# takah29/3d-reconstruction-from-multi-view-exp

Hardware: AMD Instinct MI355X
Metric: BA iterations/sec + residual-Jacobian GObs/s, 1M pts x 100 cams fp64 (higher is better)
Workload: dtype f64

## Files before the change

3d-reconstruction-from-multi-view-exp_amd/csrc/check_isa.py:

```python
#!/usr/bin/env python3
import re
import sys

KERNELS = {"k_schur_slots": (("vmcnt(7)", 7), ("vmcnt(8)", 8)),
           "k_schur_lanes": (("vmcnt(13)", 14), ("vmcnt(17)", 18))}
SLOTS_ONLY = "k_schur_slots"
VM_LOOP_OPS = ("global_load_lds_dwordx4", "global_load_lds_dword ")


def kernel_lines(text, name="k_schur_slots"):
    m = re.search(r"^_ZN\d+_GLOBAL__N_1" + str(len(name)) + name + r"E\w*:[^\n]*\n(.*?)^\.Lfunc_end", text, re.S | re.M)
    if not m:
        return None
    return [ln.strip() for ln in m.group(1).splitlines()]


def in_loop(lines, i):
    for k in range(i, -1, -1):
        m = re.match(r"\.(LBB\w+):(.*)", lines[k])
        if m:
            return "Loop" in m.group(2)
    return False


def loop_blocks(lines, wait_index):
    hdr = r"\.(LBB\w+):.*This (?:Inner )?Loop Header: Depth=1"
    head = max(i for i in range(wait_index + 1) if re.match(hdr, lines[i]))
    name = re.match(hdr, lines[head]).group(1)[1:]
    children = set()
    for ln in lines[head + 1:]:
        m = re.match(r";\s+Child Loop (BB\w+) Depth", ln)
        if not m:
            break
        children.add(m.group(1))
    own, inner = [], []
    cur = None
    for i, ln in enumerate(lines):
        m = re.match(r"\.(LBB\w+):(.*)", ln)
        if m:
            label, note = m.group(1)[1:], m.group(2)
            if i == head or f"Header={name} Depth=1" in note:
                cur = own
            elif label in children or any(f"Header={c} " in note for c in children):
                cur = inner
            else:
                cur = None
            continue
        if cur is not None:
            cur.append(ln)
    return own, inner


def check_kernel(text, name, counts):
    errs = []
    lines = kernel_lines(text, name)
    if lines is None:
        return [f"{name} not found in the ISA"]
    for count, n_ops in counts:
        idx = [i for i, ln in enumerate(lines) if ln.startswith("s_waitcnt " + count)]
        if name != SLOTS_ONLY:
            idx = [i for i in idx if in_loop(lines, i)]
        if len(idx) != 1:
            errs.append(f"{name}: expected one `s_waitcnt {count}` (the loop's counted wait), found {len(idx)}")
            continue
        body, inner = loop_blocks(lines, idx[0])
        bad = [ln for ln in body + inner if ln.startswith(("scratch_", "buffer_"))]
        if bad:
            errs.append(f"{name} {count} loop: scratch / buffer access inside the loop: {bad[:3]}")
        straight = [ln for ln in body if ln.startswith(VM_LOOP_OPS)]
        if len(straight) != n_ops:
            errs.append(f"{name} {count} loop: {len(straight)} LDS-DMA operations per iteration, the wait counts {n_ops}")
        other = [ln for ln in body if ln.startswith(("global_load", "global_store", "global_atomic", "flat_")) and not ln.startswith(VM_LOOP_OPS)]
        if other:
            errs.append(f"{name} {count} loop: vector-memory operations the wait does not count (or that return data to a register): {other[:3]}")
        stray = [ln for ln in inner if ln.startswith(VM_LOOP_OPS)]
        if stray:
            errs.append(f"{name} {count} loop: LDS-DMA inside the pacing block: {stray[:3]}")
    if name != SLOTS_ONLY:
        return errs
    for ln in lines:
        if re.match(r"\w+\s+m0\b", ln) and not ln.startswith("s_mov_b32 m0,"):
            errs.append(f"{name}: M0 written outside the gathers' asm statements: {ln}")
    vg = re.search(r"^\s*\.set _ZN\d+_GLOBAL__N_1" + str(len(name)) + name + r"E\w*\.num_vgpr, (\d+)", text, re.M)
    if vg and int(vg.group(1)) > 168:
        errs.append(f"{name} needs {vg.group(1)} VGPRs: more than the 168 of three waves per SIMD")
    return errs


# ... 48 lines not shown
```

3d-reconstruction-from-multi-view-exp_amd/csrc/host_check.cpp:

```cpp
#include <cmath>
#include <cstdio>
#include <cstring>
#include <limits>
#include <string>
#include <vector>

#include "mvba_host.h"
#include "mvba_ransac_host.h"
#include "mvba_tracks_host.h"
#include "mvba_match_host.h"

namespace mvba {
thread_local std::string g_err;
}
using namespace mvba;

static int failures = 0;
#define CHECK(x) do { if (!(x)) { std::printf("host_check: line %d: %s\n", __LINE__, #x); ++failures; } } while (0)

int main() {
  {
    const int n = 3;
    const double D[9] = {1.0, 0, 0, 0, 4.0, 0, 0, 0, 2.0};
    const double V[9] = {-0.5, 0.6, 0.0,
// ... 382 lines not shown
    int32_t cam[5], node[5], track[5];
    double xy[10];
    auto run = [&](const int64_t *kp_, const double *kxy_, const int32_t *e, int64_t ne, int32_t ml, int64_t *pt_, int32_t *cam_, int32_t *node_,
                   double *xy_, int32_t *track_, int64_t *cnt_) { return tracks_check_args(3, kp_, kxy_, e, ne, ml, pt_, cam_, node_, xy_, track_, cnt_); };
    CHECK(run(kp, kxy, edges, 3, 2, pt, cam, node, xy, track, counts) == MVBA_OK);
    CHECK(run(kp, nullptr, edges, 3, 2, pt, cam, node, nullptr, track, counts) == MVBA_OK);
    CHECK(run(kp, kxy, nullptr, 0, 2, pt, cam, node, xy, track, counts) == MVBA_OK);
    CHECK(run(nullptr, kxy, edges, 3, 2, pt, cam, node, xy, track, counts) == MVBA_ERR_BADARG && g_err == "null argument: kp_ptr (argument 2)");
    CHECK(run(kp, kxy, edges, 3, 2, nullptr, cam, node, xy, track, counts) == MVBA_ERR_BADARG && g_err == "null argument: pt_ptr (argument 8)");
    CHECK(run(kp, kxy, edges, 3, 2, pt, nullptr, node, xy, track, counts) == MVBA_ERR_BADARG && g_err == "null argument: cam_idx (argument 9)");
    CHECK(run(kp, kxy, edges, 3, 2, pt, cam, nullptr, xy, track, counts) == MVBA_ERR_BADARG && g_err == "null argument: obs_node (argument 10)");
    CHECK(run(kp, kxy, edges, 3, 2, pt, cam, node, xy, nullptr, counts) == MVBA_ERR_BADARG && g_err == "null argument: node_track (argument 12)");
    CHECK(run(kp, kxy, edges, 3, 2, pt, cam, node, xy, track, nullptr) == MVBA_ERR_BADARG && g_err == "null argument: counts (argument 13)");
    CHECK(run(kp, nullptr, edges, 3, 2, pt, cam, node, xy, track, counts) == MVBA_ERR_BADARG && g_err == "null argument: kp_xy (argument 3) with an xy to fill");
    CHECK(run(kp, kxy, edges, -1, 2, pt, cam, node, xy, track, counts) == MVBA_ERR_BADARG && g_err == "n_edges = -1: negative size");
    CHECK(run(kp, kxy, nullptr, 3, 2, pt, cam, node, xy, track, counts) == MVBA_ERR_BADARG && g_err == "null argument: edges (argument 4) with n_edges = 3");
    CHECK(run(kp, kxy, edges, 3, 1, pt, cam, node, xy, track, counts) == MVBA_ERR_BADARG && g_err == "min_length = 1 must be at least 2");
    CHECK(run(down, kxy, edges, 3, 2, pt, cam, node, xy, track, counts) == MVBA_ERR_BADARG && g_err.rfind("kp_ptr is not ascending", 0) == 0);
    CHECK(run(kp, kxy, high, 2, 2, pt, cam, node, xy, track, counts) == MVBA_ERR_BADARG && g_err == "edges[1][0] = 5: node id out of range, n_nodes = 5");
    CHECK(run(kp, kxy, low, 2, 2, pt, cam, node, xy, track, counts) == MVBA_ERR_BADARG && g_err == "edges[1][1] = -1: node id out of range, n_nodes = 5");
    CHECK(run(kp, kxy, high, 1, 2, pt, cam, node, xy, track, counts) == MVBA_OK);
  }
  {
    const double r2 = match_ratio2(0.8);
    CHECK(r2 == 0.8 * 0.8 && match_ratio2(1.0) == 1.0);
    CHECK(match_ambiguous(100, -1, r2) && match_ambiguous(0, -1, 1.0));
    CHECK(!match_ambiguous(63, 100, r2) && match_ambiguous(65, 100, r2));
    CHECK(match_ambiguous(100, 100, 1.0) && !match_ambiguous(99, 100, 1.0));
    CHECK(match_ambiguous(0, 0, 1.0) && !match_ambiguous(0, 1, r2));
    CHECK(!match_ambiguous(33292799, 33292800, 1.0) && match_ambiguous(33292800, 33292800, 1.0));
    const int64_t kp[5] = {0, 10, 10, 40, 45};
    const int32_t pr[10] = {0, 2, 2, 0, 1, 3, 3, 2, 0, 3};
    CHECK(match_chunk_end(kp, pr, 5, 0, false, 1000) == 5 && match_chunk_end(kp, pr, 5, 0, true, 1000) == 5);
    CHECK(match_chunk_end(kp, pr, 5, 0, false, 40) == 3);
    CHECK(match_chunk_end(kp, pr, 5, 0, true, 40) == 1);
    CHECK(match_chunk_end(kp, pr, 5, 1, true, 1) == 2);
    CHECK(match_chunk_end(kp, pr, 5, 2, false, 0) == 3 && match_chunk_end(kp, pr, 5, 3, false, 0) == 4);
    CHECK(match_chunk_end(kp, pr, 5, 5, true, 10) == 5 && match_chunk_end(kp, pr, 0, 0, true, 10) == 0);
    for (int32_t p0 = 0, guard = 0; p0 < 5 && guard < 10; ++guard) {
      const int32_t p1 = match_chunk_end(kp, pr, 5, p0, true, 35);
      CHECK(p1 > p0 && p1 <= 5);
      p0 = p1;
    }
  }
  {
    const int64_t kp[4] = {0, 2, 2, 5}, down[4] = {0, 3, 2, 5}, off[3] = {1, 2, 3}, big[2] = {0, 1LL << 31}, none[3] = {0, 0, 0};
    const int64_t huge[3] = {0, 1LL << 30, (1LL << 30) + 1};
    const uint8_t desc[5 * 32] = {0};
    const int32_t pr[4] = {0, 2, 2, 0}, high[4] = {0, 2, 3, 0}, low[2] = {0, -1}, self[4] = {0, 2, 2, 2}, twice[4] = {0, 1, 0, 1}, empty[4] = {1, 0, 1, 2};
    int64_t mp[3], counts[MATCH_N_COUNTS], Q = -1;
    int32_t kpp[10], d2[5];
    auto run = [&](int32_t m, const int64_t *kp_, const uint8_t *desc_, int32_t dim, const int32_t *pairs, int32_t np, double ratio, int64_t *mp_,
                   int32_t *kpp_, int32_t *d2_, int64_t *cnt_) { return match_check_args(m, kp_, desc_, dim, pairs, np, ratio, mp_, kpp_, d2_, cnt_, &Q); };
    CHECK(run(3, kp, desc, 32, pr, 2, 0.8, mp, kpp, d2, counts) == MVBA_OK && Q == 5);
    CHECK(run(3, kp, desc, 512, pr, 2, 0.0, mp, kpp, d2, counts) == MVBA_OK && run(3, kp, desc, 16, pr, 2, 1.0, mp, kpp, d2, counts) == MVBA_OK);
    CHECK(run(3, kp, desc, 32, nullptr, 0, 0.8, mp, kpp, d2, counts) == MVBA_OK && Q == 0);
    CHECK(run(3, kp, desc, 32, empty, 2, 0.8, mp, kpp, d2, counts) == MVBA_OK && Q == 0);
    CHECK(run(2, none, nullptr, 128, nullptr, 0, 0.8, mp, kpp, d2, counts) == MVBA_OK);
    CHECK(run(3, nullptr, desc, 32, pr, 2, 0.8, mp, kpp, d2, counts) == MVBA_ERR_BADARG && g_err == "null argument: kp_ptr (argument 2)");
    CHECK(run(3, kp, desc, 32, pr, 2, 0.8, nullptr, kpp, d2, counts) == MVBA_ERR_BADARG && g_err == "null argument: match_ptr (argument 10)");
    CHECK(run(3, kp, desc, 32, pr, 2, 0.8, mp, nullptr, d2, counts) == MVBA_ERR_BADARG && g_err == "null argument: kp_pairs (argument 11)");
    CHECK(run(3, kp, desc, 32, pr, 2, 0.8, mp, kpp, nullptr, counts) == MVBA_ERR_BADARG && g_err == "null argument: dist2 (argument 12)");
    CHECK(run(3, kp, desc, 32, pr, 2, 0.8, mp, kpp, d2, nullptr) == MVBA_ERR_BADARG && g_err == "null argument: counts (argument 16)");
    CHECK(run(3, kp, nullptr, 32, pr, 2, 0.8, mp, kpp, d2, counts) == MVBA_ERR_BADARG && g_err == "null argument: desc (argument 3) with 5 keypoints");
    CHECK(run(3, kp, desc, 32, nullptr, 2, 0.8, mp, kpp, d2, counts) == MVBA_ERR_BADARG && g_err == "null argument: pairs (argument 5) with n_pairs = 2");
    CHECK(run(3, kp, desc, 32, pr, -1, 0.8, mp, kpp, d2, counts) == MVBA_ERR_BADARG && g_err == "n_pairs = -1: negative size");
    CHECK(run(0, kp, desc, 32, pr, 2, 0.8, mp, kpp, d2, counts) == MVBA_ERR_BADARG && g_err == "n_images = 0 must be at least 1");
    CHECK(run(2, off, desc, 32, pr, 0, 0.8, mp, kpp, d2, counts) == MVBA_ERR_BADARG && g_err == "kp_ptr[0] = 1 must be 0");
    CHECK(run(3, down, desc, 32, pr, 2, 0.8, mp, kpp, d2, counts) == MVBA_ERR_BADARG && g_err == "kp_ptr is not ascending: kp_ptr[2] = 2 after 3");
    CHECK(run(1, big, desc, 32, pr, 0, 0.8, mp, kpp, d2, counts) == MVBA_ERR_BADARG && g_err == "n_nodes = kp_ptr[n_images] = 2147483648 must be < 2^31");
    for (int32_t dim : {0, 8, 24, 520, 528, -16}) {
      CHECK(run(3, kp, desc, dim, pr, 2, 0.8, mp, kpp, d2, counts) == MVBA_ERR_BADARG);
      CHECK(g_err == "dim = " + std::to_string(dim) + " must be a multiple of 16 in 16 .. 512");
    }
    CHECK(run(3, kp, desc, 32, pr, 2, -0.1, mp, kpp, d2, counts) == MVBA_ERR_BADARG && g_err == "ratio = -0.100000 must be in (0, 1], or 0 for no ratio test");
    CHECK(run(3, kp, desc, 32, pr, 2, 1.5, mp, kpp, d2, counts) == MVBA_ERR_BADARG && g_err == "ratio = 1.500000 must be in (0, 1], or 0 for no ratio test");
    CHECK(run(3, kp, desc, 32, pr, 2, std::numeric_limits<double>::quiet_NaN(), mp, kpp, d2, counts) == MVBA_ERR_BADARG && g_err.find("nan must be in") != std::string::npos);
    CHECK(run(3, kp, desc, 32, high, 2, 0.8, mp, kpp, d2, counts) == MVBA_ERR_BADARG && g_err == "pairs[1][0] = 3: image index out of range, n_images = 3");
    CHECK(run(3, kp, desc, 32, low, 1, 0.8, mp, kpp, d2, counts) == MVBA_ERR_BADARG && g_err == "pairs[0][1] = -1: image index out of range, n_images = 3");
    CHECK(run(3, kp, desc, 32, self, 2, 0.8, mp, kpp, d2, counts) == MVBA_ERR_BADARG && g_err == "pairs[1] = (2, 2): an image is not matched with itself");
    CHECK(run(2, huge, desc, 32, twice, 2, 0.8, mp, kpp, d2, counts) == MVBA_ERR_BADARG && g_err == "Q = 2147483648 queries up to pair 1: the sum over the pairs must be < 2^31");
    CHECK(run(2, huge, desc, 32, twice, 1, 0.8, mp, kpp, d2, counts) == MVBA_OK && Q == (1LL << 30));
  }
  if (failures) return 1;
  std::printf("host_check ok\n");
  return 0;
}
```

3d-reconstruction-from-multi-view-exp_amd/csrc/mvba.hip:

```cpp
#include <dlfcn.h>
#include <hip/hip_runtime.h>
#include <rccl/rccl.h>

#include <algorithm>
#include <atomic>
#include <chrono>
#include <cmath>
#include <cstdlib>
#include <cstring>
#include <thread>
#include <type_traits>
#include <utility>
#include <vector>

#include "mvba_common.h"
#include "mvba_host.h"
#include "mvba_ransac_host.h"
#include "mvba_tracks_host.h"
#include "mvba_match_host.h"

namespace mvba {
thread_local std::string g_err;
}
using namespace mvba;
// ... 28 lines not shown
  Rccl r;
  r.lib = lib;
  r.origin = origin;
#define BIND(field, sym)                                                                       \
  if (!(r.field = reinterpret_cast<decltype(r.field)>(dlsym(lib, sym))))                       \
    return fail(MVBA_ERR_RCCL, std::string("librccl (") + origin + ") lacks " + sym)
  BIND(GetVersion, "ncclGetVersion");
  BIND(GetUniqueId, "ncclGetUniqueId");
  BIND(CommInitRank, "ncclCommInitRank");
  BIND(CommDestroy, "ncclCommDestroy");
  BIND(AllReduce, "ncclAllReduce");
  BIND(AllGather, "ncclAllGather");
  BIND(GetErrorString, "ncclGetErrorString");
#undef BIND
  if (r.GetVersion(&r.version) != ncclSuccess) return fail(MVBA_ERR_RCCL, "ncclGetVersion failed");
  const int major = r.version >= 10000 ? r.version / 10000 : r.version / 1000;
  if (major != NCCL_MAJOR)
    return fail(MVBA_ERR_RCCL, "librccl (" + origin + ") is NCCL " + std::to_string(r.version) + ", this library was built against " +
                                   std::to_string(NCCL_VERSION_CODE));
  g_rccl = r;
  return MVBA_OK;
}
}

namespace {

#include "mvba_device.h"
#include "mvba_linearize.h"
#include "mvba_schur.h"
#include "mvba_dense.h"
#include "mvba_solve.h"
#include "mvba_tail.h"
#include "mvba_index.h"
#include "mvba_cov.h"
#include "mvba_map.h"

}

enum { SCHUR_PAIRS = 1, SCHUR_SLOTS = 2, SCHUR_DENSE = 3 };
struct mvba_handle {
  int device = 0;
  hipStream_t stream = nullptr;
  DevBufs mem;
  long long N = 0, nobs = 0;
  int m = 0, gauge_axis = 0, D = 0, ld = 0;
  double f0 = 1.0;
  long long *d_pt_ptr = nullptr;
  int *d_cam = nullptr, *d_obs_pt = nullptr;
  double2 *d_xy = nullptr;
  int *d_tiles = nullptr;
  int *d_tile_slot = nullptr;
  int4 *d_splits = nullptr;
  double *d_PLsplit = nullptr;
  int n_splits = 0;
  int n_tiles = 0;
  bool any_split = false;
  int k1_threads = 512;
  bool use_pairs = true;
  int schur_mode = 2;
  long long n_items = 0, n_items_offdiag = 0, n_slot_items = 0;
  int n_units = 0, rccl_version = 0, q_max = 0, n_waves = 0, slot_nR = 8, slot_nseg = 0;
  int slot_w = PSTEP;
  long long *d_range_o0 = nullptr;
  int *d_seg_end = nullptr, *d_prog = nullptr;
  bool check_solve = false;
  double check_solve_tol = 1e-8;
  bool gcam = false;
  double *d_cam18 = nullptr, *d_dxi10 = nullptr;
  bool index_on_device = false;
  int4 *d_wdesc = nullptr;
  int *d_it_x = nullptr;
  int *d_wunits = nullptr;
  bool force_big = false;
  int *d_it_k = nullptr, *d_it_l = nullptr, *d_it_a = nullptr, *d_unit_ptr = nullptr, *d_q_ptr = nullptr, *d_q_units = nullptr;
  int4 *d_units = nullptr;
  double *d_partial = nullptr;
  double *d_dense_part = nullptr;
  int *d_dense_obs = nullptr;
  int dense_blocks = 0, dense_tiles = 0;
  double *d_X[2] = {nullptr, nullptr}, *d_cam15[2] = {nullptr, nullptr};
  int cur = 0;
  bool have_params = false, linearized = false, have_trial = false;
  double2 *d_rec = nullptr;
  double *d_PL = nullptr, *d_PB = nullptr;
  double *d_Ab = nullptr, *d_Ared = nullptr, *d_Ztiles = nullptr, *d_Lblk = nullptr, *d_dxi = nullptr, *d_dX = nullptr, *d_lu = nullptr;
  int *d_ipiv = nullptr;
  double *d_partials = nullptr, *d_cost = nullptr, *h_cost = nullptr;
  double *d_mail = nullptr;
  unsigned long long cost_seq = 0;
  bool mail_pending = false;
  int n_partials = 0, cost_grid = 0;
  int *d_flag = nullptr, *h_flag = nullptr;
  unsigned *d_bar = nullptr;
  int n_cu = 1;
  bool chol_onepass = true;
  int trail64_min = 200;
  unsigned barrier_polls = 1u << 22;
  ncclComm_t comm = nullptr;
  mvba_host_allreduce_fn host_ar = nullptr;
  void *host_ar_user = nullptr;
  std::vector<double> host_buf;
  int rank = 0, nranks = 1;
  double *d_allcost = nullptr, *h_allcost = nullptr, *d_sim = nullptr;
  std::vector<double *> snap_slabs;
  long long n_snap = 0;
  int profiling = 0;
  mvba_stats stats{};
  struct Ev { int kid; hipEvent_t a, b; };
  std::vector<Ev> pending;
  std::vector<hipEvent_t> pool;
  double *d_cov_sig = nullptr, *d_cov_panel = nullptr, *d_cov_pts = nullptr, *d_cov_cam = nullptr;
  int loss = LOSS_SQUARED;
  double loss_b = 0.0;
  double *d_sqw = nullptr;
  double2 *d_resid = nullptr;
  double *d_init_cams = nullptr;
  bool mapped = false;
  int n_free = 0, map_ld = 0, map_U = 0;
  std::vector<int> map_col, map_ptr, map_mem;
  int *d_map_col = nullptr, *d_map_ptr = nullptr, *d_map_mem = nullptr;
  double *d_map_x = nullptr, *d_cov_sigv = nullptr;
  int2 *d_map_pairs = nullptr;
  double *d_map_part = nullptr;
  int n_map_pairs = 0, map_nblk = 1;
  uint8_t *d_held = nullptr;
  long long n_held = 0;
  int solve_D() const { return mapped ? n_free : D; }
  int solve_ld() const { return mapped ? map_ld : ld; }
};

namespace {

const char *kKernelNames[MVBA_K_COUNT] = {"resid_jac", "point_blocks", "point_inv", "schur",
                                          "allreduce", "solve",        "backsub_cost", "cost"};

struct Timed {
  mvba_handle *h;
  int kid;
  hipEvent_t a = nullptr, b = nullptr;
  bool on = false;
  Timed(mvba_handle *h_, int kid_) : h(h_), kid(kid_) {
    on = kid >= 0 && (h->profiling == 1 || (h->profiling == 2 && (kid == MVBA_K_SCHUR || kid == MVBA_K_RESID_JAC)));
    if (!on) return;
    auto get = [&]() {
      hipEvent_t e;
      if (!h->pool.empty()) { e = h->pool.back(); h->pool.pop_back(); }
      else hipEventCreate(&e);
      return e;
    };
    a = get(); b = get();
    hipEventRecord(a, h->stream);
  }
  ~Timed() {
    if (!on) return;
    hipEventRecord(b, h->stream);
    h->pending.push_back({kid, a, b});
  }
};

void drain_events(mvba_handle *h) {
  for (auto &p : h->pending) {
    float ms = 0.f;
    if (hipEventElapsedTime(&ms, p.a, p.b) == hipSuccess) {
      h->stats.ms[p.kid] += ms;
      h->stats.launches[p.kid] += 1;
    }
// ... 88 lines not shown
  const void *fn(bool rb) const { return rb ? (const void *)robust : (const void *)squared; }
};
template <typename... A>
LossKernel<A...> loss_kernel(void (*squared)(A...), void (*robust)(A..., LossArgs)) { return {squared, robust}; }

template <typename... A, typename... Args>
void launch_loss(mvba_handle *h, LossKernel<A...> k, dim3 grid, dim3 block, size_t lds, Args... args) {
  if (h->loss != LOSS_SQUARED) hipLaunchKernelGGL(k.robust, grid, block, lds, h->stream, args..., LossArgs{h->loss_b, h->d_sqw});
  else hipLaunchKernelGGL(k.squared, grid, block, lds, h->stream, args...);
}

auto resid_jac_kernel(bool gcam, int loss) {
  if (loss == LOSS_CAUCHY)
    return gcam ? loss_kernel(k_resid_jac<true>, k_resid_jac<true, LOSS_CAUCHY, LossArgs>) : loss_kernel(k_resid_jac<false>, k_resid_jac<false, LOSS_CAUCHY, LossArgs>);
  return gcam ? loss_kernel(k_resid_jac<true>, k_resid_jac<true, LOSS_HUBER, LossArgs>) : loss_kernel(k_resid_jac<false>, k_resid_jac<false, LOSS_HUBER, LossArgs>);
}
auto cost_kernel(bool gcam, int loss) {
  if (loss == LOSS_CAUCHY)
    return gcam ? loss_kernel(k_cost<true>, k_cost<true, LOSS_CAUCHY, LossArgs>) : loss_kernel(k_cost<false>, k_cost<false, LOSS_CAUCHY, LossArgs>);
  return gcam ? loss_kernel(k_cost<true>, k_cost<true, LOSS_HUBER, LossArgs>) : loss_kernel(k_cost<false>, k_cost<false, LOSS_HUBER, LossArgs>);
}
template <int G>
auto backsub_kernel_g(int bt, bool gcam) {
  if (gcam) return loss_kernel(k_backsub<G, 256, true>, k_backsub<G, 256, true, true, LossArgs>);
  if (bt == 1024) return loss_kernel(k_backsub<G, 1024>, k_backsub<G, 1024, false, true, LossArgs>);
  if (bt == 512) return loss_kernel(k_backsub<G, 512>, k_backsub<G, 512, false, true, LossArgs>);
  return loss_kernel(k_backsub<G>, k_backsub<G, 256, false, true, LossArgs>);
}
auto backsub_kernel(int G, int bt, bool gcam) {
  return G == 2 ? backsub_kernel_g<2>(bt, gcam) : (G == 4 ? backsub_kernel_g<4>(bt, gcam) : backsub_kernel_g<8>(bt, gcam));
}
template <int T>
auto dense_kernel_t(bool table) {
  return table ? loss_kernel(k_schur_dense<T, true>, k_schur_dense<T, true, true, LossArgs>)
               : loss_kernel(k_schur_dense<T, false>, k_schur_dense<T, false, true, LossArgs>);
}
auto dense_kernel(int T, bool table) {
  switch (T) {
    case 1: return dense_kernel_t<1>(table);
    case 2: return dense_kernel_t<2>(table);
    case 3: return dense_kernel_t<3>(table);
    case 4: return dense_kernel_t<4>(table);
    case 5: return dense_kernel_t<5>(table);
    case 6: return dense_kernel_t<6>(table);
    case 7: return dense_kernel_t<7>(table);
    case 8: return dense_kernel_t<8>(table);
    case 9: return dense_kernel_t<9>(table);
    case 10: return dense_kernel_t<10>(table);
    case 11: return dense_kernel_t<11>(table);
    default: return dense_kernel_t<12>(table);
  }
}
size_t dense_lds_bytes(int T, int mm) {
  const int CH = dense_ch(T);
  return sizeof(double) * ((size_t)2 * 3 * CH * 16 * T + (size_t)2 * CH * mm * 32) + sizeof(double2) * CH * ((size_t)mm * REC + 8) +
         sizeof(double) * (CH * (size_t)mm + 2 * 3 * CH);
}

size_t k1_lds_bytes(int m, bool gcam, int threads) {
  return (size_t)((gcam ? 0 : ((m * CAM_LDS + 1) & ~1)) + (threads / 64) * 64 * 2 * REC) * sizeof(double);
}
size_t cam_lds_bytes(int m, bool gcam, bool with_dxi) { return gcam ? 0 : (size_t)m * (CAM_LDS + (with_dxi ? DXI_LDS : 0)) * sizeof(double); }

void cam_tables(mvba_handle *h, const double *cam15, const double *dxi) {
  if (h->gcam) hipLaunchKernelGGL(k_cam_tables, dim3((h->m + 255) / 256), dim3(256), 0, h->stream, h->m, cam15, dxi, h->f0, h->d_cam18, h->d_dxi10);
}
int launch_cost(mvba_handle *h, const double *cam15, const double *X) {
  const size_t lds = cam_lds_bytes(h->m, h->gcam, false);
  cam_tables(h, cam15, nullptr);
  launch_loss(h, cost_kernel(h->gcam, h->loss), dim3(h->cost_grid), dim3(lds > 40 * 1024 ? 512 : 256), lds, h->nobs, h->m, cam15, X,
              h->d_obs_pt, h->d_cam, h->d_xy, h->f0, h->d_partials, h->d_cam18);
  double *mail = cost_mail(h);
  const unsigned long long seq = h->cost_seq;
  hipLaunchKernelGGL(k_sum_partials, dim3(1), dim3(1024), 0, h->stream, h->d_partials, h->cost_grid, h->d_cost, h->d_flag, mail, seq);
  MVBA_HIP(hipGetLastError());
  return MVBA_OK;
}

struct CreateKnobs {
  bool schur_set = false;
  bool schur_slots = false, schur_lanes = false, schur_pairs = false, schur_dense = false;
  bool index_host = false, index_global = false;
  bool force_big = false;
  bool chol_launches = false;
  int trail64_min = 200;
  unsigned barrier_polls = 1u << 22;
  bool check_solve = false;
  double check_solve_tol = 1e-8;
  bool timing = false;
};

CreateKnobs read_create_knobs() {
  CreateKnobs k;
  auto is = [](const char *ev, const char *v) { return ev && !strcmp(ev, v); };
  const char *schur = getenv("MVBA_SCHUR");
  k.schur_set = schur != nullptr;
  k.schur_slots = is(schur, "slots");
  k.schur_lanes = is(schur, "lanes");
  k.schur_pairs = is(schur, "pairs");
  k.schur_dense = is(schur, "dense");
  const char *index = getenv("MVBA_INDEX");
  k.index_host = is(index, "host");
  k.index_global = is(index, "global");
  k.force_big = getenv("MVBA_FORCE_BIG") != nullptr;
  k.chol_launches = is(getenv("MVBA_CHOL"), "launches");
  if (const char *ev = getenv("MVBA_TRAIL64_MIN")) k.trail64_min = std::max(0, atoi(ev));
  if (const char *ev = getenv("MVBA_CHOL_BARRIER_POLLS")) k.barrier_polls = (unsigned)std::max(0LL, atoll(ev));
  if (const char *ev = getenv("MVBA_CHECK_SOLVE")) {
    const double v = atof(ev);
    k.check_solve = v != 0.0;
    if (v > 0.0 && v < 1.0) k.check_solve_tol = v;
  }
  k.timing = getenv("MVBA_CREATE_TIMING") != nullptr;
  return k;
}

#include "mvba_create.h"

}

extern "C" {

const char *mvba_version(void) { return "mvba 0.2 (gfx950)"; }
const char *mvba_last_error(void) { return g_err.c_str(); }
const char *mvba_kernel_name(int32_t k) { return (k >= 0 && k < MVBA_K_COUNT) ? kKernelNames[k] : ""; }

int mvba_device_count(int32_t *count) {
  int n = 0;
  hipError_t e = hipGetDeviceCount(&n);
  if (e != hipSuccess) {
    *count = 0;
    return fail(MVBA_ERR_HIP, std::string("hipGetDeviceCount: ") + hipGetErrorString(e));
  }
  *count = n;
  return MVBA_OK;
}

int mvba_create(const mvba_problem *p, mvba_handle **out) { return create_engine(p, LOSS_SQUARED, 0.0, out); }

int mvba_create_robust(const mvba_problem *p, int32_t loss, double scale, mvba_handle **out) {
  if (!p || !out) return fail(MVBA_ERR_BADARG, "null argument");
  if (loss == LOSS_SQUARED) return create_engine(p, LOSS_SQUARED, 0.0, out);
  if (loss != LOSS_HUBER && loss != LOSS_CAUCHY)
    return fail(MVBA_ERR_BADARG, "loss = " + std::to_string(loss) + " is not a loss (0 squared, 1 Huber, 2 Cauchy)");
  if (!(scale > 0.0) || !std::isfinite(scale))
    return fail(MVBA_ERR_BADARG, "loss scale = " + std::to_string(scale) + " must be finite and > 0 for a robust loss");
  if (!(p->f0 > 0.0) || !std::isfinite(p->f0)) return fail(MVBA_ERR_BADARG, "a robust loss needs f0 > 0");
  const double r = scale / p->f0;
  return create_engine(p, loss, r * r, out);
}

void mvba_destroy(mvba_handle *h) {
  if (!h) return;
  hipSetDevice(h->device);
  if (h->stream) hipStreamSynchronize(h->stream);
  if (h->comm) g_rccl.CommDestroy(h->comm);
  h->mem.release_all();
  if (h->h_cost) hipHostFree(h->h_cost);
  if (h->h_allcost) hipHostFree(h->h_allcost);
  for (auto &p : h->pending) { hipEventDestroy(p.a); hipEventDestroy(p.b); }
  for (auto e : h->pool) hipEventDestroy(e);
  if (h->stream) hipStreamDestroy(h->stream);
  delete h;
}

namespace {
void pack_cam15(int m, const double *f, const double *u, const double *t, const double *R, double *cam ) {
  for (int k = 0; k < m; ++k) {
    double *c = cam + (size_t)k * CAM_IN;
    c[0] = f[k]; c[1] = u[2 * k]; c[2] = u[2 * k + 1];
    for (int i = 0; i < 3; ++i) c[3 + i] = t[3 * k + i];
    for (int i = 0; i < 9; ++i) c[6 + i] = R[9 * k + i];
  }
}
void unpack_cam15(const double *cam , int m, double *f, double *u, double *t, double *R) {
  for (int k = 0; k < m; ++k) {
    const double *c = cam + (size_t)k * CAM_IN;
    f[k] = c[0]; u[2 * k] = c[1]; u[2 * k + 1] = c[2];
    for (int i = 0; i < 3; ++i) t[3 * k + i] = c[3 + i];
    for (int i = 0; i < 9; ++i) R[9 * k + i] = c[6 + i];
  }
}
}

int mvba_set_params(mvba_handle *h, const double *X, const double *f, const double *u, const double *t, const double *R) {
  if (!h || !X || !f || !u || !t || !R) return fail(MVBA_ERR_BADARG, "null argument");
  MVBA_HIP(hipSetDevice(h->device));
  std::vector<double> cam((size_t)h->m * CAM_IN);
  pack_cam15(h->m, f, u, t, R, cam.data());
  MVBA_HIP(hipMemcpyAsync(h->d_X[h->cur], X, sizeof(double) * 3 * h->N, hipMemcpyHostToDevice, h->stream));
  MVBA_HIP(hipMemcpyAsync(h->d_cam15[h->cur], cam.data(), sizeof(double) * cam.size(), hipMemcpyHostToDevice, h->stream));
  MVBA_HIP(hipStreamSynchronize(h->stream));
  h->have_params = true; h->linearized = false; h->have_trial = false;
  return MVBA_OK;
}

int mvba_get_params(mvba_handle *h, double *X, double *f, double *u, double *t, double *R) {
  if (!h || !X || !f || !u || !t || !R) return fail(MVBA_ERR_BADARG, "null argument");
  if (!h->have_params) return fail(MVBA_ERR_STATE, "no parameters set");
  MVBA_HIP(hipSetDevice(h->device));
  std::vector<double> cam((size_t)h->m * CAM_IN);
  MVBA_HIP(hipMemcpyAsync(X, h->d_X[h->cur], sizeof(double) * 3 * h->N, hipMemcpyDeviceToHost, h->stream));
  MVBA_HIP(hipMemcpyAsync(cam.data(), h->d_cam15[h->cur], sizeof(double) * cam.size(), hipMemcpyDeviceToHost, h->stream));
  MVBA_HIP(hipStreamSynchronize(h->stream));
  unpack_cam15(cam.data(), h->m, f, u, t, R);
  return MVBA_OK;
}

int mvba_apply_similarity(mvba_handle *h, const double *R0, const double *t0, double scale) {
  if (!h || !R0 || !t0) return fail(MVBA_ERR_BADARG, "null argument");
  if (!h->have_params) return fail(MVBA_ERR_STATE, "no parameters set");
  MVBA_HIP(hipSetDevice(h->device));
  double T[13];
  memcpy(T, R0, 9 * sizeof(double));
  memcpy(T + 9, t0, 3 * sizeof(double));
  T[12] = scale;
  if (!h->d_sim) {
    int rc = h->mem.alloc(&h->d_sim, 13);
    if (rc) return rc;
  }
  MVBA_HIP(hipMemcpyAsync(h->d_sim, T, sizeof(T), hipMemcpyHostToDevice, h->stream));
  const long long n = std::max<long long>(h->N, h->m);
  hipLaunchKernelGGL(k_similarity, dim3((unsigned)((n + 255) / 256)), dim3(256), 0, h->stream, h->N, h->m, h->d_X[h->cur],
                     h->d_cam15[h->cur], h->d_sim);
  MVBA_HIP(hipGetLastError());
  MVBA_HIP(hipStreamSynchronize(h->stream));
  h->linearized = false; h->have_trial = false;
  return MVBA_OK;
}

int mvba_cost(mvba_handle *h, double *E) {
  if (!h || !E) return fail(MVBA_ERR_BADARG, "null argument");
  if (!h->have_params) return fail(MVBA_ERR_STATE, "no parameters set");
  MVBA_HIP(hipSetDevice(h->device));
  {
    Timed t(h, MVBA_K_COST);
    int rc = launch_cost(h, h->d_cam15[h->cur], h->d_X[h->cur]);
    if (rc) return rc;
  }
  return global_cost(h, E);
}

namespace {
void launch_resid_jac(mvba_handle *h) {
  const int kt = h->k1_threads;
  cam_tables(h, h->d_cam15[h->cur], nullptr);
  const int wpb = kt / 64;
  const int grid = std::max(1, std::min(2048 * 256 / kt, (h->n_tiles + wpb - 1) / wpb));
  launch_loss(h, resid_jac_kernel(h->gcam, h->loss), dim3(grid), dim3(kt), k1_lds_bytes(h->m, h->gcam, kt), h->nobs, h->m, h->d_cam15[h->cur],
              h->d_X[h->cur], h->d_obs_pt, h->d_cam, h->d_xy, h->f0, h->d_tiles, h->n_tiles, h->d_rec, h->d_PL,
              h->d_tile_slot, h->d_PLsplit, h->d_cam18);
  if (h->n_splits)
    hipLaunchKernelGGL(k_sum_split, dim3((9 * h->n_splits + 255) / 256), dim3(256), 0, h->stream, h->n_splits, h->d_splits,
                       h->d_PLsplit, h->d_PL);
}

void launch_point_inv(mvba_handle *h, double c) {
  const int m = h->m;
  const size_t n9 = 9 * (size_t)m, nA = strip_offset(m, m);
  const long long nAb = (long long)(nA + n9);
  const unsigned grid = (unsigned)std::max<long long>((h->N + 255) / 256, std::min<long long>((nAb + 1023) / 1024, 4096));
  const long long nprog = h->slot_w == LANES_W ? 0 : (long long)h->slot_nR * h->slot_nseg * PACE_STRIDE;
  const int want_r = h->schur_mode == SCHUR_DENSE ? 1 : 0;
  if (h->n_held)
    hipLaunchKernelGGL(k_point_inv<const uint8_t *>, dim3(std::max(grid, 1u)), dim3(256), 0, h->stream, h->N, c, h->d_PL, h->d_PB, h->d_flag,
                       h->d_Ab, nAb, h->d_prog, nprog, want_r, (const uint8_t *)h->d_held);
  else
    hipLaunchKernelGGL(k_point_inv<>, dim3(std::max(grid, 1u)), dim3(256), 0, h->stream, h->N, c, h->d_PL, h->d_PB, h->d_flag,
                       h->d_Ab, nAb, h->d_prog, nprog, want_r);
}

void launch_schur(mvba_handle *h, double c) {
  const int m = h->m;
  const size_t nA = strip_offset(m, m);
  double *d_A = h->d_Ab, *d_b = h->d_Ab + nA;
  if (h->use_pairs) {
    const bool big = (std::max<long long>(h->nobs, h->N) + 1) * 128LL >= (1LL << 32) || h->force_big;
    if (h->schur_mode == SCHUR_SLOTS && h->slot_w == LANES_W) {
      if (h->n_waves)
        hipLaunchKernelGGL(k_schur_lanes, dim3(h->n_waves), dim3(64), LANES_LDS, h->stream, h->d_wdesc, h->d_wunits, h->d_it_x, h->d_rec, h->d_PB, c,
                           h->f0, h->d_partial, h->slot_nR, h->d_range_o0);
    } else if (h->schur_mode == SCHUR_SLOTS) {
      if (h->n_waves)
        hipLaunchKernelGGL(k_schur_slots, dim3(h->n_waves), dim3(64), SLOT_LDS, h->stream, h->d_wdesc,
                           h->d_wunits, h->d_it_x, (const int *)nullptr, (const int *)nullptr, h->d_rec, h->d_PB, c, h->f0, h->d_partial,
                           h->slot_nR, h->d_seg_end, h->d_prog, h->slot_nseg, SLOT_LAG, h->d_range_o0);
    } else if (h->n_units) {
      auto launch = [&](auto kern, auto... robust) {
        hipLaunchKernelGGL(kern, dim3(8 * h->q_max), dim3(64), PAIRS_LDS, h->stream, h->d_units, h->d_q_ptr, h->d_q_units, h->d_it_k, h->d_it_l,
                           h->d_it_a, h->d_rec, h->d_PB, c, h->f0, h->d_partial, robust...);
      };
      if (h->loss != LOSS_SQUARED) launch(big ? k_schur_pairs_big_robust : k_schur_pairs_robust, (const double *)h->d_sqw);
      else launch(big ? k_schur_pairs_big : k_schur_pairs);
    }
    hipLaunchKernelGGL(k_schur_reduce, dim3((unsigned)((long long)m * (m + 1) / 2)), dim3(128), 0, h->stream, m, h->d_unit_ptr,
                       h->d_partial, d_A, d_b);
  } else if (h->schur_mode == SCHUR_DENSE) {
    const int T = (9 * m + 15) / 16;
    launch_loss(h, dense_kernel(T, h->d_dense_obs != nullptr), dim3(h->dense_blocks), dim3(64 * (dense_consumers(T) + dense_ch(T))), dense_lds_bytes(T, m),
                (const double2 *)h->d_rec, (const double *)h->d_PB, (const int *)h->d_dense_obs, (long long)h->N, m, 1.0 / h->f0, h->d_dense_part);
    const long long n_el = (long long)nA + 9 * m;
    hipLaunchKernelGGL(k_schur_dense_finish, dim3((unsigned)((n_el + 3) / 4)), dim3(256), 0, h->stream, m, T, h->dense_blocks,
                       (const double *)h->d_dense_part, c, d_A, d_b);
  }
}

int allreduce_Ab(mvba_handle *h, bool timed) {
  const int m = h->m;
  const size_t n9 = 9 * (size_t)m, nA = strip_offset(m, m);
  if (h->comm) {
    Timed t(h, timed ? MVBA_K_ALLREDUCE : -1);
    ncclResult_t r = g_rccl.AllReduce(h->d_Ab, h->d_Ab, nA + n9, ncclDouble, ncclSum, h->comm, h->stream);
    if (r != ncclSuccess) return fail(MVBA_ERR_RCCL, std::string("ncclAllReduce: ") + g_rccl.GetErrorString(r));
  } else if (h->host_ar) {
    h->host_buf.resize(nA + n9);
    MVBA_HIP(hipMemcpyAsync(h->host_buf.data(), h->d_Ab, sizeof(double) * (nA + n9), hipMemcpyDeviceToHost, h->stream));
    MVBA_HIP(hipStreamSynchronize(h->stream));
    const auto t0 = std::chrono::steady_clock::now();
    if (h->host_ar(h->host_ar_user, h->host_buf.data(), (int64_t)(nA + n9))) return fail(MVBA_ERR_RCCL, "host all-reduce callback failed");
    MVBA_HIP(hipMemcpyAsync(h->d_Ab, h->host_buf.data(), sizeof(double) * (nA + n9), hipMemcpyHostToDevice, h->stream));
    if (timed && h->profiling) {
      h->stats.ms[MVBA_K_ALLREDUCE] += std::chrono::duration<double, std::milli>(std::chrono::steady_clock::now() - t0).count();
      h->stats.launches[MVBA_K_ALLREDUCE] += 1;
    }
  }
  return MVBA_OK;
}

void launch_map_tied(mvba_handle *h, double *M, int ld, int mirror) {
  if (!h->n_map_pairs) return;
  hipLaunchKernelGGL(k_map_tied, dim3(h->n_map_pairs, h->map_nblk), dim3(256), 0, h->stream, h->m, (const double *)h->d_Ab,
                     (const int *)h->d_map_ptr, (const int *)h->d_map_mem, (const int2 *)h->d_map_pairs, h->d_map_part);
  hipLaunchKernelGGL(k_map_tied_finish, dim3((h->n_map_pairs + 255) / 256), dim3(256), 0, h->stream, h->n_map_pairs, h->map_nblk, ld,
                     mirror, (const int2 *)h->d_map_pairs, (const double *)h->d_map_part, M);
}

void launch_factor(mvba_handle *h) {
  const int m = h->m, D = h->solve_D();
  double *d_A = h->d_Ab, *d_b = h->d_Ab + strip_offset(m, m);
  const int ld = h->solve_ld();
  const int ntc = (D + NB - 1) / NB;
  if (h->mapped) {
    const int U = h->map_U, ntu = (U + NB - 1) / NB;
    hipLaunchKernelGGL(k_map_compact, dim3(ntu * (ntu + 1) / 2 + (D + 255) / 256), dim3(256), 0, h->stream, D, ld, m, U, ntu, d_A, d_b,
                       h->d_map_ptr, h->d_map_mem, h->d_Ared, h->d_bar, 1 + 4 * ((D + SBW - 1) / SBW));
    if (U < D)
      hipLaunchKernelGGL(k_map_rows, dim3((D + 63) / 64, D - U), dim3(256), 0, h->stream, D, ld, m, U, d_A, h->d_map_ptr, h->d_map_mem,
                         h->d_Ared);
    launch_map_tied(h, h->d_Ared, ld, 0);
  } else
  hipLaunchKernelGGL(k_compact, dim3(ntc * (ntc + 1) / 2 + (D + 255) / 256), dim3(256), 0, h->stream, D, ld, m, h->gauge_axis, ntc, d_A, d_b,
                     h->d_Ared, h->d_bar, 1 + 4 * ((D + SBW - 1) / SBW));
  for (int jS = 0; jS < D; jS += SBW) {
    const int jE = std::min(jS + SBW, D);
    hipLaunchKernelGGL(k_chol_super, dim3((D + 1 - jE + 63) / 64), dim3(SUPER_THREADS), SUPER_LDS, h->stream, h->d_Ared, ld, D, jS,
                       h->d_Ztiles + (size_t)(jS / NB) * NB * NB, h->d_Lblk + (size_t)(jS / SBW) * SBW * SBW, h->d_flag);
    if (jE < D) {
      const int nt32 = (D + 1 - jE + NB - 1) / NB, nt64 = (D + 1 - jE + TB - 1) / TB;
      if (jE - jS == SBW && nt64 * (nt64 + 1) / 2 >= h->trail64_min)
        hipLaunchKernelGGL(k_chol_trail64, dim3(nt64 * (nt64 + 1) / 2), dim3(256), TRAIL64_LDS, h->stream, h->d_Ared, ld, D, jS, jE);
      else
        hipLaunchKernelGGL(k_chol_trail32, dim3(nt32 * (nt32 + 1) / 2), dim3(256), 0, h->stream, h->d_Ared, ld, D, jS, jE);
// ... 291 lines not shown
  if (!pairs.empty()) MVBA_HIP(hipMemcpy(h->d_map_pairs, pairs.data(), sizeof(int2) * pairs.size(), hipMemcpyHostToDevice));
  MVBA_HIP(hipMemcpy(h->d_map_col, col, sizeof(int) * n9, hipMemcpyHostToDevice));
  MVBA_HIP(hipMemcpy(h->d_map_ptr, ptr.data(), sizeof(int) * (n_free + 1), hipMemcpyHostToDevice));
  MVBA_HIP(hipMemcpy(h->d_map_mem, mem.data(), sizeof(int) * mem.size(), hipMemcpyHostToDevice));
  h->map_col.assign(col, col + n9);
  h->map_ptr = ptr;
  h->map_mem = mem;
  h->n_free = n_free;
  h->map_ld = (n_free + 3) & ~3;
  h->map_U = U;
  h->mapped = true;
  return MVBA_OK;
}

int mvba_set_point_hold(mvba_handle *h, const uint8_t *held) {
  if (!h) return fail(MVBA_ERR_BADARG, "null handle");
  MVBA_HIP(hipSetDevice(h->device));
  long long n_held = 0;
  std::vector<uint8_t> mask;
  if (held) {
    mask.resize((size_t)h->N);
    for (long long a = 0; a < h->N; ++a) n_held += (mask[(size_t)a] = held[a] ? 1 : 0);
  }
  if (n_held && !h->d_held) {
    int rc = h->mem.alloc(&h->d_held, (size_t)h->N);
    if (rc) return rc;
  }
  if (n_held) {
    MVBA_HIP(hipStreamSynchronize(h->stream));
    MVBA_HIP(hipMemcpy(h->d_held, mask.data(), mask.size(), hipMemcpyHostToDevice));
  }
  h->n_held = n_held;
  h->have_trial = false;
  return MVBA_OK;
}

int mvba_residuals(mvba_handle *h, double *e) {
  if (!h || !e) return fail(MVBA_ERR_BADARG, "null argument");
  if (!h->have_params) return fail(MVBA_ERR_STATE, "no parameters set");
  MVBA_HIP(hipSetDevice(h->device));
  if (!h->nobs) return MVBA_OK;
  if (!h->d_resid) {
    int rc = h->mem.alloc(&h->d_resid, h->nobs);
    if (rc) return rc;
  }
  const size_t lds = cam_lds_bytes(h->m, h->gcam, false);
  cam_tables(h, h->d_cam15[h->cur], nullptr);
  const unsigned grid = (unsigned)std::min<long long>(4096, (h->nobs + 255) / 256);
  hipLaunchKernelGGL(h->gcam ? k_residuals<true> : k_residuals<false>, dim3(grid), dim3(256), lds, h->stream, h->nobs, h->m,
                     (const double *)h->d_cam15[h->cur], (const double *)h->d_X[h->cur], (const int *)h->d_obs_pt, (const int *)h->d_cam,
                     (const double2 *)h->d_xy, h->f0, h->d_resid, (const double *)h->d_cam18);
  MVBA_HIP(hipGetLastError());
  MVBA_HIP(hipMemcpyAsync(e, h->d_resid, sizeof(double2) * h->nobs, hipMemcpyDeviceToHost, h->stream));
  MVBA_HIP(hipStreamSynchronize(h->stream));
  return MVBA_OK;
}

int mvba_covariance(mvba_handle *h, double *point_cov, double *cam_cov, double *cam_cov_full, double *timings_ms) {
  if (!h) return fail(MVBA_ERR_BADARG, "null handle");
  if (h->loss != LOSS_SQUARED)
    return fail(MVBA_ERR_BADARG, "mvba_covariance: the covariance is defined for the squared loss only (this engine has a robust loss)");
  if (!h->have_params) return fail(MVBA_ERR_STATE, "no parameters set");
  MVBA_HIP(hipSetDevice(h->device));
  const int m = h->m, D = h->solve_D(), ld = h->solve_ld(), nt = (D + NB - 1) / NB;
  const size_t n_sig = sig_block(m, m, m);
  auto free_cov = [&]() {
    for (double **q : {&h->d_cov_sig, &h->d_cov_panel, &h->d_cov_pts, &h->d_cov_cam}) h->mem.release(*q);
  };
  int local_rc = MVBA_OK;
  if (!h->d_cov_sig || !h->d_cov_panel || !h->d_cov_pts || !h->d_cov_cam) {
    free_cov();
    local_rc = h->mem.alloc(&h->d_cov_sig, n_sig);
    if (!local_rc) local_rc = h->mem.alloc(&h->d_cov_panel, 2 * (size_t)h->D * NB);
    if (!local_rc) local_rc = h->mem.alloc(&h->d_cov_pts, 6 * (size_t)h->N);
    if (!local_rc) local_rc = h->mem.alloc(&h->d_cov_cam, 81 * (size_t)m);
    if (local_rc) free_cov();
  }
  hipEvent_t ev[5] = {};
  struct EvFree { hipEvent_t *e; ~EvFree() { for (int i = 0; i < 5; ++i) if (e[i]) hipEventDestroy(e[i]); } } ev_free{ev};
  for (auto &e : ev)
    if (!local_rc && hipEventCreate(&e) != hipSuccess) local_rc = fail(MVBA_ERR_HIP, "hipEventCreate failed");
  const int mv = (D + 6) / 9 + 1;
  if (!local_rc && h->mapped && D > 0 && !h->d_cov_sigv) local_rc = h->mem.alloc(&h->d_cov_sigv, n_sig);
  const bool sharded = h->comm || h->host_ar;
  if (local_rc && !sharded) return local_rc;
  const std::string local_err = local_rc ? g_err : std::string();
  double *d_b = h->d_Ab + strip_offset(m, m);
  if (!local_rc) {
    MVBA_HIP(hipEventRecord(ev[0], h->stream));
    if (h->nobs) launch_resid_jac(h);
    h->linearized = true; h->have_trial = false;
    launch_point_inv(h, 0.0);
    launch_schur(h, 0.0);
    MVBA_HIP(hipGetLastError());
  } else {
    MVBA_HIP(hipMemsetAsync(d_b + 3, 0xFF, sizeof(double), h->stream));
  }
  {
    int rc = allreduce_Ab(h, false);
    if (rc) return rc;
  }
  if (sharded) {
    double mark = 0.0;
    MVBA_HIP(hipMemcpyAsync(&mark, d_b + 3, sizeof(double), hipMemcpyDeviceToHost, h->stream));
    MVBA_HIP(hipStreamSynchronize(h->stream));
    if (local_rc) return fail(local_rc, local_err);
    if (std::isnan(mark))
      return fail(MVBA_ERR_HIP, "mvba_covariance: another rank could not allocate its covariance buffers (or the reduced system is not finite)");
  }
  MVBA_HIP(hipEventRecord(ev[1], h->stream));
  if (D > 0) launch_factor(h);
  MVBA_HIP(hipEventRecord(ev[2], h->stream));
  if (D > 0)
  hipLaunchKernelGGL(k_cov_assemble, dim3(nt), dim3(256), 0, h->stream, h->d_Ared, ld, D, (const double *)h->d_Ztiles,
                     (const double *)h->d_Lblk);
  double *panel[2] = {h->d_cov_panel, h->d_cov_panel + (size_t)D * NB};
  for (int J = nt - 1; J >= 0; --J) {
    const int grid = (nt - 1 - J) + (J >= 1 ? nt - J : 0);
    if (grid)
      hipLaunchKernelGGL(k_cov_trtri, dim3(grid), dim3(256), 0, h->stream, h->d_Ared, ld, D, nt, J, (const double *)panel[J & 1],
                         panel[(J + 1) & 1]);
  }
  MVBA_HIP(hipMemsetAsync(h->d_cov_sig, 0, sizeof(double) * n_sig, h->stream));
  if (h->mapped) {
    if (D > 0) {
      hipLaunchKernelGGL(k_cov_lauum, dim3(nt * (nt + 1) / 2), dim3(256), 0, h->stream, (const double *)h->d_Ared, ld, D, nt, mv,
                         h->gauge_axis, h->d_cov_sigv);
      hipLaunchKernelGGL(k_map_cov_expand, dim3((unsigned)((81 * m + 255) / 256), m), dim3(256), 0, h->stream, m, mv, h->gauge_axis,
                         (const int *)h->d_map_col, (const double *)h->d_cov_sigv, h->d_cov_sig);
    }
  } else
  hipLaunchKernelGGL(k_cov_lauum, dim3(nt * (nt + 1) / 2), dim3(256), 0, h->stream, (const double *)h->d_Ared, ld, D, nt, m,
                     h->gauge_axis, h->d_cov_sig);
  MVBA_HIP(hipEventRecord(ev[3], h->stream));
  if (h->N && point_cov) {
    const double pairs = h->N ? 0.5 * ((double)h->nobs / (double)h->N) * ((double)h->nobs / (double)h->N + 1.0) : 0.0;
    const int G = pairs > 48.0 ? 64 : (pairs > 24.0 ? 32 : (pairs > 12.0 ? 16 : 8));
    const unsigned grid = (unsigned)std::min<long long>(8192, (h->N * G + 255) / 256);
    auto launch = [&](auto kern, auto... held) {
      hipLaunchKernelGGL(kern, dim3(grid), dim3(256), 0, h->stream, h->N, m, (const long long *)h->d_pt_ptr, (const int *)h->d_cam,
                         (const double2 *)h->d_rec, (const double *)h->d_PL, (const double *)h->d_cov_sig, 1.0 / h->f0, h->d_cov_pts,
                         h->d_flag, held...);
    };
    if (h->n_held) {
      using M = const uint8_t *;
      launch(G == 64 ? k_point_cov<64, M> : (G == 32 ? k_point_cov<32, M> : (G == 16 ? k_point_cov<16, M> : k_point_cov<8, M>)), (M)h->d_held);
    } else
      launch(G == 64 ? k_point_cov<64> : (G == 32 ? k_point_cov<32> : (G == 16 ? k_point_cov<16> : k_point_cov<8>)));
  }
  if (cam_cov)
    hipLaunchKernelGGL(k_cov_cam_diag, dim3((unsigned)((81LL * m + 255) / 256)), dim3(256), 0, h->stream, m,
                       (const double *)h->d_cov_sig, h->d_cov_cam);
  MVBA_HIP(hipGetLastError());
  MVBA_HIP(hipEventRecord(ev[4], h->stream));
  int fl = 0;
  MVBA_HIP(hipMemcpyAsync(&fl, h->d_flag, sizeof(int), hipMemcpyDeviceToHost, h->stream));
  MVBA_HIP(hipStreamSynchronize(h->stream));
  if (fl) {
    MVBA_HIP(hipMemsetAsync(h->d_flag, 0, sizeof(int), h->stream));
    MVBA_HIP(hipStreamSynchronize(h->stream));
    if (fl & (FLAG_POINT_SINGULAR | FLAG_COV_POINT)) return fail(MVBA_ERR_SINGULAR, "Singular matrix (a point block E_a is singular: a point seen once, or without parallax)");
    return fail(MVBA_ERR_SINGULAR, "Singular matrix (the undamped reduced camera system is not positive definite)");
  }
  if (timings_ms)
    for (int i = 0; i < 4; ++i) {
      float ms = 0.f;
      MVBA_HIP(hipEventElapsedTime(&ms, ev[i], ev[i + 1]));
      timings_ms[i] = ms;
    }
  if (point_cov && h->N) MVBA_HIP(hipMemcpy(point_cov, h->d_cov_pts, sizeof(double) * 6 * h->N, hipMemcpyDeviceToHost));
  if (cam_cov) MVBA_HIP(hipMemcpy(cam_cov, h->d_cov_cam, sizeof(double) * 81 * m, hipMemcpyDeviceToHost));
  if (cam_cov_full) {
    std::vector<double> strip((size_t)SIG_BS * m);
    const size_t n9 = 9 * (size_t)m;
    for (int k = 0; k < m; ++k) {
      MVBA_HIP(hipMemcpy(strip.data(), h->d_cov_sig + sig_block(k, k, m), sizeof(double) * SIG_BS * (m - k), hipMemcpyDeviceToHost));
      for (int l = k; l < m; ++l) {
        const double *b = strip.data() + (size_t)SIG_BS * (l - k);
        for (int i = 0; i < 9; ++i)
          for (int j = 0; j < 9; ++j) {
            const double v = 2.0 * b[9 * i + j];
            cam_cov_full[(9 * (size_t)k + i) * n9 + 9 * (size_t)l + j] = v;
            cam_cov_full[(9 * (size_t)l + j) * n9 + 9 * (size_t)k + i] = v;
          }
      }
    }
  }
  return MVBA_OK;
}

namespace {
constexpr int SNAP_SLAB = 8;
size_t snap_stride(const mvba_handle *h) { return (3 * (size_t)h->N + (size_t)CAM_IN * h->m + 1) & ~(size_t)1; }
double *snap_entry(const mvba_handle *h, long long i) { return h->snap_slabs[(size_t)(i / SNAP_SLAB)] + snap_stride(h) * (size_t)(i % SNAP_SLAB); }
}

int mvba_snapshot(mvba_handle *h) {
  if (!h) return fail(MVBA_ERR_BADARG, "null handle");
  if (!h->have_params) return fail(MVBA_ERR_STATE, "no parameters set");
  MVBA_HIP(hipSetDevice(h->device));
  if ((size_t)(h->n_snap / SNAP_SLAB) >= h->snap_slabs.size()) {
    double *p = nullptr;
    int rc = h->mem.alloc(&p, snap_stride(h) * SNAP_SLAB);
    if (rc) return rc;
    h->snap_slabs.push_back(p);
  }
  double *dst = snap_entry(h, h->n_snap);
  MVBA_HIP(hipMemcpyAsync(dst, h->d_X[h->cur], sizeof(double) * 3 * h->N, hipMemcpyDeviceToDevice, h->stream));
  MVBA_HIP(hipMemcpyAsync(dst + 3 * h->N, h->d_cam15[h->cur], sizeof(double) * CAM_IN * h->m, hipMemcpyDeviceToDevice, h->stream));
  h->n_snap++;
  return MVBA_OK;
}

int mvba_snapshot_count(mvba_handle *h, int64_t *n) {
  if (!h || !n) return fail(MVBA_ERR_BADARG, "null argument");
  *n = h->n_snap;
  return MVBA_OK;
}

int mvba_snapshot_read(mvba_handle *h, int64_t i, double *X, double *f, double *u, double *t, double *R) {
  if (!h || !X || !f || !u || !t || !R) return fail(MVBA_ERR_BADARG, "null argument");
  if (i < 0 || i >= h->n_snap) return fail(MVBA_ERR_BADARG, "no such log entry");
  MVBA_HIP(hipSetDevice(h->device));
  const double *src = snap_entry(h, i);
  std::vector<double> cam((size_t)h->m * CAM_IN);
  MVBA_HIP(hipMemcpyAsync(X, src, sizeof(double) * 3 * h->N, hipMemcpyDeviceToHost, h->stream));
  MVBA_HIP(hipMemcpyAsync(cam.data(), src + 3 * h->N, sizeof(double) * cam.size(), hipMemcpyDeviceToHost, h->stream));
  MVBA_HIP(hipStreamSynchronize(h->stream));
  unpack_cam15(cam.data(), h->m, f, u, t, R);
  return MVBA_OK;
}

int mvba_snapshot_restore(mvba_handle *h, int64_t i) {
  if (!h) return fail(MVBA_ERR_BADARG, "null handle");
  if (i < 0 || i >= h->n_snap) return fail(MVBA_ERR_BADARG, "no such log entry");
  MVBA_HIP(hipSetDevice(h->device));
  const double *src = snap_entry(h, i);
  MVBA_HIP(hipMemcpyAsync(h->d_X[h->cur], src, sizeof(double) * 3 * h->N, hipMemcpyDeviceToDevice, h->stream));
  MVBA_HIP(hipMemcpyAsync(h->d_cam15[h->cur], src + 3 * h->N, sizeof(double) * CAM_IN * h->m, hipMemcpyDeviceToDevice, h->stream));
  h->have_params = true; h->linearized = false; h->have_trial = false;
  return MVBA_OK;
}

int mvba_snapshot_clear(mvba_handle *h) {
  if (!h) return fail(MVBA_ERR_BADARG, "null handle");
  h->n_snap = 0;
  return MVBA_OK;
}

int mvba_set_profiling(mvba_handle *h, int32_t enabled) {
  if (!h) return fail(MVBA_ERR_BADARG, "null handle");
  h->profiling = enabled == 2 ? 2 : (enabled != 0);
  return MVBA_OK;
}

int mvba_get_stats(mvba_handle *h, mvba_stats *out) {
  if (!h || !out) return fail(MVBA_ERR_BADARG, "null argument");
  MVBA_HIP(hipSetDevice(h->device));
  int rc = sync_and_drain(h);
  if (rc) return rc;
  *out = h->stats;
  return MVBA_OK;
}

int mvba_get_info(mvba_handle *h, int64_t *out8) {
  if (!h || !out8) return fail(MVBA_ERR_BADARG, "null argument");
  out8[0] = h->n_items;
  out8[1] = h->n_items_offdiag;
  out8[2] = h->n_units;
  out8[3] = h->schur_mode | (h->schur_mode == SCHUR_SLOTS ? h->slot_w << 8 : 0);
  out8[4] = h->rccl_version;
  out8[5] = NCCL_VERSION_CODE;
  out8[6] = h->nranks;
  out8[7] = h->schur_mode == SCHUR_SLOTS ? h->n_slot_items : 0;
  return MVBA_OK;
}

int mvba_reset_stats(mvba_handle *h) {
  if (!h) return fail(MVBA_ERR_BADARG, "null handle");
  MVBA_HIP(hipSetDevice(h->device));
  int rc = sync_and_drain(h);
  if (rc) return rc;
  h->stats = mvba_stats{};
  return MVBA_OK;
}

int mvba_comm_unique_id(void *id128) {
  if (!id128) return fail(MVBA_ERR_BADARG, "null argument");
  static_assert(sizeof(ncclUniqueId) == 128, "ncclUniqueId size");
  if (int rc = rccl_load()) return rc;
  ncclUniqueId id;
  ncclResult_t r = g_rccl.GetUniqueId(&id);
  if (r != ncclSuccess) return fail(MVBA_ERR_RCCL, std::string("ncclGetUniqueId: ") + g_rccl.GetErrorString(r));
  memcpy(id128, &id, 128);
  return MVBA_OK;
}

int mvba_comm_init(mvba_handle *h, const void *id128, int32_t rank, int32_t n_ranks) {
  if (!h || !id128 || n_ranks < 1 || rank < 0 || rank >= n_ranks) return fail(MVBA_ERR_BADARG, "bad comm arguments");
  MVBA_HIP(hipSetDevice(h->device));
  if (int rc = rccl_load()) return rc;
  ncclUniqueId id;
  memcpy(&id, id128, 128);
  ncclResult_t r = g_rccl.CommInitRank(&h->comm, n_ranks, id, rank);
  if (r != ncclSuccess) return fail(MVBA_ERR_RCCL, std::string("ncclCommInitRank: ") + g_rccl.GetErrorString(r));
  h->rank = rank; h->nranks = n_ranks;
  h->rccl_version = g_rccl.version;
  int rc = h->mem.alloc(&h->d_allcost, 2 * (size_t)n_ranks);
  if (rc) return rc;
  MVBA_HIP(hipHostMalloc((void **)&h->h_allcost, 2 * sizeof(double) * n_ranks));
  return MVBA_OK;
}

int mvba_comm_init_host(mvba_handle *h, int32_t rank, int32_t n_ranks, mvba_host_allreduce_fn fn, void *user) {
  if (!h || !fn || n_ranks < 1 || rank < 0 || rank >= n_ranks) return fail(MVBA_ERR_BADARG, "bad comm arguments");
  if (h->comm) return fail(MVBA_ERR_STATE, "handle already has an RCCL communicator");
  h->host_ar = fn; h->host_ar_user = user;
  h->rank = rank; h->nranks = n_ranks;
  return MVBA_OK;
}

int mvba_debug_read(mvba_handle *h, int32_t which, double *out, int64_t capacity, int64_t *n) {
  if (!h || !n) return fail(MVBA_ERR_BADARG, "null argument");
  MVBA_HIP(hipSetDevice(h->device));
  const size_t n9 = 9 * (size_t)h->m;
  long long cnt = 0;
  switch (which) {
    case MVBA_BUF_RESIDUAL: cnt = 2 * h->nobs; break;
    case MVBA_BUF_JX: cnt = 6 * h->nobs; break;
    case MVBA_BUF_JC: cnt = 18 * h->nobs; break;
    case MVBA_BUF_E: cnt = 6 * h->N; break;
    case MVBA_BUF_DP: cnt = 3 * h->N; break;
    case MVBA_BUF_A_FULL: cnt = n9 * n9; break;
    case MVBA_BUF_B_FULL: cnt = n9; break;
    case MVBA_BUF_DXI: cnt = n9; break;
    case MVBA_BUF_DX: case MVBA_BUF_TRIAL_X: cnt = 3 * h->N; break;
    case MVBA_BUF_TRIAL_CAM: cnt = (long long)CAM_IN * h->m; break;
    case MVBA_BUF_INDEX_K: case MVBA_BUF_INDEX_L: case MVBA_BUF_INDEX_A:
      cnt = h->schur_mode == SCHUR_SLOTS ? h->n_slot_items : (h->schur_mode == SCHUR_PAIRS ? h->n_items : 0);
      break;
    case MVBA_BUF_INDEX_SEG: cnt = h->schur_mode == SCHUR_SLOTS ? (long long)h->n_waves * h->slot_nseg : 0; break;
    case MVBA_BUF_WEIGHT: cnt = h->nobs; break;
    default: return fail(MVBA_ERR_BADARG, "unknown buffer id");
  }
  *n = cnt;
  if (!out) return MVBA_OK;
  if (capacity < cnt) return fail(MVBA_ERR_BADARG, "output buffer too small");
  MVBA_HIP(hipStreamSynchronize(h->stream));
  auto d2h = [&](const void *src, size_t bytes) { return hipMemcpy(out, src, bytes, hipMemcpyDeviceToHost); };
  if (which == MVBA_BUF_RESIDUAL || which == MVBA_BUF_JX || which == MVBA_BUF_JC) {
    std::vector<double> r((size_t)2 * REC * h->nobs);
    MVBA_HIP(hipMemcpy(r.data(), h->d_rec, sizeof(double) * r.size(), hipMemcpyDeviceToHost));
    std::vector<double> sw;
    if (h->loss != LOSS_SQUARED && which == MVBA_BUF_JC) {
      sw.resize(h->nobs);
      MVBA_HIP(hipMemcpy(sw.data(), h->d_sqw, sizeof(double) * sw.size(), hipMemcpyDeviceToHost));
    }
    for (long long o = 0; o < h->nobs; ++o) {
      const double cu = sw.empty() ? 1.0 / h->f0 : sw[o] / h->f0;
      const double *q = r.data() + (size_t)o * 2 * REC;
      if (which == MVBA_BUF_RESIDUAL) {
        out[2 * o] = q[14]; out[2 * o + 1] = q[15];
      } else if (which == MVBA_BUF_JX) {
        for (int rr = 0; rr < 2; ++rr) for (int i = 0; i < 3; ++i) out[6 * o + 3 * rr + i] = q[2 * i + rr];
      } else {
        double *jc = out + 18 * o;
        for (int rr = 0; rr < 2; ++rr) {
          jc[9 * rr + 0] = q[6 + rr];
          jc[9 * rr + 1] = rr == 0 ? cu : 0.0;
          jc[9 * rr + 2] = rr == 1 ? cu : 0.0;
          for (int i = 0; i < 3; ++i) jc[9 * rr + 3 + i] = -q[2 * i + rr];
          for (int i = 0; i < 3; ++i) jc[9 * rr + 6 + i] = q[8 + 2 * i + rr];
        }
      }
    }
  } else if (which == MVBA_BUF_WEIGHT) {
    if (h->loss != LOSS_SQUARED) MVBA_HIP(d2h(h->d_sqw, sizeof(double) * h->nobs));
    else for (long long o = 0; o < h->nobs; ++o) out[o] = 1.0;
  } else if (which == MVBA_BUF_E || which == MVBA_BUF_DP) {
    std::vector<double> pl(9 * (size_t)h->N);
    MVBA_HIP(hipMemcpy(pl.data(), h->d_PL, sizeof(double) * pl.size(), hipMemcpyDeviceToHost));
    for (long long a = 0; a < h->N; ++a) {
      if (which == MVBA_BUF_E) for (int i = 0; i < 6; ++i) out[6 * a + i] = pl[9 * a + i];
      else for (int i = 0; i < 3; ++i) out[3 * a + i] = pl[9 * a + 6 + i];
    }
  } else if (which == MVBA_BUF_A_FULL) {
    const int m = h->m;
    std::vector<double> pk(strip_offset(m, m));
    MVBA_HIP(hipMemcpy(pk.data(), h->d_Ab, sizeof(double) * pk.size(), hipMemcpyDeviceToHost));
    for (size_t r = 0; r < n9; ++r)
      for (size_t cc = 0; cc < n9; ++cc) {
        const size_t lo = std::min(r, cc), hi = std::max(r, cc);
        const int k = (int)(lo / 9), l = (int)(hi / 9);
        const size_t rr = (k == l) ? r : lo, c2 = (k == l) ? cc : hi;
        out[r * n9 + cc] = pk[strip_offset(k, m) + (rr - 9 * k) * (size_t)(9 * (m - k)) + (c2 - 9 * k)];
      }
  } else if (which == MVBA_BUF_B_FULL) {
    MVBA_HIP(d2h(h->d_Ab + strip_offset(h->m, h->m), sizeof(double) * cnt));
  } else if (which == MVBA_BUF_DXI) {
    MVBA_HIP(d2h(h->d_dxi, sizeof(double) * cnt));
  } else if (which == MVBA_BUF_DX) {
    MVBA_HIP(d2h(h->d_dX, sizeof(double) * cnt));
  } else if (which == MVBA_BUF_TRIAL_X) {
    MVBA_HIP(d2h(h->d_X[1 - h->cur], sizeof(double) * cnt));
  } else if (which == MVBA_BUF_TRIAL_CAM) {
    MVBA_HIP(d2h(h->d_cam15[1 - h->cur], sizeof(double) * cnt));
  } else if (which >= MVBA_BUF_INDEX_K && which <= MVBA_BUF_INDEX_SEG) {
    if (h->schur_mode == SCHUR_SLOTS && which != MVBA_BUF_INDEX_SEG) {
      const int W = h->slot_w, row = slot_idx_ints(W);
      const long long n_steps = cnt / W;
      std::vector<int> tmp((size_t)n_steps * row);
      if (cnt) MVBA_HIP(hipMemcpy(tmp.data(), h->d_it_x, sizeof(int) * tmp.size(), hipMemcpyDeviceToHost));
      const int off = which == MVBA_BUF_INDEX_K ? 0 : (which == MVBA_BUF_INDEX_L ? W : 2 * W);
      for (long long st = 0; st < n_steps; ++st)
        for (int sl = 0; sl < W; ++sl) out[st * W + sl] = (double)tmp[(size_t)st * row + off + sl];
      return MVBA_OK;
    }
    const int *src = which == MVBA_BUF_INDEX_K ? h->d_it_k : (which == MVBA_BUF_INDEX_L ? h->d_it_l : (which == MVBA_BUF_INDEX_A ? h->d_it_a : h->d_seg_end));
    std::vector<int> tmp((size_t)cnt);
    if (cnt) MVBA_HIP(hipMemcpy(tmp.data(), src, sizeof(int) * tmp.size(), hipMemcpyDeviceToHost));
    for (long long i = 0; i < cnt; ++i) out[i] = (double)tmp[i];
  }
  return MVBA_OK;
}

int mvba_project(const double *X, int64_t n_points, const double *K, const double *R, const double *t, int32_t n_images,
                 const int64_t *pt_ptr, const int32_t *cam_idx, int64_t n_obs, double *xy, int32_t device) {
  if (!X || !K || !R || !t || !xy) return fail(MVBA_ERR_BADARG, "null argument");
  if (n_points < 0 || n_images < 1 || n_obs < 0 || (pt_ptr && !cam_idx)) return fail(MVBA_ERR_BADARG, "bad sizes");
  if (!pt_ptr && n_obs != n_points * (int64_t)n_images) return fail(MVBA_ERR_BADARG, "dense grid needs n_obs = n_points * n_images");
  if (n_points >= (1LL << 31)) return fail(MVBA_ERR_BADARG, "n_points must be < 2^31");
  if ((size_t)n_images * 12 * sizeof(double) > 160 * 1024 - 256) return fail(MVBA_ERR_BADARG, "too many cameras for the LDS camera table (max 1704)");
  if (n_obs == 0) return MVBA_OK;
  if (device >= 0) MVBA_HIP(hipSetDevice(device));
// ... 66 lines not shown
```

3d-reconstruction-from-multi-view-exp_amd/csrc/mvba_create.h:

```cpp

__global__ __launch_bounds__(256) void k_xy_from_planes(const double2 *__restrict__ planes, long long N, int m, double2 *__restrict__ xy) {
  const long long a = (long long)blockIdx.x * 256 + threadIdx.x;
  const int k = blockIdx.y;
  if (a < N) xy[a * m + k] = planes[(long long)k * N + a];
}

#define CR(x) do { int rc_ = (x); if (rc_) return rc_; } while (0)
#define CRH(x) do { hipError_t e_ = (x); if (e_ != hipSuccess) return fail(MVBA_ERR_HIP, std::string(#x) + ": " + hipGetErrorString(e_)); } while (0)

struct CreateTimer {
  bool on;
  std::chrono::steady_clock::time_point t_last = std::chrono::steady_clock::now();
  void lap(const char *what) {
    if (!on) return;
    const auto now = std::chrono::steady_clock::now();
    fprintf(stderr, "mvba_create: %-28s %8.1f ms\n", what, std::chrono::duration<double, std::milli>(now - t_last).count());
    t_last = now;
  }
};

int validate_problem(const mvba_problem *p, std::vector<int> &obs_pt) {
  if (p->n_points < 0 || p->n_images < 2 || p->n_obs < 0 || !p->pt_ptr || (p->n_obs && (!p->cam_idx || !p->xy)))
    return fail(MVBA_ERR_BADARG, "bad problem sizes or null arrays (need n_images >= 2)");
  if (p->gauge_axis != 0 && p->gauge_axis != 1) return fail(MVBA_ERR_BADARG, "gauge_axis must be 0 or 1");
// ... 544 lines not shown
  hipLaunchKernelGGL(dv.hist_lds ? k_idx_fill<false> : k_idx_fill<true>, dim3((unsigned)(dv.idx_waves / IDX_WAVES)), dim3(64 * IDX_WAVES), dv.idx_lds,
                     stream, N, m, (int)P, in.d_pt_ptr, in.d_cam, dv.idx_chunk, dv.d_hist, d_S, d_vp_ptr, d_vp_off, d_pk, d_pl, d_pa,
                     (const int *)nullptr);
  CRH(hipGetLastError());
  timer.lap("items sorted by pair");
  std::vector<long long> lo_tab((size_t)VP * (nR + 1));
  {
    long long *d_rl = nullptr, *d_lo = nullptr;
    CR(tmp.alloc(&d_rl, (size_t)nR + 1)); CR(tmp.alloc(&d_lo, lo_tab.size()));
    CRH(hipMemcpyAsync(d_rl, R.lo.data(), sizeof(long long) * (nR + 1), hipMemcpyHostToDevice, stream));
    const long long nt = (long long)lo_tab.size();
    hipLaunchKernelGGL(k_idx_bounds, dim3((unsigned)((nt + 255) / 256)), dim3(256), 0, stream, VP, nR, d_vp_off, d_rl, d_pa, d_lo, (const int *)nullptr);
    CRH(hipMemcpyAsync(lo_tab.data(), d_lo, sizeof(long long) * nt, hipMemcpyDeviceToHost, stream));
    CRH(hipStreamSynchronize(stream));
    tmp.release(d_rl); tmp.release(d_lo);
  }
  std::vector<int> uid;
  number_units(in, plan, [&](int v, int r) { return lo_tab[(size_t)v * (nR + 1) + r]; }, ix, uid);
  timer.lap("units");
  if (plan.mode == SCHUR_SLOTS) {
    SlotWaves sw = make_slot_waves(in, plan, uid, ix);
    const long long n_waves = sw.n_waves;
    const int nSeg = sw.nSeg;
    CR(upload_range_o0(in, R, engine, ix));
    long long *d_slbeg = nullptr, *d_wbeg = nullptr;
    int *d_sllen = nullptr, *d_wsteps = nullptr;
    CR(tmp.alloc(&d_slbeg, sw.sl_beg.size())); CR(tmp.alloc(&d_sllen, sw.sl_len.size()));
    CR(tmp.alloc(&d_wsteps, (size_t)n_waves)); CR(tmp.alloc(&d_wbeg, (size_t)n_waves + 1));
    CRH(hipMemcpyAsync(d_slbeg, sw.sl_beg.data(), sizeof(long long) * sw.sl_beg.size(), hipMemcpyHostToDevice, stream));
    CRH(hipMemcpyAsync(d_sllen, sw.sl_len.data(), sizeof(int) * sw.sl_len.size(), hipMemcpyHostToDevice, stream));
    const int W = plan.W;
    const auto merge_count = W == LANES_W ? k_idx_merge<false, LANES_W> : k_idx_merge<false, PSTEP>;
    const auto merge_fill = W == LANES_W ? k_idx_merge<true, LANES_W> : k_idx_merge<true, PSTEP>;
    hipLaunchKernelGGL(merge_count, dim3((unsigned)n_waves), dim3(64), 0, stream, n_waves, nR, nSeg, slot_skew(W), SLOT_SEG, d_slbeg, d_sllen,
                       ix.d_range_o0, d_pk, d_pl, d_pa, d_wbeg, 0, (int)N, d_wsteps, (int *)nullptr, (int *)nullptr, (int *)nullptr,
                       (int *)nullptr, (const long long *)in.d_pt_ptr);
    std::vector<int> ws32(n_waves);
    CRH(hipMemcpyAsync(ws32.data(), d_wsteps, sizeof(int) * n_waves, hipMemcpyDeviceToHost, stream));
    CRH(hipStreamSynchronize(stream));
    for (long long b = 0; b < n_waves; ++b) sw.w_steps[b] = ws32[b];
    timer.lap("slot merge (count)");
    long long total_steps = 0;
    CR(place_slot_steps(plan, sw, ix, total_steps));
    const size_t rows = (size_t)total_steps * W;
    CR(engine.alloc(&ix.d_it_k, rows)); CR(engine.alloc(&ix.d_it_l, rows)); CR(engine.alloc(&ix.d_it_a, rows));
    CR(engine.alloc(&ix.d_seg_end, ix.seg_end.size()));
    CRH(hipMemcpyAsync(d_wbeg, sw.w_beg.data(), sizeof(long long) * (n_waves + 1), hipMemcpyHostToDevice, stream));
    hipLaunchKernelGGL(merge_fill, dim3((unsigned)n_waves), dim3(64), 0, stream, n_waves, nR, nSeg, slot_skew(W), SLOT_SEG, d_slbeg, d_sllen,
                       ix.d_range_o0, d_pk, d_pl, d_pa, d_wbeg, 0, (int)N, d_wsteps, ix.d_it_k, ix.d_it_l, ix.d_it_a, ix.d_seg_end, (const long long *)in.d_pt_ptr);
    CRH(hipGetLastError());
    CRH(hipStreamSynchronize(stream));
    timer.lap("slot merge (fill)");
    finish_slot_waves(plan, sw, total_steps, ix);
  } else {
    build_work_queues(in, plan, uid, ix);
    engine.adopt(tmp, d_pk); engine.adopt(tmp, d_pl); engine.adopt(tmp, d_pa);
    ix.d_it_k = d_pk; ix.d_it_l = d_pl; ix.d_it_a = d_pa;
  }
  tmp.release_all();
  ix.on_device = true;
  return MVBA_OK;
}

int alloc_engine_buffers(mvba_handle *h, K1Tiles &t) {
  const long long N = h->N, nobs = h->nobs;
  const int m = h->m;
  h->cost_grid = (int)std::max<long long>(1, std::min<long long>(2048, (nobs + 255) / 256));
  h->n_partials = std::max(h->cost_grid, 4096);
  CR(h->mem.alloc(&h->d_obs_pt, nobs));
  CR(h->mem.alloc(&h->d_xy, nobs));
  h->n_tiles = (int)t.tiles.size() - 1;
  h->any_split = t.any_split;
  if (t.any_split) {
    t.tile_slot.resize(t.tiles.size(), -1);
    h->n_splits = (int)t.splits.size();
    CR(h->mem.alloc(&h->d_tile_slot, t.tile_slot.size()));
    CR(h->mem.alloc(&h->d_splits, t.splits.size()));
    CR(h->mem.alloc(&h->d_PLsplit, 9 * (size_t)t.n_split_slots));
    CRH(hipMemcpy(h->d_tile_slot, t.tile_slot.data(), sizeof(int) * t.tile_slot.size(), hipMemcpyHostToDevice));
    CRH(hipMemcpy(h->d_splits, t.splits.data(), sizeof(int4) * t.splits.size(), hipMemcpyHostToDevice));
  }
  CR(h->mem.alloc(&h->d_tiles, t.tiles.size()));
  for (int i = 0; i < 2; ++i) { CR(h->mem.alloc(&h->d_X[i], 3 * N)); CR(h->mem.alloc(&h->d_cam15[i], (size_t)CAM_IN * m)); }
  CR(h->mem.alloc(&h->d_rec, (size_t)REC * (nobs + 1)));
  if (h->loss != LOSS_SQUARED) {
    CR(h->mem.alloc(&h->d_sqw, nobs + 1));
    CRH(hipMemset(h->d_sqw, 0, sizeof(double) * (nobs + 1)));
  }
  CR(h->mem.alloc(&h->d_PL, 9 * N));
  CR(h->mem.alloc(&h->d_PB, (size_t)PBS * (N + 1)));
  CRH(hipMemset(h->d_rec + (size_t)REC * nobs, 0, sizeof(double2) * REC));
  CRH(hipMemset(h->d_PB + (size_t)PBS * N, 0, sizeof(double) * PBS));
  const size_t n9 = 9 * (size_t)m;
  CR(h->mem.alloc(&h->d_Ab, strip_offset(m, m) + n9));
  CR(h->mem.alloc(&h->d_Ared, (size_t)(h->D + 1) * h->ld));
  CR(h->mem.alloc(&h->d_Lblk, (size_t)((h->D + SBW - 1) / SBW) * SBW * SBW));
  CR(h->mem.alloc(&h->d_Ztiles, (size_t)((h->D + NB - 1) / NB) * NB * NB));
  CR(h->mem.alloc(&h->d_dxi, n9));
  CR(h->mem.alloc(&h->d_dX, 3 * N));
  CR(h->mem.alloc(&h->d_partials, h->n_partials));
  CR(h->mem.alloc(&h->d_cost, 2));
  CR(h->mem.alloc(&h->d_flag, 1));
  CR(h->mem.alloc(&h->d_bar, 1 + 4 * (size_t)((9 * m + SBW - 1) / SBW)));
  CRH(hipHostMalloc((void **)&h->h_cost, 4 * sizeof(double), hipHostMallocMapped));
  memset(h->h_cost, 0, 4 * sizeof(double));
  if (hipHostGetDevicePointer((void **)&h->d_mail, h->h_cost, 0) != hipSuccess) h->d_mail = nullptr;
  h->h_flag = reinterpret_cast<int *>(h->h_cost + 1);
  return MVBA_OK;
}

int upload_schur_index(mvba_handle *h, const SchurPlan &plan, SchurIndex &ix) {
  const int m = h->m;
  h->n_items = plan.L.T;
  h->n_items_offdiag = plan.L.T - plan.L.Tdiag;
  h->n_units = (int)ix.units.size();
  h->n_waves = ix.n_waves; h->slot_nR = ix.slot_nR; h->slot_nseg = ix.slot_nseg; h->n_slot_items = ix.n_slot_items;
  h->slot_w = ix.slot_w;
  h->index_on_device = ix.on_device;
  h->d_range_o0 = ix.d_range_o0;
  if (ix.on_device) { h->d_it_k = ix.d_it_k; h->d_it_l = ix.d_it_l; h->d_it_a = ix.d_it_a; h->d_seg_end = ix.d_seg_end; }
  const size_t P1 = (size_t)m * (m + 1) / 2 + 1;
  if (!ix.on_device) { CR(h->mem.alloc(&h->d_it_k, ix.it_k.size())); CR(h->mem.alloc(&h->d_it_l, ix.it_l.size())); CR(h->mem.alloc(&h->d_it_a, ix.it_a.size())); }
  CR(h->mem.alloc(&h->d_units, ix.units.size())); CR(h->mem.alloc(&h->d_unit_ptr, P1));
  CR(h->mem.alloc(&h->d_q_ptr, 9)); CR(h->mem.alloc(&h->d_q_units, ix.q_units.size()));
  CR(h->mem.alloc(&h->d_wdesc, ix.wdesc.size())); CR(h->mem.alloc(&h->d_wunits, ix.wunits.size()));
  if (!ix.on_device) CR(h->mem.alloc(&h->d_seg_end, ix.seg_end.size()));
  CR(h->mem.alloc(&h->d_prog, (size_t)h->slot_nR * std::max(1, h->slot_nseg) * PACE_STRIDE));
  if (!ix.seg_end.empty() && !ix.on_device) CRH(hipMemcpy(h->d_seg_end, ix.seg_end.data(), sizeof(int) * ix.seg_end.size(), hipMemcpyHostToDevice));
  if (!ix.wdesc.empty()) {
    CRH(hipMemcpy(h->d_wdesc, ix.wdesc.data(), sizeof(int4) * ix.wdesc.size(), hipMemcpyHostToDevice));
    CRH(hipMemcpy(h->d_wunits, ix.wunits.data(), sizeof(int) * ix.wunits.size(), hipMemcpyHostToDevice));
  }
  CR(h->mem.alloc(&h->d_partial, (size_t)UNIT_STRIDE * ix.units.size()));
  if (!ix.it_k.empty()) {
    CRH(hipMemcpy(h->d_it_k, ix.it_k.data(), sizeof(int) * ix.it_k.size(), hipMemcpyHostToDevice));
    CRH(hipMemcpy(h->d_it_l, ix.it_l.data(), sizeof(int) * ix.it_l.size(), hipMemcpyHostToDevice));
    CRH(hipMemcpy(h->d_it_a, ix.it_a.data(), sizeof(int) * ix.it_a.size(), hipMemcpyHostToDevice));
  }
  if (!ix.it_k.empty() || ix.on_device) {
    if (h->schur_mode == SCHUR_PAIRS) {
      std::vector<int4> qdesc(ix.units.size());
      for (size_t i = 0; i < ix.q_units.size(); ++i) qdesc[i] = ix.units[ix.q_units[i]];
      CRH(hipMemcpy(h->d_units, qdesc.data(), sizeof(int4) * qdesc.size(), hipMemcpyHostToDevice));
      int mx = 0;
      for (int x = 0; x < 8; ++x) mx = std::max(mx, ix.q_ptr[x + 1] - ix.q_ptr[x]);
      h->q_max = mx;
    }
    if (!ix.q_units.empty()) CRH(hipMemcpy(h->d_q_units, ix.q_units.data(), sizeof(int) * ix.q_units.size(), hipMemcpyHostToDevice));
  }
  if (h->schur_mode == SCHUR_SLOTS && h->n_slot_items) {
    const int W = h->slot_w, row = slot_idx_ints(W);
    const long long n_steps = h->n_slot_items / W;
    CR(h->mem.alloc(&h->d_it_x, (size_t)n_steps * row));
    hipLaunchKernelGGL(k_idx_interleave, dim3((unsigned)((n_steps * row + 255) / 256)), dim3(256), 0, h->stream, n_steps, W, row, h->d_it_k, h->d_it_l,
                       h->d_it_a, h->d_it_x);
    CRH(hipGetLastError());
    CRH(hipStreamSynchronize(h->stream));
    h->mem.release(h->d_it_k); h->mem.release(h->d_it_l); h->mem.release(h->d_it_a);
  }
  CRH(hipMemcpy(h->d_unit_ptr, ix.unit_ptr.data(), sizeof(int) * P1, hipMemcpyHostToDevice));
  CRH(hipMemcpy(h->d_q_ptr, ix.q_ptr.data(), sizeof(int) * 9, hipMemcpyHostToDevice));
  CRH(hipMemset(h->d_partial, 0, sizeof(double) * UNIT_STRIDE * std::max<size_t>(ix.units.size(), 1)));
  return MVBA_OK;
}

int upload_engine(mvba_handle *h, const mvba_problem *p, const std::vector<int> &obs_pt, const K1Tiles &t, const SchurPlan &plan, SchurIndex &ix) {
  const long long N = h->N, nobs = h->nobs;
  const int m = h->m;
  if (nobs) {
    CRH(hipMemcpy(h->d_obs_pt, obs_pt.data(), sizeof(int) * nobs, hipMemcpyHostToDevice));
    if (p->xy_layout == 1) {
      DevBufs tmp;
      double2 *planes = nullptr;
      CRH(hipMalloc((void **)&planes, sizeof(double2) * nobs));
      tmp.own(planes);
      hipError_t e = hipMemcpy(planes, p->xy, sizeof(double2) * nobs, hipMemcpyHostToDevice);
      if (e == hipSuccess) {
        hipLaunchKernelGGL(k_xy_from_planes, dim3((unsigned)((N + 255) / 256), m), dim3(256), 0, 0, planes, N, m, h->d_xy);
        e = hipGetLastError();
        if (e == hipSuccess) e = hipDeviceSynchronize();
      }
      CRH(e);
    } else {
      CRH(hipMemcpy(h->d_xy, p->xy, sizeof(double2) * nobs, hipMemcpyHostToDevice));
    }
  }
  CRH(hipMemcpy(h->d_tiles, t.tiles.data(), sizeof(int) * t.tiles.size(), hipMemcpyHostToDevice));
  CRH(hipMemset(h->d_PL, 0, sizeof(double) * 9 * std::max<long long>(N, 1)));
  CRH(hipMemset(h->d_flag, 0, sizeof(int)));
  if (h->schur_mode == SCHUR_DENSE) {
    const int T = (9 * m + 15) / 16;
    int n_cu_dense = 256;
    hipDeviceGetAttribute(&n_cu_dense, hipDeviceAttributeMultiprocessorCount, h->device);
    h->dense_tiles = T * (T + 1) / 2 + m;
    h->dense_blocks = (int)std::max<long long>(1, std::min<long long>((N + dense_ch(T) - 1) / dense_ch(T), (long long)n_cu_dense * dense_wgs(T)));
    CR(h->mem.alloc(&h->d_dense_part, (size_t)h->dense_blocks * h->dense_tiles * 256));
    if (!plan.dense_obs.empty()) {
      CR(h->mem.alloc(&h->d_dense_obs, plan.dense_obs.size()));
      CRH(hipMemcpy(h->d_dense_obs, plan.dense_obs.data(), sizeof(int) * plan.dense_obs.size(), hipMemcpyHostToDevice));
    }
  }
  if (h->use_pairs) CR(upload_schur_index(h, plan, ix));
  return MVBA_OK;
}

int set_kernel_attributes(mvba_handle *h, const CreateKnobs &knobs) {
  const int m = h->m;
  const bool robust = h->loss != LOSS_SQUARED;
  auto set_lds = [](const void *f, size_t bytes) { return hipFuncSetAttribute(f, hipFuncAttributeMaxDynamicSharedMemorySize, (int)bytes); };
  const size_t cam_lds = cam_lds_bytes(m, h->gcam, true);
  if (h->gcam) { CR(h->mem.alloc(&h->d_cam18, (size_t)m * CAM_LDS)); CR(h->mem.alloc(&h->d_dxi10, (size_t)m * DXI_LDS)); }
  for (int G : {2, 4, 8})
    for (int bt : {256, 512, 1024}) {
      CRH(set_lds(backsub_kernel(G, bt, false).fn(false), cam_lds));
      if (robust) CRH(set_lds(backsub_kernel(G, bt, false).fn(true), cam_lds));
    }
  CRH(set_lds((const void *)k_chol_super, SUPER_LDS));
  CRH(set_lds((const void *)k_chol_backsolve_all<true>, BACKSOLVE_LDS));
  {
    int per_cu = 0;
    CRH(hipDeviceGetAttribute(&h->n_cu, hipDeviceAttributeMultiprocessorCount, h->device));
    CRH(hipOccupancyMaxActiveBlocksPerMultiprocessor(&per_cu, (const void *)k_chol_backsolve_all<true>, SUPER_THREADS, BACKSOLVE_LDS));
    h->chol_onepass = per_cu >= 1 && !knobs.chol_launches;
    h->trail64_min = knobs.trail64_min;
    h->barrier_polls = knobs.barrier_polls;
  }
  const size_t k1_lds = k1_lds_bytes(m, h->gcam, h->k1_threads);
  CRH(set_lds(resid_jac_kernel(h->gcam, h->loss).fn(false), k1_lds));
  CRH(set_lds(cost_kernel(false, h->loss).fn(false), cam_lds));
  CRH(set_lds((const void *)k_residuals<false>, cam_lds));
  if (robust) {
    CRH(set_lds(resid_jac_kernel(h->gcam, h->loss).fn(true), k1_lds));
    CRH(set_lds(cost_kernel(false, h->loss).fn(true), cam_lds));
  }
  if (h->schur_mode == SCHUR_DENSE) {
    const int T = (9 * m + 15) / 16;
    CRH(set_lds(dense_kernel(T, h->d_dense_obs != nullptr).fn(robust), dense_lds_bytes(T, 16 * T / 9)));
  }
  return MVBA_OK;
}

int build_engine(mvba_handle *h, const mvba_problem *p, const CreateKnobs &knobs, const std::vector<int> &obs_pt, K1Tiles &tiles, CreateTimer &timer) {
  const long long N = h->N, nobs = h->nobs;
  const int m = h->m;
  if (p->device >= 0) CRH(hipSetDevice(p->device));
  CRH(hipGetDevice(&h->device));
  CRH(hipStreamCreateWithFlags(&h->stream, hipStreamNonBlocking));
  CR(h->mem.alloc(&h->d_pt_ptr, N + 1));
  CR(h->mem.alloc(&h->d_cam, nobs));
  CRH(hipMemcpy(h->d_pt_ptr, p->pt_ptr, sizeof(long long) * (N + 1), hipMemcpyHostToDevice));
  if (nobs) CRH(hipMemcpy(h->d_cam, p->cam_idx, sizeof(int) * nobs, hipMemcpyHostToDevice));
  timer.lap("device, topology upload");
  h->k1_threads = k1_block_threads(m, h->gcam);

  const bool dev_build = N > 0 && nobs > 0 && !knobs.index_host;
  const IndexInput in{p, N, nobs, (long long)m * (m + 1) / 2, m,
                      (int)std::max(1u, std::min({std::thread::hardware_concurrency(), 16u, (unsigned)m})), h->stream, h->d_pt_ptr, h->d_cam};
  DeviceIndexBuild dv;
  SchurPlan plan;
  SchurIndex ix;
  CR(decide_schur_form(in, knobs, h->loss, h->device, [&](std::vector<long long> &cnt) {
    return dev_build ? count_pairs_device(in, knobs, dv, cnt) : count_pairs_host(in, cnt);
  }, plan, timer));
  h->schur_mode = plan.mode;
  h->use_pairs = plan.mode != SCHUR_DENSE;
  if (h->use_pairs) CR(dev_build ? build_index_device(in, plan, dv, h->mem, ix, timer) : build_index_host(in, plan, h->mem, ix, timer));
  timer.lap("queues / wave descriptors");

  CR(alloc_engine_buffers(h, tiles));
  timer.lap("allocations");
  CR(upload_engine(h, p, obs_pt, tiles, plan, ix));
  timer.lap("uploads");
  CR(set_kernel_attributes(h, knobs));
  timer.lap("attributes");
  return MVBA_OK;
}

int create_engine(const mvba_problem *p, int loss, double loss_b, mvba_handle **out) {
  if (!p || !out) return fail(MVBA_ERR_BADARG, "null argument");
  const CreateKnobs knobs = read_create_knobs();
  CreateTimer timer{knobs.timing};
  std::vector<int> obs_pt;
  CR(validate_problem(p, obs_pt));
  timer.lap("validate, obs_pt");
  K1Tiles tiles = build_k1_tiles(p);
  timer.lap("K1 tiles");

  mvba_handle *h = new mvba_handle();
  const int m = p->n_images;
  h->N = p->n_points; h->nobs = p->n_obs; h->m = m; h->gauge_axis = p->gauge_axis; h->f0 = p->f0; h->D = 9 * m - 7; h->ld = (h->D + 3) & ~3;
  h->loss = loss; h->loss_b = loss_b;
  h->gcam = m > LDS_CAMERAS;
  h->force_big = knobs.force_big;
  h->check_solve = knobs.check_solve;
  h->check_solve_tol = knobs.check_solve_tol;
  if (int rc = build_engine(h, p, knobs, obs_pt, tiles, timer)) {
    const std::string err = g_err;
    mvba_destroy(h);
    g_err = err;
    return rc;
  }
  *out = h;
  return MVBA_OK;
}

#undef CR
#undef CRH
```

3d-reconstruction-from-multi-view-exp_amd/csrc/mvba_device.h:

```cpp

__device__ __forceinline__ double wave_sum(double v) {
#pragma unroll
  for (int off = 32; off > 0; off >>= 1) v += __shfl_down(v, off, 64);
  return v;
}

__device__ __forceinline__ double block_sum(double v, double *s_red ) {
  v = wave_sum(v);
  const int lane = threadIdx.x & 63, w = threadIdx.x >> 6;
  if (lane == 0) s_red[w] = v;
  __syncthreads();
  double t = 0.0;
  if (threadIdx.x == 0) {
    const int nw = (blockDim.x + 63) >> 6;
    for (int i = 0; i < nw; ++i) t += s_red[i];
  }
  return t;
}

__device__ __forceinline__ void load_cams_to_lds(const double *__restrict__ cam15, int m, double f0,
                                                 double *s_cam) {
  for (int k = threadIdx.x; k < m; k += blockDim.x) expand_cam(cam15 + (size_t)k * CAM_IN, f0, s_cam + k * CAM_LDS);
}

__host__ __device__ __forceinline__ size_t strip_offset(int k, int m) {
  return 81 * ((size_t)k * m - (size_t)k * (k - 1) / 2);
}

__device__ __forceinline__ int keep_index(int i, int gauge_axis) {
  if (i < 3) return i;
  return (i + 6 < 12 + gauge_axis) ? i + 6 : i + 7;
}

#define MVBA_CONST_AS __attribute__((address_space(4)))
template <typename T>
__device__ __forceinline__ const T MVBA_CONST_AS *as_const(const T *p) {
#pragma clang diagnostic push
#pragma clang diagnostic ignored "-Wold-style-cast"
  return (const T MVBA_CONST_AS *)p;
#pragma clang diagnostic pop
}

constexpr int REC = 8;
constexpr int LDS_CAMERAS = 646;

template <bool GCAM>
__device__ __forceinline__ const double *cam_row(const double *gcam, const double *s_cam, int k) {
  if constexpr (GCAM) return gcam + (size_t)k * CAM_LDS;
  else return s_cam + k * CAM_LDS;
}
template <bool GCAM>
__device__ __forceinline__ const double *dxi_row(const double *gdxi, const double *s_dxi, int k) {
  if constexpr (GCAM) return gdxi + (size_t)DXI_LDS * k;
  else return s_dxi + DXI_LDS * k;
}
template <bool GCAM>
__device__ __forceinline__ void stage_cams(const double *cam15, int m, double f0, double *s_cam) {
  if constexpr (!GCAM) {
    load_cams_to_lds(cam15, m, f0, s_cam);
    __syncthreads();
  }
}

struct LossArgs {
  double b;
  double *sqw;
};

constexpr int PBS = 16;
constexpr int PACE_STRIDE = 32;
```

3d-reconstruction-from-multi-view-exp_amd/csrc/mvba_host.h:

```cpp
#pragma once
#include <algorithm>
#include <cmath>
#include <cstddef>
#include <numeric>
#include <vector>

#include "mvba_common.h"

namespace mvba {

struct DevBufs {
  std::vector<void *> bufs;
  DevBufs() = default;
  DevBufs(const DevBufs &) = delete;
  DevBufs &operator=(const DevBufs &) = delete;
  ~DevBufs() { release_all(); }
  template <typename T>
  int alloc(T **p, size_t n) {
    const size_t bytes = std::max<size_t>(n, 1) * sizeof(T);
    const hipError_t e = hipMalloc((void **)p, bytes);
    if (e != hipSuccess) {
      size_t fr = 0, tot = 0;
      hipMemGetInfo(&fr, &tot);
      *p = nullptr;
      return fail(MVBA_ERR_HIP, std::string("hipMalloc of ") + std::to_string(bytes) + " bytes: " + hipGetErrorString(e) + " (" + std::to_string(fr >> 20) +
                                    " MiB free of " + std::to_string(tot >> 20) + ")");
    }
    bufs.push_back(*p);
    return MVBA_OK;
  }
  void own(void *q) { bufs.push_back(q); }
  bool forget(void *q) {
    auto it = std::find(bufs.begin(), bufs.end(), q);
    if (it == bufs.end()) return false;
    bufs.erase(it);
    return true;
  }
  template <typename T>
  void release(T *&p) {
    if (p && forget(p)) hipFree(p);
    p = nullptr;
  }
  template <typename T>
  void adopt(DevBufs &from, T *p) {
    if (p && from.forget(p)) bufs.push_back(p);
  }
  void release_all() {
    for (void *q : bufs) hipFree(q);
    bufs.clear();
  }
};

inline void descending_order(const double *v, size_t stride, int k, int *order) {
  std::iota(order, order + k, 0);
  std::sort(order, order + k, [&](int a, int b) { return v[(size_t)a * stride] > v[(size_t)b * stride]; });
}

struct Basis {
  std::vector<int> order;
  std::vector<double> sign;
};
inline int select_basis(const double *D, const double *V, int k, int n, int n_rank, Basis &b) {
  for (int i = 0; i < k; ++i)
    if (!std::isfinite(D[(size_t)i * k + i])) return fail(MVBA_ERR_SINGULAR, "SVD did not converge (non-finite values in the measurement matrix)");
  b.order.resize(k);
  descending_order(D, (size_t)k + 1, k, b.order.data());
  b.sign.resize(n_rank);
  for (int i = 0; i < n_rank; ++i) {
    const int col = b.order[i];
    int big = 0;
    for (int c = 1; c < n; ++c)
      if (std::fabs(V[(size_t)c * k + col]) > std::fabs(V[(size_t)big * k + col])) big = c;
    b.sign[i] = V[(size_t)big * k + col] < 0.0 ? -1.0 : 1.0;
  }
  return MVBA_OK;
}
inline double basis_at(const Basis &b, const double *V, int k, int c, int i) { return b.sign[i] * V[(size_t)c * k + b.order[i]]; }
inline void basis_block(const Basis &b, const double *V, int k, int n, int g0, int n_rank, double *Mg) {
  for (int c = 0; c < n; ++c)
    for (int i = 0; i < 4; ++i) Mg[(size_t)c * 4 + i] = g0 + i < n_rank ? basis_at(b, V, k, c, g0 + i) : 0.0;
}

constexpr int GT = 16;
constexpr int ROWS_PER_STEP = 32;
constexpr int GRAM_ROWS = 4 * ROWS_PER_STEP;
constexpr int WIDE_MIN = 64;
constexpr int JACOBI_MAX = 256;
constexpr int WB = 32;
constexpr int JW = 32;
constexpr int JACOBI_LDS_ORDER = 64;
constexpr int PC = 64;
constexpr int DG_ROWS_MAX = 128;
constexpr int FZ_MAXM = 10;
constexpr int DEPTH_MAX_IMAGES = 768;
constexpr size_t LDS_DEFAULT = 64 * 1024;
constexpr size_t JACOBI_LDS_MAX = 96 * 1024;
constexpr size_t ROTATE_LDS_MAX = 64 * 1024;
constexpr size_t PROJECT_LDS_MAX = 160 * 1024 - 64;
constexpr size_t DEPTH_LDS_MAX = 148 * 1024;
constexpr size_t TILE_MAX_BYTES = 120 * 1024;

inline int gram_mode(int n) { return n <= 16 ? 1 : (n <= 24 ? 2 : (n <= 32 ? 3 : 0)); }
inline int gram_tiles(int n) { return (n + GT - 1) / GT; }
inline int gram_pairs(int n) { return gram_mode(n) == 2 ? 2 : gram_tiles(n) * (gram_tiles(n) + 1) / 2; }
inline size_t gram_fused_lds(size_t el, int n) { return std::max<size_t>(el * GRAM_ROWS * n, (size_t)gram_pairs(n) * 8192); }
inline size_t gram_xz_lds(int m, bool rot) {
  return std::max<size_t>(sizeof(double) * (size_t)GRAM_ROWS * ((rot ? 2 : 1) * 3 * m + 2 * m), (size_t)gram_pairs(3 * m) * 8192);
}
inline size_t jacobi_lds(int n) {
  const int np = (n + 1) & ~1;
  if (n <= JW) return 0;
  return sizeof(double) * (3 * (np / 2) + 2) + 16 + (n <= JACOBI_LDS_ORDER ? sizeof(double) * 2 * (size_t)n * n : 0);
}
inline size_t rotate_rows_lds(size_t el, int n) { return (size_t)GRAM_ROWS * n * el; }
inline size_t project_lds(size_t el, int n) { return sizeof(double) * (5 * (size_t)n) + el * 4 * 64 * (size_t)(std::min(n, PC) | 1) + 16; }
inline size_t row_tile_lds(size_t el, int cols) { return el * 4 * 64 * (size_t)(cols | 1); }
inline bool tile_fits(size_t el, int cols) { return row_tile_lds(el, cols) <= TILE_MAX_BYTES; }
inline bool depth_tiled(size_t el, int m) { return tile_fits(el, 4 * m) && 24 * m * sizeof(double) <= 24 * 1024; }
inline size_t depth_primary_lds(size_t el, int m) { return sizeof(double) * 12 * m + row_tile_lds(el, 4 * m) + 16; }
inline size_t depth_primary_wide_lds(int m) { return sizeof(double) * (12 * (size_t)m + 4 * 64 * 14); }
inline size_t dual_apply_lds(size_t el, int m) { return sizeof(double) * 24 * m + row_tile_lds(el, 4 * m) + 16; }
inline size_t dual_apply_wide_lds(int m) { return sizeof(double) * 24 * m; }
inline int dual_gram_rows(int m) { return (int)std::max<size_t>(1, std::min<size_t>(DG_ROWS_MAX, DEPTH_LDS_MAX / (sizeof(double) * (size_t)(((3 * m) | 1) + 4)))); }
inline size_t dual_gram_lds(int m, int rows) { return sizeof(double) * ((size_t)rows * (((3 * m) | 1) + 4)); }
inline size_t dual_gram_mfma_lds(int m) {
  return sizeof(double) * (12 * (size_t)m + 4 * ((size_t)ROWS_PER_STEP * (4 * m + 4) + 4 * ((size_t)ROWS_PER_STEP * (m | 1) + 8)));
}

struct DepthScratch {
  double *Epart = nullptr, *Eout = nullptr, *G12 = nullptr, *V12 = nullptr, *colsum = nullptr, *w12 = nullptr, *own = nullptr;
  DepthScratch() = default;
  static size_t prefix(int blocks, int m) { return (size_t)blocks + 8 + (size_t)m * (144 + 144 + 12 + 12); }
  DepthScratch(double *ddep, int blocks, int m)
      : Epart(ddep), Eout(Epart + blocks), G12(Eout + 8), V12(G12 + (size_t)m * 144), colsum(V12 + (size_t)m * 144),
// ... 5 lines not shown
```

3d-reconstruction-from-multi-view-exp_amd/csrc/mvba_lanes.h:

```cpp
#pragma once

constexpr int LANES_W = 64;
constexpr int LANES_IDX = 3 * LANES_W;
constexpr int LANES_BUF = SchurStage<LANES_W, false, true>::SIZE;
constexpr int LANES_LDS = 3 * LANES_BUF + 2 * LANES_IDX * 4;
static_assert(LANES_BUF == 17408 && LANES_LDS == 53760, "the launch's LDS bytes");
static_assert(SchurStage<LANES_W, true, true>::SIZE <= LANES_BUF, "a diagonal step fits the buffer");
static_assert(3 * ((LANES_LDS + 511) / 512 * 512) <= 160 * 1024, "three waves per CU");

template <bool DIAG>
__device__ __forceinline__ void schur_lanes_run(char *wbuf, const int lane, const long long beg, const int nst,
                                                const int *__restrict__ it_x, const double2 *__restrict__ rec,
                                                const double *__restrict__ PB, const double c, const double cu,
                                                double *__restrict__ out, const int *__restrict__ slot_unit) {
  using S = SchurStage<LANES_W, DIAG, true>;
  constexpr int NPS = S::NPS, BUFSZ = S::SIZE, NBUF = 3;
  constexpr int G = DIAG ? 7 + 1 + 5 : 7 + 7 + 3;
  double acc[9][9];
#pragma unroll
  for (int i = 0; i < 9; ++i)
#pragma unroll
    for (int j = 0; j < 9; ++j) acc[i][j] = 0.0;
  double dg[9], rb[9];
#pragma unroll
  for (int j = 0; j < 9; ++j) dg[j] = rb[j] = 0.0;

  const unsigned lds0 = (unsigned)(unsigned long long)(__attribute__((address_space(3))) char *)wbuf;
  const unsigned ldsx0 = lds0 + NBUF * BUFSZ;
  const int *xring = reinterpret_cast<const int *>(wbuf + NBUF * BUFSZ);
  const int *xbase = it_x + beg * LANES_IDX;
  const int last_st = nst - 1;
  auto rec_row = [&](int j) { return (64 * j + lane) / 7; };
  auto rec_s16 = [&](int j) { return (unsigned)((64 * j + lane) % 7) << 4; };
  auto pb_row = [&](int j) { return (64 * j + lane) / NPS; };
  auto pb_s16 = [&](int j) { return (unsigned)((64 * j + lane) % NPS) << 4; };
  const unsigned lane16 = (unsigned)min(lane, 47) << 4;
  auto index_row = [&](int st, unsigned ring_off) {
    const int *src = xbase + (size_t)min(st, last_st) * LANES_IDX;
    const unsigned dst = ldsx0 + ring_off;
    if (lane < 48) lds_index_row(lane16, src, dst);
  };
  constexpr unsigned RING_B = LANES_IDX * 4;
  auto issue_step = [&](unsigned ring_off, unsigned ring_next, unsigned buf_off, int st_idx) {
    index_row(st_idx, ring_next);
    const int *x = reinterpret_cast<const int *>(reinterpret_cast<const char *>(xring) + ring_off);
    const unsigned buf = lds0 + buf_off;
    int kx[7], ax[NPS], lx[7];
#pragma unroll
    for (int j = 0; j < 7; ++j) kx[j] = x[rec_row(j)];
#pragma unroll
    for (int j = 0; j < NPS; ++j) ax[j] = x[2 * LANES_W + pb_row(j)];
#pragma unroll
    for (int j = 0; j < 7; ++j) lx[j] = DIAG ? (j == 0 ? x[lane] : 0) : x[LANES_W + rec_row(j)];
#pragma unroll
    for (int j = 0; j < 7; ++j) asm volatile("" : "+v"(kx[j]), "+v"(lx[j]));
#pragma unroll
    for (int j = 0; j < NPS; ++j) asm volatile("" : "+v"(ax[j]));
    if (!DIAG) {
#pragma unroll
      for (int j = 0; j < 7; ++j) {
        lds_gather16(kx[j], rec_s16(j), rec, buf + 1024 * j);
        lds_gather16(lx[j], rec_s16(j), rec, buf + S::L + 1024 * j);
      }
    } else {
#pragma unroll
      for (int j = 0; j < 7; ++j) lds_gather16(kx[j], rec_s16(j), rec, buf + 1024 * j);
      lds_gather16(lx[0], 7u << 4, rec, buf + S::L);
    }
#pragma unroll
    for (int j = 0; j < NPS; ++j) lds_gather16(ax[j], pb_s16(j), PB, buf + S::P + 1024 * j);
  };

  auto compute = [&](const char *buf) {
    const double2 *kr = reinterpret_cast<const double2 *>(buf + lane * PROW);
    const double2 *lr = DIAG ? kr : reinterpret_cast<const double2 *>(buf + S::L + lane * PROW);
    const double *pb = reinterpret_cast<const double *>(buf + S::P + lane * (16 * NPS));
    const double2 kx0 = kr[0], kx1 = kr[1], kx2 = kr[2];
    const double2 lx0 = lr[0], lx1 = lr[1], lx2 = lr[2];
    double t00, t01, t10, t11, w0, w1, wgt;
    schur_item<DIAG, true>(kx0, kx1, kx2, lx0, lx1, lx2, pb, buf, S::L, lane, t00, t01, t10, t11, w0, w1, wgt);
    const double2 lf = lr[3], lw0 = lr[4], lw1 = lr[5], lw2 = lr[6];
    const double sx[9] = {lf.x, 1.0, 0.0, lx0.x, lx1.x, lx2.x, lw0.x, lw1.x, lw2.x};
    const double sy[9] = {lf.y, 0.0, 1.0, lx0.y, lx1.y, lx2.y, lw0.y, lw1.y, lw2.y};
    double v0[9], v1[9];
#pragma unroll
    for (int j = 0; j < 9; ++j) {
      if (j == 1) { v0[j] = t00; v1[j] = t10; }
      else if (j == 2) { v0[j] = t01; v1[j] = t11; }
      else { v0[j] = t00 * sx[j] + t01 * sy[j]; v1[j] = t10 * sx[j] + t11 * sy[j]; }
      if (DIAG) {
        dg[j] = fma(wgt, sx[j] * sx[j] + sy[j] * sy[j], dg[j]);
        rb[j] += sx[j] * w0 + sy[j] * w1;
      }
    }
    const double2 kf = kr[3];
#pragma unroll
    for (int j = 0; j < 9; ++j) {
      acc[0][j] = fma(kf.y, v1[j], fma(kf.x, v0[j], acc[0][j]));
      acc[1][j] += v0[j];
      acc[2][j] += v1[j];
      acc[3][j] = fma(kx0.y, v1[j], fma(kx0.x, v0[j], acc[3][j]));
      acc[4][j] = fma(kx1.y, v1[j], fma(kx1.x, v0[j], acc[4][j]));
      acc[5][j] = fma(kx2.y, v1[j], fma(kx2.x, v0[j], acc[5][j]));
    }
    const double2 kw0 = kr[4], kw1 = kr[5], kw2 = kr[6];
#pragma unroll
    for (int j = 0; j < 9; ++j) {
      acc[6][j] = fma(kw0.y, v1[j], fma(kw0.x, v0[j], acc[6][j]));
      acc[7][j] = fma(kw1.y, v1[j], fma(kw1.x, v0[j], acc[7][j]));
      acc[8][j] = fma(kw2.y, v1[j], fma(kw2.x, v0[j], acc[8][j]));
    }
    lds_reads_done();
  };

  constexpr int SLOT_OPS = G;
  index_row(0, 0);
  asm volatile("s_waitcnt vmcnt(0)" ::: "memory");
  issue_step(0, RING_B, 0, 1);
  if (DIAG) asm volatile("s_waitcnt vmcnt(13)" ::: "memory");
  else asm volatile("s_waitcnt vmcnt(17)" ::: "memory");
  issue_step(RING_B, 0, BUFSZ, 2);
  unsigned b0 = 0, b1 = BUFSZ, b2 = 2 * BUFSZ, r0 = 0, r1 = RING_B;
  for (int st = 0; st < nst; ++st) {
    if (DIAG) asm volatile("s_waitcnt vmcnt(13)" ::: "memory");
    else asm volatile("s_waitcnt vmcnt(17)" ::: "memory");
    issue_step(r0, r1, b2, st + 3);
    compute(wbuf + b0);
    { const unsigned tb = b0, tr = r0; b0 = b1; b1 = b2; b2 = tb; r0 = r1; r1 = tr; }
  }
  static_assert(SLOT_OPS == (DIAG ? 13 : 17), "counted wait");
  asm volatile("s_waitcnt vmcnt(0)" ::: "memory");
  const int u = slot_unit[lane];
  if (u >= 0) {
    double *o = out + (size_t)u * UNIT_STRIDE;
#pragma unroll
    for (int i = 0; i < 9; ++i) {
      const double rs = jc_sign(i, cu);
#pragma unroll
      for (int j = 0; j < 9; ++j) {
        const double cs = jc_sign(j, cu);
        o[9 * i + j] = -4.0 * rs * cs * acc[i][j];
      }
    }
    if (DIAG) {
#pragma unroll
      for (int j = 0; j < 9; ++j) {
        const double cs = jc_sign(j, cu);
        o[81 + j] = 2.0 * c * cs * cs * dg[j];
        o[90 + j] = 2.0 * cs * rb[j];
      }
    }
  }
}
```

3d-reconstruction-from-multi-view-exp_amd/csrc/mvba_linearize.h:

```cpp

#define MVBA_RESID_JAC_ARGS                                                                                                 \
  long long nobs, int m, const double *__restrict__ cam15, const double *__restrict__ X, const int *__restrict__ obs_pt,   \
      const int *__restrict__ cam_idx, const double2 *__restrict__ xy, double f0, const int *__restrict__ tile_start,     \
      int n_tiles, double2 *__restrict__ rec, double *__restrict__ PL, const int *__restrict__ tile_slot,                 \
      double *__restrict__ PLsplit, const double *__restrict__ gcam
template <bool GCAM, int LOSS = LOSS_SQUARED, typename... Robust>
__global__ __launch_bounds__(1024, 4) void k_resid_jac(MVBA_RESID_JAC_ARGS, Robust... robust) {
  extern __shared__ __attribute__((aligned(16))) double smem[];
  double *s_cam = smem;
  const int lane = threadIdx.x & 63, wave = threadIdx.x >> 6, nwave = blockDim.x >> 6;
  double2 *stage = reinterpret_cast<double2 *>(smem + (GCAM ? 0 : ((m * CAM_LDS + 1) & ~1))) + wave * (64 * REC);
  constexpr int CS = 65;
  double *contrib = reinterpret_cast<double *>(stage);
  int *seg_start = reinterpret_cast<int *>(contrib + 9 * CS), *seg_pt = seg_start + 66;
  stage_cams<GCAM>(cam15, m, f0, s_cam);
  for (int tile = blockIdx.x * nwave + wave; tile < n_tiles; tile += gridDim.x * nwave) {
    const int ts0 = tile_start[tile], ts1 = tile_start[tile + 1];
    const bool split = ts0 < 0;
    const int slot = split ? as_const(tile_slot)[tile] : 0;
    const long long wbase = split ? ~ts0 : ts0;
    const int n = (int)((ts1 < 0 ? ~ts1 : ts1) - wbase);
    const long long o = wbase + lane;
    const bool live = lane < n;
    int a = -1;
    double c9[9] = {0, 0, 0, 0, 0, 0, 0, 0, 0};
    if (live) {
      a = obs_pt[o];
      const int k = cam_idx[o];
      const double2 z = xy[o];
      const double *Xa = X + 3 * (size_t)a;
      ObsJ J;
      obs_math(Xa[0], Xa[1], Xa[2], cam_row<GCAM>(gcam, s_cam, k), z.x, z.y, f0, J);
      if constexpr (LOSS != LOSS_SQUARED) {
        const LossArgs la = (robust, ...);
        const double sw = loss_sqrt_w<LOSS>(J.e0 * J.e0 + J.e1 * J.e1, la.b);
        J.e0 *= sw;
        J.e1 *= sw;
#pragma unroll
        for (int rr = 0; rr < 2; ++rr) {
#pragma unroll
          for (int i = 0; i < 3; ++i) J.jx[rr][i] *= sw;
          J.jc[rr][0] *= sw;
#pragma unroll
          for (int i = 6; i < 9; ++i) J.jc[rr][i] *= sw;
        }
        la.sqw[o] = sw;
      }
      double2 *row = stage + lane * REC;
      const int sw = lane & 7;
      row[0 ^ sw] = make_double2(J.jx[0][0], J.jx[1][0]);
      row[1 ^ sw] = make_double2(J.jx[0][1], J.jx[1][1]);
      row[2 ^ sw] = make_double2(J.jx[0][2], J.jx[1][2]);
      row[3 ^ sw] = make_double2(J.jc[0][0], J.jc[1][0]);
      row[4 ^ sw] = make_double2(J.jc[0][6], J.jc[1][6]);
      row[5 ^ sw] = make_double2(J.jc[0][7], J.jc[1][7]);
      row[6 ^ sw] = make_double2(J.jc[0][8], J.jc[1][8]);
      row[7 ^ sw] = make_double2(J.e0, J.e1);
      c9[0] = 2.0 * (J.jx[0][0] * J.jx[0][0] + J.jx[1][0] * J.jx[1][0]);
      c9[1] = 2.0 * (J.jx[0][0] * J.jx[0][1] + J.jx[1][0] * J.jx[1][1]);
      c9[2] = 2.0 * (J.jx[0][0] * J.jx[0][2] + J.jx[1][0] * J.jx[1][2]);
      c9[3] = 2.0 * (J.jx[0][1] * J.jx[0][1] + J.jx[1][1] * J.jx[1][1]);
      c9[4] = 2.0 * (J.jx[0][1] * J.jx[0][2] + J.jx[1][1] * J.jx[1][2]);
      c9[5] = 2.0 * (J.jx[0][2] * J.jx[0][2] + J.jx[1][2] * J.jx[1][2]);
      c9[6] = 2.0 * (J.jx[0][0] * J.e0 + J.jx[1][0] * J.e1);
      c9[7] = 2.0 * (J.jx[0][1] * J.e0 + J.jx[1][1] * J.e1);
      c9[8] = 2.0 * (J.jx[0][2] * J.e0 + J.jx[1][2] * J.e1);
    }
    wave_sync();
#pragma unroll
    for (int q = 0; q < REC; ++q) {
      const int ol = q * 8 + (lane >> 3), pos = lane & 7;
      const double2 v = stage[ol * REC + pos];
      if (ol < n) rec[(wbase + ol) * REC + (pos ^ (ol & 7))] = v;
    }
    wave_sync();
    const int a_prev = __shfl_up(a, 1, 64);
    const bool head = live && (lane == 0 || a != a_prev);
    const unsigned long long heads = __ballot(head);
    const int nseg = __popcll(heads);
#pragma unroll
    for (int q = 0; q < 9; ++q) contrib[q * CS + lane] = c9[q];
    if (head) {
      const int rank = __popcll(heads & ((1ull << lane) - 1ull));
      seg_start[rank] = lane;
      seg_pt[rank] = a;
    }
    if (lane == 0) seg_start[nseg] = n;
    wave_sync();
    const int sl = lane / 9, comp = lane - 9 * sl;
    for (int s0 = 0; s0 < nseg; s0 += 7) {
      const int sg = s0 + sl;
      if (sl < 7 && sg < nseg) {
        const int i0 = seg_start[sg], i1 = seg_start[sg + 1];
        double acc = 0.0;
        for (int i = i0; i < i1; ++i) acc += contrib[comp * CS + i];
        if (split) PLsplit[9 * (size_t)slot + comp] = acc;
        else PL[9 * (size_t)seg_pt[sg] + comp] = acc;
      }
    }
    wave_sync();
  }
}

__global__ void k_sum_split(int n_split, const int4 *__restrict__ splits ,
                            const double *__restrict__ PLsplit, double *__restrict__ PL) {
  const int t = blockIdx.x * blockDim.x + threadIdx.x, sp = t / 9, comp = t - 9 * sp;
  if (sp >= n_split) return;
  const int4 d = splits[sp];
  double v = 0.0;
  for (int q = 0; q < d.z; ++q) v += PLsplit[9 * (size_t)(d.y + q) + comp];
  PL[9 * (size_t)d.x + comp] = v;
}

template <typename... Held>
__global__ __launch_bounds__(256) void k_point_inv(long long npts, double c, const double *__restrict__ PL,
                                                   double *__restrict__ PB, int *__restrict__ flag,
                                                   double *__restrict__ Ab, long long nAb, int *__restrict__ prog, long long nprog, int want_r,
                                                   Held... held) {
  static_assert(sizeof...(Held) <= 1, "at most the held mask");
  __shared__ double2 s_out[256 * 8];
  double *s_in = reinterpret_cast<double *>(s_out);
  const long long a0 = (long long)blockIdx.x * 256, a = a0 + threadIdx.x;
  for (long long i = a; i < nAb; i += (long long)gridDim.x * blockDim.x) Ab[i] = 0.0;
  for (long long i = a; i < nprog; i += (long long)gridDim.x * blockDim.x) prog[i] = 0;
  if (a0 >= npts) return;
  const int np = (int)min<long long>(256, npts - a0);
  {
    double t[9];
#pragma unroll
    for (int i = 0; i < 9; ++i) t[i] = PL[9 * a0 + min((int)threadIdx.x + 256 * i, 9 * np - 1)];
#pragma unroll
    for (int i = 0; i < 9; ++i)
      if ((int)threadIdx.x + 256 * i < 9 * np) s_in[threadIdx.x + 256 * i] = t[i];
  }
  __syncthreads();
  double in[9];
#pragma unroll
  for (int i = 0; i < 9; ++i) in[i] = s_in[9 * min((int)threadIdx.x, np - 1) + i];
  __syncthreads();
  bool free_pt = threadIdx.x < np;
  if constexpr (sizeof...(Held) == 1) {
    if (free_pt && (held, ...)[a] != 0) {
      free_pt = false;
      double2 *out = s_out + 8 * threadIdx.x;
      const int sw = threadIdx.x & 7;
#pragma unroll
      for (int q = 0; q < 8; ++q) out[q ^ sw] = make_double2(0.0, q == 4 ? 1.0 : 0.0);
    }
  }
  if (free_pt) {
    const double s = 1.0 + c;
    const double xx = in[0] * s, xy = in[1], xz = in[2], yy = in[3] * s, yz = in[4], zz = in[5] * s;
    const double c00 = yy * zz - yz * yz, c01 = xz * yz - xy * zz, c02 = xy * yz - xz * yy;
    const double det = xx * c00 + xy * c01 + xz * c02;
    if (!(det != 0.0) || !isfinite(det)) atomicOr(flag, FLAG_POINT_SINGULAR);
    const double id = 1.0 / det;
    const double i00 = c00 * id, i01 = c01 * id, i02 = c02 * id;
    const double i11 = (xx * zz - xz * xz) * id, i12 = (xy * xz - xx * yz) * id, i22 = (xx * yy - xy * xy) * id;
    const double g0 = in[6], g1 = in[7], g2 = in[8];
    double2 *out = s_out + 8 * threadIdx.x;
    const int sw = threadIdx.x & 7;
    out[0 ^ sw] = make_double2(i00, i01);
    out[1 ^ sw] = make_double2(i02, i11);
    out[2 ^ sw] = make_double2(i12, i22);
    out[3 ^ sw] = make_double2(i00 * g0 + i01 * g1 + i02 * g2, i01 * g0 + i11 * g1 + i12 * g2);
    out[4 ^ sw] = make_double2(i02 * g0 + i12 * g1 + i22 * g2, 1.0);
    if (want_r) {
      const double d0 = i00, q0 = d0 != 0.0 ? 1.0 / d0 : 0.0, l10 = i01 * q0, l20 = i02 * q0;
      const double d1 = i11 - l10 * i01, q1 = d1 != 0.0 ? 1.0 / d1 : 0.0, l21 = (i12 - l20 * i01) * q1;
      const double d2 = i22 - l20 * i02 - l21 * l21 * d1;
      const double a0 = sqrt(fabs(d0)), a1 = sqrt(fabs(d1)), a2 = sqrt(fabs(d2));
      out[4 ^ sw].y = 1.0 + (d0 < 0.0 ? 1.0 : 0.0) + (d1 < 0.0 ? 2.0 : 0.0) + (d2 < 0.0 ? 4.0 : 0.0);
      out[5 ^ sw] = make_double2(a0, l10 * a0);
      out[6 ^ sw] = make_double2(l20 * a0, a1);
      out[7 ^ sw] = make_double2(l21 * a1, a2);
    } else {
      out[5 ^ sw] = out[6 ^ sw] = out[7 ^ sw] = make_double2(0.0, 0.0);
    }
  }
  __syncthreads();
  double2 *dst = reinterpret_cast<double2 *>(PB + PBS * a0);
  for (int e = threadIdx.x; e < 8 * np; e += 256) {
    const int p = e >> 3, sl = e & 7;
    dst[e] = s_out[8 * p + (sl ^ (p & 7))];
  }
}
```

3d-reconstruction-from-multi-view-exp_amd/csrc/mvba_schur.h:

```cpp


constexpr int PSTEP = 21;
constexpr int PROW = 7 * 16;
constexpr int UNIT_STRIDE = 104;
constexpr int SLOT_IDX = 64;
constexpr int SLOT_IDX_RING = 3;

template <int W, bool DIAG, bool PACKED>
struct SchurStage {
  static constexpr int NPS = DIAG ? 5 : 3;
  static constexpr int L = W * PROW;
  static constexpr int P = L + ((PACKED && DIAG) ? W * 16 : W * PROW);
  static constexpr int SIZE = P + W * 16 * (PACKED ? NPS : 5);
  static constexpr int SQW = DIAG ? L + W * 16 : P + W * 16 * NPS;
  static constexpr int SQW_END = SQW + (DIAG ? 1 : 2) * W * 8;
};
constexpr int PWAVE_LDS = SchurStage<PSTEP, false, false>::SIZE;
constexpr int SLOT_BUF = SchurStage<PSTEP, false, true>::SIZE;
constexpr int PAIRS_LDS = 2 * PWAVE_LDS;
constexpr int SLOT_LDS = 3 * SLOT_BUF + SLOT_IDX_RING * SLOT_IDX * 4;
static_assert(PWAVE_LDS == 6384 && SLOT_BUF == 5712 && SLOT_LDS == 17904, "the launches' LDS bytes");
static_assert(SchurStage<PSTEP, true, false>::SIZE == PWAVE_LDS && SchurStage<PSTEP, true, true>::SIZE <= SLOT_BUF, "a diagonal step fits the buffer");
static_assert(SchurStage<PSTEP, true, false>::SQW_END <= SchurStage<PSTEP, true, false>::P && SchurStage<PSTEP, false, false>::SQW_END <= PWAVE_LDS,
              "robust weights fit the staging buffer");
static_assert(9 * ((SLOT_LDS + 511) / 512 * 512) <= 160 * 1024, "nine waves per CU");

__device__ __forceinline__ void lds_dma16(const void *gsrc, void *lds_wave_uniform) {
  __builtin_amdgcn_global_load_lds(gsrc, (__attribute__((address_space(3))) void *)lds_wave_uniform, 16, 0, 0);
}
__device__ __forceinline__ void lds_gather16(int row, unsigned slot16, const void *base, unsigned lds) {
  unsigned o;
  asm volatile("s_mov_b32 m0, %4\n\tv_lshl_add_u32 %0, %1, 7, %2\n\tglobal_load_lds_dwordx4 %0, %3" : "=&v"(o) : "v"(row), "v"(slot16), "s"(base), "s"(lds) : "memory");
}
__device__ __forceinline__ void lds_index_row(unsigned lane16, const int *src, unsigned dst) {
  asm volatile("s_mov_b32 m0, %2\n\ts_nop 0\n\tglobal_load_lds_dwordx4 %0, %1" ::"v"(lane16), "s"(src), "s"(dst) : "memory");
}
__device__ __forceinline__ void lds_reads_done() { asm volatile("s_waitcnt lgkmcnt(0)" ::: "memory"); }

__device__ __forceinline__ constexpr double jc_sign(int i, double cu) { return (i == 1 || i == 2) ? cu : ((i >= 3 && i < 6) ? -1.0 : 1.0); }

template <bool DIAG, bool PADDED>
__device__ __forceinline__ void schur_item(const double2 kx0, const double2 kx1, const double2 kx2, const double2 lx0, const double2 lx1,
                                           const double2 lx2, const double *pb, const char *buf, const int l_off, const int row, double &t00, double &t01,
                                           double &t10, double &t11, double &w0, double &w1, double &wgt) {
  const double i00 = pb[0], i01 = pb[1], i02 = pb[2], i11 = pb[3], i12 = pb[4], i22 = pb[5];
  const double h0x = i00 * lx0.x + i01 * lx1.x + i02 * lx2.x, h0y = i00 * lx0.y + i01 * lx1.y + i02 * lx2.y;
  const double h1x = i01 * lx0.x + i11 * lx1.x + i12 * lx2.x, h1y = i01 * lx0.y + i11 * lx1.y + i12 * lx2.y;
  const double h2x = i02 * lx0.x + i12 * lx1.x + i22 * lx2.x, h2y = i02 * lx0.y + i12 * lx1.y + i22 * lx2.y;
  t00 = kx0.x * h0x + kx1.x * h1x + kx2.x * h2x, t01 = kx0.x * h0y + kx1.x * h1y + kx2.x * h2y;
  t10 = kx0.y * h0x + kx1.y * h1x + kx2.y * h2x, t11 = kx0.y * h0y + kx1.y * h1y + kx2.y * h2y;
  w0 = 0.0, w1 = 0.0;
  wgt = (DIAG && PADDED) ? pb[9] : 1.0;
  if (DIAG) {
    t00 -= PADDED ? 0.5 * wgt : 0.5;
    t11 -= PADDED ? 0.5 * wgt : 0.5;
    const double2 e = reinterpret_cast<const double2 *>(buf + l_off)[row];
    w0 = kx0.x * pb[6] + kx1.x * pb[7] + kx2.x * pb[8] - e.x;
    w1 = kx0.y * pb[6] + kx1.y * pb[7] + kx2.y * pb[8] - e.y;
    if (PADDED) {
      w0 *= wgt;
      w1 *= wgt;
    }
  }
}

template <class S, bool DIAG, bool PADDED, bool ROBUST>
__device__ __forceinline__ void schur_colgroup_step(const int it, const int sel0, const int sel1, const int sel2, const double al12,
                                                    const double bx1, const char *buf, const int ns,
                                                    double (&acc)[9][3], double (&dg)[3], double (&rb)[3]) {
  const char *kbuf = buf, *lbuf = buf + S::L, *pbuf = buf + S::P;
  if (it < ns) {
    double swk = 1.0, swl = 1.0;
    if (ROBUST) {
      const double *wl = reinterpret_cast<const double *>(buf + S::SQW);
      swk = wl[it];
      swl = DIAG ? swk : wl[PSTEP + it];
    }
    const double2 *kr = reinterpret_cast<const double2 *>(kbuf + it * PROW);
    const double2 *lr = DIAG ? kr : reinterpret_cast<const double2 *>(lbuf + it * PROW);
    const double *pb = reinterpret_cast<const double *>(pbuf + it * (16 * S::NPS));
    const double2 kx0 = kr[0], kx1 = kr[1], kx2 = kr[2], kf = kr[3], kw0 = kr[4], kw1 = kr[5], kw2 = kr[6];
    const double2 lx0 = lr[0], lx1 = lr[1], lx2 = lr[2];
    double t00, t01, t10, t11, w0, w1, wgt;
    schur_item<DIAG, PADDED>(kx0, kx1, kx2, lx0, lx1, lx2, pb, buf, S::L, it, t00, t01, t10, t11, w0, w1, wgt);
    const double2 s0v = lr[sel0], s1v = lr[sel1], s2v = lr[sel2];
    const double bxw = ROBUST ? bx1 * swl : bx1;
    const double sx[3] = {s0v.x, al12 * s1v.x + bxw, al12 * s2v.x};
    const double sy[3] = {s0v.y, al12 * s1v.y, al12 * s2v.y + bxw};
#pragma unroll
    for (int q = 0; q < 3; ++q) {
      const double v0 = t00 * sx[q] + t01 * sy[q], v1 = t10 * sx[q] + t11 * sy[q];
      acc[0][q] = fma(kf.y, v1, fma(kf.x, v0, acc[0][q]));
      if (ROBUST) {
        acc[1][q] = fma(swk, v0, acc[1][q]);
        acc[2][q] = fma(swk, v1, acc[2][q]);
// ... 297 lines not shown
  for (int st = 0; st < nst; ++st) {
    if (DIAG) asm volatile("s_waitcnt vmcnt(7)" ::: "memory");
    else asm volatile("s_waitcnt vmcnt(8)" ::: "memory");
    pace_at(st * PSTEP);
    issue_step(r2, b2);
    index_row(st + 4, r1);
    compute(wbuf + b0, PSTEP);
    { const unsigned tb = b0, tr = r0; b0 = b1; b1 = b2; b2 = tb; r0 = r1; r1 = r2; r2 = tr; }
  }
  static_assert(SLOT_OPS == (DIAG ? 7 : 8), "counted wait");
  asm volatile("s_waitcnt vmcnt(0)" ::: "memory");
  const double cs0 = cg == 1 ? -1.0 : 1.0, cs12 = cg == 0 ? cu : cs0;
  if (lane == 0)
    for (; seg < pace.nseg; ++seg) __hip_atomic_fetch_add(pace.prog + PACE_STRIDE * seg, 1, __ATOMIC_RELAXED, __HIP_MEMORY_SCOPE_AGENT);
  const int u = it < PSTEP ? slot_unit[it] : -1;
  if (u >= 0) {
    double *o = out + (size_t)u * UNIT_STRIDE;
#pragma unroll
    for (int i = 0; i < 9; ++i) {
      const double rs = jc_sign(i, cu);
#pragma unroll
      for (int q = 0; q < 3; ++q) o[9 * i + 3 * cg + q] = -4.0 * rs * (q == 0 ? cs0 : cs12) * acc[i][q];
    }
    if (DIAG) {
#pragma unroll
      for (int q = 0; q < 3; ++q) {
        const double cs = q == 0 ? cs0 : cs12;
        o[81 + 3 * cg + q] = 2.0 * c * cs * cs * dg[q];
        o[90 + 3 * cg + q] = 2.0 * cs * rb[q];
      }
    }
  }
}
__device__ __forceinline__ void schur_slots_wave(const int4 *__restrict__ wdesc, const int *__restrict__ wunits,
                                                 const int *__restrict__ it_k, const int *__restrict__ it_l,
                                                 const int *__restrict__ it_a, const double2 *__restrict__ rec,
                                                 const double *__restrict__ PB, double c, double f0,
                                                 double *__restrict__ partial, int nR, const int *__restrict__ seg_end,
                                                 int *__restrict__ prog, int nseg, int lag,
                                                 const long long *__restrict__ range_o0) {
  extern __shared__ char smem_pairs[];
  const int bid = blockIdx.x;
  const int MVBA_CONST_AS *dp = as_const(reinterpret_cast<const int *>(wdesc)) + 4 * (size_t)bid;
  const int d_x = dp[0], d_y = dp[1], nsteps = dp[2], flags = dp[3];
  if (nsteps <= 0) return;
  const long long beg = ((long long)d_y << 32) | (unsigned)d_x;
  const int *su = wunits + (size_t)bid * PSTEP;
  const int r = bid % nR, live = (flags >> 8) & 0xfff;
  const double2 *rec_r = rec + (size_t)as_const(range_o0)[r] * REC;
  const SlotPace pace{seg_end + (size_t)bid * nseg, prog + (size_t)r * nseg * PACE_STRIDE, live, nseg, lag};
  if (flags & 1)
    schur_slots_run<true>(smem_pairs, (int)threadIdx.x, beg, nsteps, it_k, rec_r, PB, c, 1.0 / f0, partial, su, pace);
  else
    schur_slots_run<false>(smem_pairs, (int)threadIdx.x, beg, nsteps, it_k, rec_r, PB, c, 1.0 / f0, partial, su, pace);
}
#define MVBA_SLOTS_ARGS                                                                                                  \
  const int4 *__restrict__ wdesc, const int *__restrict__ wunits, const int *__restrict__ it_k, const int *__restrict__ it_l, \
      const int *__restrict__ it_a, const double2 *__restrict__ rec, const double *__restrict__ PB, double c, double f0,  \
      double *__restrict__ partial, int nR, const int *__restrict__ seg_end, int *__restrict__ prog,                      \
      int nseg, int lag, const long long *__restrict__ range_o0
__global__ __launch_bounds__(64, 3) void k_schur_slots(MVBA_SLOTS_ARGS) {
  schur_slots_wave(wdesc, wunits, it_k, it_l, it_a, rec, PB, c, f0, partial, nR, seg_end, prog, nseg, lag, range_o0);
}

#include "mvba_lanes.h"
constexpr int slot_idx_ints(int W) { return W == LANES_W ? LANES_IDX : SLOT_IDX; }

__global__ __launch_bounds__(64, 1) void k_schur_lanes(const int4 *__restrict__ wdesc, const int *__restrict__ wunits,
                                                       const int *__restrict__ it_x, const double2 *__restrict__ rec,
                                                       const double *__restrict__ PB, double c, double f0,
                                                       double *__restrict__ partial, int nR,
                                                       const long long *__restrict__ range_o0) {
  extern __shared__ char smem_pairs[];
  const int bid = blockIdx.x;
  const int MVBA_CONST_AS *dp = as_const(reinterpret_cast<const int *>(wdesc)) + 4 * (size_t)bid;
  const int d_x = dp[0], d_y = dp[1], nsteps = dp[2], flags = dp[3];
  if (nsteps <= 0) return;
  const long long beg = ((long long)d_y << 32) | (unsigned)d_x;
  const int *su = wunits + (size_t)bid * LANES_W;
  const double2 *rec_r = rec + (size_t)as_const(range_o0)[bid % nR] * REC;
  if (flags & 1) schur_lanes_run<true>(smem_pairs, (int)threadIdx.x, beg, nsteps, it_x, rec_r, PB, c, 1.0 / f0, partial, su);
  else schur_lanes_run<false>(smem_pairs, (int)threadIdx.x, beg, nsteps, it_x, rec_r, PB, c, 1.0 / f0, partial, su);
}

__global__ __launch_bounds__(128) void k_schur_reduce(int m, const int *__restrict__ unit_ptr,
                                                      const double *__restrict__ partial, double *__restrict__ Afull,
                                                      double *__restrict__ bfull) {
  const long long p = blockIdx.x;
  int k = (int)((2.0 * m + 1.0 - sqrt((2.0 * m + 1.0) * (2.0 * m + 1.0) - 8.0 * (double)p)) * 0.5);
  while ((long long)k * m - (long long)k * (k - 1) / 2 > p) --k;
  while ((long long)(k + 1) * m - (long long)(k + 1) * k / 2 <= p) ++k;
  const int l = k + (int)(p - ((long long)k * m - (long long)k * (k - 1) / 2));
  const int u0 = unit_ptr[p], u1 = unit_ptr[p + 1];
  const int e = threadIdx.x;
  if (e >= (k == l ? 99 : 81)) return;
  auto ordered_sum = [&](int off) {
    double v = 0.0;
    int uu = u0;
    for (; uu + 8 <= u1; uu += 8) {
      double t[8];
#pragma unroll
      for (int q = 0; q < 8; ++q) t[q] = partial[(size_t)(uu + q) * UNIT_STRIDE + off];
#pragma unroll
      for (int q = 0; q < 8; ++q) v += t[q];
    }
    for (; uu < u1; ++uu) v += partial[(size_t)uu * UNIT_STRIDE + off];
    return v;
  };
  const double v = ordered_sum(e);
  double *Ak = Afull + strip_offset(k, m);
  const int Wk = 9 * (m - k);
  if (e < 81) {
    const int i = e / 9, j = e - 9 * i;
    const double d = (k == l && i == j) ? ordered_sum(81 + i) : 0.0;
    Ak[(size_t)i * Wk + 9 * (l - k) + j] = v + d;
  } else if (e >= 90) {
    bfull[9 * k + (e - 90)] = v;
  }
}
```

3d-reconstruction-from-multi-view-exp_amd/lib/_mvba.py:

```python
from __future__ import annotations

import ctypes as C
import os
import threading

import numpy as np

_HERE = os.path.dirname(os.path.abspath(__file__))
LIB_PATH = os.environ.get("MVBA_LIBRARY", os.path.join(os.path.dirname(_HERE), "libmvba.so"))

MVBA_OK, MVBA_ERR_BADARG, MVBA_ERR_SINGULAR, MVBA_ERR_HIP, MVBA_ERR_RCCL, MVBA_ERR_STATE = range(6)

KERNEL_IDS = ("resid_jac", "point_blocks", "point_inv", "schur", "allreduce", "solve", "backsub_cost", "cost")
BUF = {"residual": 0, "JX": 1, "JC": 2, "E": 3, "dP": 4, "A_full": 5, "b_full": 6, "dxi": 7, "dX": 8,
       "trial_X": 9, "trial_cam": 10, "index_k": 11, "index_l": 12, "index_a": 13, "index_seg": 14, "weight": 15}
LOSSES = {"squared": 0, "huber": 1, "cauchy": 2}


def check_loss(loss, loss_scale):
    if not isinstance(loss, str) or loss not in LOSSES:
        raise ValueError(f"loss must be one of {sorted(LOSSES)}, got {loss!r}")
    if loss == "squared":
        return 0, 0.0
    if loss_scale is None:
# ... 298 lines not shown
        self.n_solves += 1
        return E.value

    def commit(self):
        raise_for(self.lib.mvba_commit(self._h), self.lib)

    def set_parameter_map(self, col, n_free=None):
        if col is None:
            raise_for(self.lib.mvba_set_parameter_map(self._h, None, 0), self.lib)
            self.n_free = 9 * self.m - 7
            return
        col = _as(col, np.int32).reshape(-1)
        if col.shape != (9 * self.m,):
            raise ValueError(f"col must have 9 n_images = {9 * self.m} entries, got {col.shape[0]}")
        if n_free is None:
            n_free = int(col.max()) + 1 if col.size else 0
        raise_for(self.lib.mvba_set_parameter_map(self._h, col.ctypes.data_as(C.POINTER(C.c_int32)), int(n_free)), self.lib)
        self.n_free = int(n_free)

    def set_point_hold(self, mask):
        if mask is None:
            raise_for(self.lib.mvba_set_point_hold(self._h, None), self.lib)
            self.n_held_points = 0
            return
        mask = np.asarray(mask)
        if mask.dtype != np.bool_ or mask.shape != (self.n,):
            raise ValueError(f"mask must be a bool array of shape ({self.n},), got {mask.dtype} {mask.shape}")
        m8 = _as(mask, np.uint8)
        raise_for(self.lib.mvba_set_point_hold(self._h, m8.ctypes.data_as(C.POINTER(C.c_uint8))), self.lib)
        self.n_held_points = int(mask.sum())

    def covariance(self, points=True, cameras=True, full=False):
        P = np.empty((self.n, 6)) if points else None
        Cc = np.empty((self.m, 9, 9)) if cameras else None
        Cf = np.empty((9 * self.m, 9 * self.m)) if full else None
        tm = np.zeros(4)
        raise_for(self.lib.mvba_covariance(self._h, _ptr(P) if P is not None else None, _ptr(Cc) if Cc is not None else None,
                                           _ptr(Cf) if Cf is not None else None, _ptr(tm)), self.lib)
        out = {"timings_ms": dict(zip(("schur", "factor", "inverse", "points"), tm.tolist()))}
        if P is not None:
            i = np.array([[0, 1, 2], [1, 3, 4], [2, 4, 5]])
            out["points"] = P[:, i]
        if Cc is not None:
            out["cameras"] = Cc
        if Cf is not None:
            out["cameras_full"] = Cf
        return out

    def triangulate(self, n_refine=2):
        q = np.empty((self.n, 3))
        st = np.empty(self.n, np.int32)
        tm = np.zeros(3)
        raise_for(self.lib.mvba_triangulate_state(self._h, int(n_refine), _ptr(q), st.ctypes.data_as(C.POINTER(C.c_int32)), _ptr(tm)),
                  self.lib)
        return q, st, _timings3(tm)

    def residuals(self):
        e = np.empty((self.n_obs, 2))
        raise_for(self.lib.mvba_residuals(self._h, _ptr(e)), self.lib)
        return e

    def set_profiling(self, on):
        raise_for(self.lib.mvba_set_profiling(self._h, 2 if on == 2 and on is not True else int(bool(on))), self.lib)

    def reset_stats(self):
        raise_for(self.lib.mvba_reset_stats(self._h), self.lib)

    def stats(self):
        s = Stats()
        raise_for(self.lib.mvba_get_stats(self._h, C.byref(s)), self.lib)
        out = {k: {"ms": s.ms[i], "launches": s.launches[i]} for i, k in enumerate(KERNEL_IDS)}
        out["counts"] = {"linearize": s.n_linearize, "try_step": s.n_try_step, "commit": s.n_commit,
                         "lu_fallback": s.n_lu_fallback, "barrier_fallback": s.n_barrier_fallback}
        return out

    def _info(self):
        out = (C.c_int64 * 8)()
        raise_for(self.lib.mvba_get_info(self._h, out), self.lib)
        return list(out)

    def schur_info(self):
        i = self._info()
        return {"items": i[0], "offdiag_items": i[1], "units": i[2], "kernel": ("strip", "pairs", "slots", "dense")[i[3] & 0xff],
                "slot_rows": i[7], "step_width": (i[3] >> 8) & 0xff}

    def rccl_version(self):
        i = self._info()
        return {"loaded": i[4], "compiled_against": i[5], "ranks": i[6]}

    def comm_init(self, id128: bytes, rank: int, n_ranks: int):
        buf = C.create_string_buffer(bytes(id128), 128)
        raise_for(self.lib.mvba_comm_init(self._h, buf, int(rank), int(n_ranks)), self.lib)

    def comm_init_host(self, rank: int, n_ranks: int, allreduce):
        HOSTFN = C.CFUNCTYPE(C.c_int, C.c_void_p, _dp, C.c_int64)

        def _cb(_user, buf, n):
            try:
                allreduce(np.ctypeslib.as_array(buf, shape=(n,)))
                return 0
            except Exception:
                return 1

        self._host_cb = HOSTFN(_cb)
        raise_for(self.lib.mvba_comm_init_host(self._h, int(rank), int(n_ranks), C.cast(self._host_cb, C.c_void_p), None),
                  self.lib)

    def debug_read(self, name):
        n = C.c_int64()
        raise_for(self.lib.mvba_debug_read(self._h, BUF[name], None, 0, C.byref(n)), self.lib)
        out = np.empty(n.value)
        raise_for(self.lib.mvba_debug_read(self._h, BUF[name], _ptr(out), n.value, C.byref(n)), self.lib)
        return out


def comm_unique_id() -> bytes:
    lib = load_library()
    buf = C.create_string_buffer(128)
    raise_for(lib.mvba_comm_unique_id(buf), lib)
    return buf.raw


def project(X, K, R, t, pt_ptr=None, cam_idx=None, device=-1):
    lib = load_library()
    _require_device("mvba_project")
    X, K, R, t = (_as(v, np.float64) for v in (X, K, R, t))
    n, m = X.shape[0], K.shape[0]
    assert X.shape == (n, 3) and K.shape == (m, 3, 3) and R.shape == (m, 3, 3) and t.shape == (m, 3)
    _, n_obs, pp, cp, _ = _obs_list(pt_ptr, cam_idx, None, m, n if pt_ptr is None else None)
    out = np.empty((n, m, 2) if pt_ptr is None else (n_obs, 2))
    raise_for(lib.mvba_project(_ptr(X), n, _ptr(K), _ptr(R), _ptr(t), m, pp, cp, n_obs, _ptr(out), int(device)), lib)
    return out


def triangulate(K, R, t, pt_ptr, cam_idx, xy, n_refine=2, device=-1):
    lib = load_library()
    _require_device("mvba_triangulate")
    K, R, t, xy = (_as(v, np.float64) for v in (K, R, t, xy))
    m = K.shape[0]
    assert K.shape == (m, 3, 3) and R.shape == (m, 3, 3) and t.shape == (m, 3)
    n, n_obs, pp, cp, xy = _obs_list(pt_ptr, cam_idx, xy, m)
    X, q, st, tm = np.empty((n, 3)), np.empty((n, 3)), np.empty(n, np.int32), np.zeros(3)
    raise_for(lib.mvba_triangulate(_ptr(K), _ptr(R), _ptr(t), m, n, pp, cp, _ptr(xy), n_obs, int(n_refine), _ptr(X), _ptr(q),
                                   st.ctypes.data_as(C.POINTER(C.c_int32)), _ptr(tm), int(device)), lib)
    return X, q, st, _timings3(tm)


def resect(X, pt_ptr, cam_idx, xy, n_images, point_ok=None, device=-1):
    lib = load_library()
    _require_device("mvba_resect")
    X, xy = _as(X, np.float64), _as(xy, np.float64)
    n, m = X.shape[0], int(n_images)
    assert X.shape == (n, 3)
    _, n_obs, pp, cp, xy = _obs_list(pt_ptr, cam_idx, xy, m, n)
    ok, okp = _point_ok_ptr(point_ok, n)
    P, q, st, tm = np.empty((m, 3, 4)), np.empty((m, 2)), np.empty(m, np.int32), np.zeros(3)
    raise_for(lib.mvba_resect(_ptr(X), n, pp, cp, _ptr(xy), n_obs, m, okp, _ptr(P), _ptr(q), st.ctypes.data_as(C.POINTER(C.c_int32)),
                              _ptr(tm), int(device)), lib)
    return P, q, st, _timings3(tm)


def covisibility(pt_ptr, cam_idx, n_images, n_points=None, device=-1):
    lib = load_library()
    _require_device("mvba_covisibility")
    m = int(n_images)
    n, n_obs, pp, cp, _ = _obs_list(pt_ptr, cam_idx, None, m, n_points)
    count, tm = np.zeros((max(m, 0), max(m, 0)), np.int64), np.zeros(3)
# ... 474 lines not shown
```

Measured before the change: 432.0.

## Store compact per-observation Jacobian records and rebuild rotation columns in Schur kernel

Each observation's stored record shrinks from 8 to 4 double2 slots. The residual moves to a separate array, and the three rotation Jacobian columns are no longer stored: the new lanes Schur kernel rebuilds them as cross products of the point Jacobian with (X - t), using point coordinates packed into the PB record and camera translations. This cuts the bytes the linearize kernel writes and the Schur kernel gathers per observation, at the cost of extra arithmetic, an extra residual gather, and a second full-record pass when point covariance is requested. It applies only with squared loss, the lanes slot width and no GCAM, and can be turned off with MVBA_REC=full.

```diff
diff --git a/3d-reconstruction-from-multi-view-exp_amd/csrc/check_isa.py b/3d-reconstruction-from-multi-view-exp_amd/csrc/check_isa.py
--- a/3d-reconstruction-from-multi-view-exp_amd/csrc/check_isa.py
+++ b/3d-reconstruction-from-multi-view-exp_amd/csrc/check_isa.py
@@ -3,7 +3,8 @@
 import sys
 
 KERNELS = {"k_schur_slots": (("vmcnt(7)", 7), ("vmcnt(8)", 8)),
-           "k_schur_lanes": (("vmcnt(13)", 14), ("vmcnt(17)", 18))}
+           "k_schur_lanes": (("vmcnt(13)", 14), ("vmcnt(17)", 18)),
+           "k_schur_lanes_compact": (("vmcnt(12)", 13), ("vmcnt(13)", 14))}
 SLOTS_ONLY = "k_schur_slots"
 VM_LOOP_OPS = ("global_load_lds_dwordx4", "global_load_lds_dword ")
 
diff --git a/3d-reconstruction-from-multi-view-exp_amd/csrc/host_check.cpp b/3d-reconstruction-from-multi-view-exp_amd/csrc/host_check.cpp
--- a/3d-reconstruction-from-multi-view-exp_amd/csrc/host_check.cpp
+++ b/3d-reconstruction-from-multi-view-exp_amd/csrc/host_check.cpp
@@ -488,6 +488,28 @@
     CHECK(run(2, huge, desc, 32, twice, 2, 0.8, mp, kpp, d2, counts) == MVBA_ERR_BADARG && g_err == "Q = 2147483648 queries up to pair 1: the sum over the pairs must be < 2^31");
     CHECK(run(2, huge, desc, 32, twice, 1, 0.8, mp, kpp, d2, counts) == MVBA_OK && Q == (1LL << 30));
   }
+  {
+    const double f0 = 600.0, th = 0.3;
+    const double cam[CAM_IN] = {1.1 * f0, 7.0, -5.0, 0.4, -0.2, -3.0, cos(th), 0.0, sin(th), 0.0, 1.0, 0.0, -sin(th), 0.0, cos(th)};
+    alignas(16) double c18[CAM_LDS];
+    expand_cam(cam, f0, c18);
+    const double X[3] = {0.7, -0.4, 2.5};
+    ObsJ J;
+    obs_math(X[0], X[1], X[2], c18, 31.0, -12.0, f0, J);
+    double c8[8], e2[2] = {J.e0, J.e1}, full[16];
+    for (int i = 0; i < 3; ++i) { c8[2 * i] = J.jx[0][i]; c8[2 * i + 1] = J.jx[1][i]; }
+    c8[6] = J.jc[0][0]; c8[7] = J.jc[1][0];
+    expand_compact_record(c8, e2, X, cam + 3, full);
+    for (int i = 0; i < 8; ++i) CHECK(full[i] == c8[i]);
+    CHECK(full[14] == J.e0 && full[15] == J.e1);
+    double big = 0.0;
+    for (int rr = 0; rr < 2; ++rr) for (int i = 6; i < 9; ++i) big = std::max(big, std::fabs(J.jc[rr][i]));
+    CHECK(big > 0.0);
+    for (int rr = 0; rr < 2; ++rr) for (int i = 0; i < 3; ++i) CHECK(std::fabs(full[8 + 2 * i + rr] - J.jc[rr][6 + i]) <= 1e-14 * big);
+    const double jx[8] = {1.0, 0.0, 0.0, 1.0, 0.0, 0.0, 0.0, 0.0}, zero[3] = {0.0, 0.0, 0.0}, d[3] = {2.0, 3.0, 5.0};
+    expand_compact_record(jx, e2, d, zero, full);
+    CHECK(full[8] == 0.0 && full[10] == -5.0 && full[12] == 3.0 && full[9] == 5.0 && full[11] == 0.0 && full[13] == -2.0);
+  }
   if (failures) return 1;
   std::printf("host_check ok\n");
   return 0;
diff --git a/3d-reconstruction-from-multi-view-exp_amd/csrc/mvba.hip b/3d-reconstruction-from-multi-view-exp_amd/csrc/mvba.hip
--- a/3d-reconstruction-from-multi-view-exp_amd/csrc/mvba.hip
+++ b/3d-reconstruction-from-multi-view-exp_amd/csrc/mvba.hip
@@ -134,6 +134,8 @@
   int cur = 0;
   bool have_params = false, linearized = false, have_trial = false;
   double2 *d_rec = nullptr;
+  bool rec_compact = false;
+  double2 *d_res = nullptr, *d_rec_full = nullptr;
   double *d_PL = nullptr, *d_PB = nullptr;
   double *d_Ab = nullptr, *d_Ared = nullptr, *d_Ztiles = nullptr, *d_Lblk = nullptr, *d_dxi = nullptr, *d_dX = nullptr, *d_lu = nullptr;
   int *d_ipiv = nullptr;
@@ -388,6 +390,7 @@
   bool schur_slots = false, schur_lanes = false, schur_pairs = false, schur_dense = false;
   bool index_host = false, index_global = false;
   bool force_big = false;
+  bool rec_full = false;
   bool chol_launches = false;
   int trail64_min = 200;
   unsigned barrier_polls = 1u << 22;
@@ -409,6 +412,7 @@
   k.index_host = is(index, "host");
   k.index_global = is(index, "global");
   k.force_big = getenv("MVBA_FORCE_BIG") != nullptr;
+  k.rec_full = is(getenv("MVBA_REC"), "full");
   k.chol_launches = is(getenv("MVBA_CHOL"), "launches");
   if (const char *ev = getenv("MVBA_TRAIL64_MIN")) k.trail64_min = std::max(0, atoi(ev));
   if (const char *ev = getenv("MVBA_CHOL_BARRIER_POLLS")) k.barrier_polls = (unsigned)std::max(0LL, atoll(ev));
@@ -548,13 +552,18 @@
 }
 
 namespace {
-void launch_resid_jac(mvba_handle *h) {
+void launch_resid_jac(mvba_handle *h, double2 *full_rec = nullptr) {
   const int kt = h->k1_threads;
   cam_tables(h, h->d_cam15[h->cur], nullptr);
   const int wpb = kt / 64;
   const int grid = std::max(1, std::min(2048 * 256 / kt, (h->n_tiles + wpb - 1) / wpb));
+  if (h->rec_compact && !full_rec)
+    hipLaunchKernelGGL((k_resid_jac<false, LOSS_SQUARED, CompactRec>), dim3(grid), dim3(kt), k1_lds_bytes(h->m, false, kt), h->stream, h->nobs, h->m,
+                       h->d_cam15[h->cur], h->d_X[h->cur], h->d_obs_pt, h->d_cam, h->d_xy, h->f0, h->d_tiles, h->n_tiles, h->d_rec, h->d_PL,
+                       h->d_tile_slot, h->d_PLsplit, h->d_cam18, CompactRec{h->d_res});
+  else
   launch_loss(h, resid_jac_kernel(h->gcam, h->loss), dim3(grid), dim3(kt), k1_lds_bytes(h->m, h->gcam, kt), h->nobs, h->m, h->d_cam15[h->cur],
-              h->d_X[h->cur], h->d_obs_pt, h->d_cam, h->d_xy, h->f0, h->d_tiles, h->n_tiles, h->d_rec, h->d_PL,
+              h->d_X[h->cur], h->d_obs_pt, h->d_cam, h->d_xy, h->f0, h->d_tiles, h->n_tiles, full_rec ? full_rec : h->d_rec, h->d_PL,
               h->d_tile_slot, h->d_PLsplit, h->d_cam18);
   if (h->n_splits)
     hipLaunchKernelGGL(k_sum_split, dim3((9 * h->n_splits + 255) / 256), dim3(256), 0, h->stream, h->n_splits, h->d_splits,
@@ -568,12 +577,13 @@
   const unsigned grid = (unsigned)std::max<long long>((h->N + 255) / 256, std::min<long long>((nAb + 1023) / 1024, 4096));
   const long long nprog = h->slot_w == LANES_W ? 0 : (long long)h->slot_nR * h->slot_nseg * PACE_STRIDE;
   const int want_r = h->schur_mode == SCHUR_DENSE ? 1 : 0;
+  const double *Xc = h->rec_compact ? h->d_X[h->cur] : nullptr;
   if (h->n_held)
     hipLaunchKernelGGL(k_point_inv<const uint8_t *>, dim3(std::max(grid, 1u)), dim3(256), 0, h->stream, h->N, c, h->d_PL, h->d_PB, h->d_flag,
-                       h->d_Ab, nAb, h->d_prog, nprog, want_r, (const uint8_t *)h->d_held);
+                       h->d_Ab, nAb, h->d_prog, nprog, want_r, Xc, (const uint8_t *)h->d_held);
   else
     hipLaunchKernelGGL(k_point_inv<>, dim3(std::max(grid, 1u)), dim3(256), 0, h->stream, h->N, c, h->d_PL, h->d_PB, h->d_flag,
-                       h->d_Ab, nAb, h->d_prog, nprog, want_r);
+                       h->d_Ab, nAb, h->d_prog, nprog, want_r, Xc);
 }
 
 void launch_schur(mvba_handle *h, double c) {
@@ -583,7 +593,10 @@
   if (h->use_pairs) {
     const bool big = (std::max<long long>(h->nobs, h->N) + 1) * 128LL >= (1LL << 32) || h->force_big;
     if (h->schur_mode == SCHUR_SLOTS && h->slot_w == LANES_W) {
-      if (h->n_waves)
+      if (h->n_waves && h->rec_compact)
+        hipLaunchKernelGGL(k_schur_lanes_compact, dim3(h->n_waves), dim3(64), LANES_LDS_C, h->stream, h->d_wdesc, h->d_wunits, h->d_it_x, h->d_rec,
+                           h->d_PB, c, h->f0, h->d_partial, h->slot_nR, h->d_range_o0, h->d_res, h->d_units, h->d_cam15[h->cur]);
+      else if (h->n_waves)
         hipLaunchKernelGGL(k_schur_lanes, dim3(h->n_waves), dim3(64), LANES_LDS, h->stream, h->d_wdesc, h->d_wunits, h->d_it_x, h->d_rec, h->d_PB, c,
                            h->f0, h->d_partial, h->slot_nR, h->d_range_o0);
     } else if (h->schur_mode == SCHUR_SLOTS) {
@@ -1041,12 +1054,14 @@
     if (!local_rc && hipEventCreate(&e) != hipSuccess) local_rc = fail(MVBA_ERR_HIP, "hipEventCreate failed");
   const int mv = (D + 6) / 9 + 1;
   if (!local_rc && h->mapped && D > 0 && !h->d_cov_sigv) local_rc = h->mem.alloc(&h->d_cov_sigv, n_sig);
+  if (!local_rc && h->rec_compact && point_cov && h->nobs && !h->d_rec_full) local_rc = h->mem.alloc(&h->d_rec_full, (size_t)REC * h->nobs);
   const bool sharded = h->comm || h->host_ar;
   if (local_rc && !sharded) return local_rc;
   const std::string local_err = local_rc ? g_err : std::string();
   double *d_b = h->d_Ab + strip_offset(m, m);
   if (!local_rc) {
     MVBA_HIP(hipEventRecord(ev[0], h->stream));
+    if (h->nobs && h->rec_compact && point_cov) launch_resid_jac(h, h->d_rec_full);
     if (h->nobs) launch_resid_jac(h);
     h->linearized = true; h->have_trial = false;
     launch_point_inv(h, 0.0);
@@ -1098,7 +1113,7 @@
     const unsigned grid = (unsigned)std::min<long long>(8192, (h->N * G + 255) / 256);
     auto launch = [&](auto kern, auto... held) {
       hipLaunchKernelGGL(kern, dim3(grid), dim3(256), 0, h->stream, h->N, m, (const long long *)h->d_pt_ptr, (const int *)h->d_cam,
-                         (const double2 *)h->d_rec, (const double *)h->d_PL, (const double *)h->d_cov_sig, 1.0 / h->f0, h->d_cov_pts,
+                         (const double2 *)(h->rec_compact ? h->d_rec_full : h->d_rec), (const double *)h->d_PL, (const double *)h->d_cov_sig, 1.0 / h->f0, h->d_cov_pts,
                          h->d_flag, held...);
     };
     if (h->n_held) {
@@ -1227,7 +1242,7 @@
   out8[0] = h->n_items;
   out8[1] = h->n_items_offdiag;
   out8[2] = h->n_units;
-  out8[3] = h->schur_mode | (h->schur_mode == SCHUR_SLOTS ? h->slot_w << 8 : 0);
+  out8[3] = h->schur_mode | (h->schur_mode == SCHUR_SLOTS ? h->slot_w << 8 : 0) | (h->rec_compact ? 1 << 16 : 0);
   out8[4] = h->rccl_version;
   out8[5] = NCCL_VERSION_CODE;
   out8[6] = h->nranks;
@@ -1309,6 +1324,19 @@
   auto d2h = [&](const void *src, size_t bytes) { return hipMemcpy(out, src, bytes, hipMemcpyDeviceToHost); };
   if (which == MVBA_BUF_RESIDUAL || which == MVBA_BUF_JX || which == MVBA_BUF_JC) {
     std::vector<double> r((size_t)2 * REC * h->nobs);
+    if (h->rec_compact) {
+      const size_t no = (size_t)h->nobs;
+      std::vector<double> c8(2 * REC_C * no), e2(2 * no), X(3 * (size_t)h->N), cam((size_t)CAM_IN * h->m);
+      std::vector<int> pt(no), ck(no);
+      MVBA_HIP(hipMemcpy(c8.data(), h->d_rec, sizeof(double) * c8.size(), hipMemcpyDeviceToHost));
+      MVBA_HIP(hipMemcpy(e2.data(), h->d_res, sizeof(double) * e2.size(), hipMemcpyDeviceToHost));
+      MVBA_HIP(hipMemcpy(X.data(), h->d_X[h->cur], sizeof(double) * X.size(), hipMemcpyDeviceToHost));
+      MVBA_HIP(hipMemcpy(cam.data(), h->d_cam15[h->cur], sizeof(double) * cam.size(), hipMemcpyDeviceToHost));
+      MVBA_HIP(hipMemcpy(pt.data(), h->d_obs_pt, sizeof(int) * no, hipMemcpyDeviceToHost));
+      MVBA_HIP(hipMemcpy(ck.data(), h->d_cam, sizeof(int) * no, hipMemcpyDeviceToHost));
+      for (size_t o = 0; o < no; ++o)
+        expand_compact_record(&c8[2 * REC_C * o], &e2[2 * o], &X[3 * (size_t)pt[o]], &cam[(size_t)CAM_IN * ck[o] + 3], &r[2 * REC * o]);
+    } else
     MVBA_HIP(hipMemcpy(r.data(), h->d_rec, sizeof(double) * r.size(), hipMemcpyDeviceToHost));
     std::vector<double> sw;
     if (h->loss != LOSS_SQUARED && which == MVBA_BUF_JC) {
diff --git a/3d-reconstruction-from-multi-view-exp_amd/csrc/mvba_create.h b/3d-reconstruction-from-multi-view-exp_amd/csrc/mvba_create.h
--- a/3d-reconstruction-from-multi-view-exp_amd/csrc/mvba_create.h
+++ b/3d-reconstruction-from-multi-view-exp_amd/csrc/mvba_create.h
@@ -650,14 +650,19 @@
   }
   CR(h->mem.alloc(&h->d_tiles, t.tiles.size()));
   for (int i = 0; i < 2; ++i) { CR(h->mem.alloc(&h->d_X[i], 3 * N)); CR(h->mem.alloc(&h->d_cam15[i], (size_t)CAM_IN * m)); }
-  CR(h->mem.alloc(&h->d_rec, (size_t)REC * (nobs + 1)));
+  const int rec_slots = h->rec_compact ? REC_C : REC;
+  CR(h->mem.alloc(&h->d_rec, (size_t)rec_slots * (nobs + 1)));
+  if (h->rec_compact) {
+    CR(h->mem.alloc(&h->d_res, (size_t)nobs + 1));
+    CRH(hipMemset(h->d_res + nobs, 0, sizeof(double2)));
+  }
   if (h->loss != LOSS_SQUARED) {
     CR(h->mem.alloc(&h->d_sqw, nobs + 1));
     CRH(hipMemset(h->d_sqw, 0, sizeof(double) * (nobs + 1)));
   }
   CR(h->mem.alloc(&h->d_PL, 9 * N));
   CR(h->mem.alloc(&h->d_PB, (size_t)PBS * (N + 1)));
-  CRH(hipMemset(h->d_rec + (size_t)REC * nobs, 0, sizeof(double2) * REC));
+  CRH(hipMemset(h->d_rec + (size_t)rec_slots * nobs, 0, sizeof(double2) * rec_slots));
   CRH(hipMemset(h->d_PB + (size_t)PBS * N, 0, sizeof(double) * PBS));
   const size_t n9 = 9 * (size_t)m;
   CR(h->mem.alloc(&h->d_Ab, strip_offset(m, m) + n9));
@@ -716,6 +721,7 @@
     }
     if (!ix.q_units.empty()) CRH(hipMemcpy(h->d_q_units, ix.q_units.data(), sizeof(int) * ix.q_units.size(), hipMemcpyHostToDevice));
   }
+  if (h->rec_compact && !ix.units.empty()) CRH(hipMemcpy(h->d_units, ix.units.data(), sizeof(int4) * ix.units.size(), hipMemcpyHostToDevice));
   if (h->schur_mode == SCHUR_SLOTS && h->n_slot_items) {
     const int W = h->slot_w, row = slot_idx_ints(W);
     const long long n_steps = h->n_slot_items / W;
@@ -795,6 +801,7 @@
   }
   const size_t k1_lds = k1_lds_bytes(m, h->gcam, h->k1_threads);
   CRH(set_lds(resid_jac_kernel(h->gcam, h->loss).fn(false), k1_lds));
+  if (h->rec_compact) CRH(set_lds((const void *)k_resid_jac<false, LOSS_SQUARED, CompactRec>, k1_lds));
   CRH(set_lds(cost_kernel(false, h->loss).fn(false), cam_lds));
   CRH(set_lds((const void *)k_residuals<false>, cam_lds));
   if (robust) {
@@ -832,6 +839,7 @@
   }, plan, timer));
   h->schur_mode = plan.mode;
   h->use_pairs = plan.mode != SCHUR_DENSE;
+  h->rec_compact = plan.mode == SCHUR_SLOTS && plan.W == LANES_W && h->loss == LOSS_SQUARED && !h->gcam && !knobs.rec_full;
   if (h->use_pairs) CR(dev_build ? build_index_device(in, plan, dv, h->mem, ix, timer) : build_index_host(in, plan, h->mem, ix, timer));
   timer.lap("queues / wave descriptors");
 
diff --git a/3d-reconstruction-from-multi-view-exp_amd/csrc/mvba_device.h b/3d-reconstruction-from-multi-view-exp_amd/csrc/mvba_device.h
--- a/3d-reconstruction-from-multi-view-exp_amd/csrc/mvba_device.h
+++ b/3d-reconstruction-from-multi-view-exp_amd/csrc/mvba_device.h
@@ -42,6 +42,14 @@
 }
 
 constexpr int REC = 8;
+constexpr int REC_C = 4;
+struct CompactRec {
+  double2 *res;
+};
+template <typename... T>
+struct is_compact_rec { static constexpr bool value = false; };
+template <>
+struct is_compact_rec<CompactRec> { static constexpr bool value = true; };
 constexpr int LDS_CAMERAS = 646;
 
 template <bool GCAM>
diff --git a/3d-reconstruction-from-multi-view-exp_amd/csrc/mvba_host.h b/3d-reconstruction-from-multi-view-exp_amd/csrc/mvba_host.h
--- a/3d-reconstruction-from-multi-view-exp_amd/csrc/mvba_host.h
+++ b/3d-reconstruction-from-multi-view-exp_amd/csrc/mvba_host.h
@@ -50,6 +50,17 @@
     bufs.clear();
   }
 };
+
+inline void expand_compact_record(const double *c8, const double *e2, const double *X3, const double *t3, double *full16) {
+  for (int i = 0; i < 8; ++i) full16[i] = c8[i];
+  const double d[3] = {X3[0] - t3[0], X3[1] - t3[1], X3[2] - t3[2]};
+  for (int i = 0; i < 3; ++i) {
+    const int i1 = (i + 1) % 3, i2 = (i + 2) % 3;
+    for (int rr = 0; rr < 2; ++rr) full16[8 + 2 * i + rr] = c8[2 * i1 + rr] * d[i2] - c8[2 * i2 + rr] * d[i1];
+  }
+  full16[14] = e2[0];
+  full16[15] = e2[1];
+}
 
 inline void descending_order(const double *v, size_t stride, int k, int *order) {
   std::iota(order, order + k, 0);
diff --git a/3d-reconstruction-from-multi-view-exp_amd/csrc/mvba_lanes.h b/3d-reconstruction-from-multi-view-exp_amd/csrc/mvba_lanes.h
--- a/3d-reconstruction-from-multi-view-exp_amd/csrc/mvba_lanes.h
+++ b/3d-reconstruction-from-multi-view-exp_amd/csrc/mvba_lanes.h
@@ -7,15 +7,39 @@
 static_assert(LANES_BUF == 17408 && LANES_LDS == 53760, "the launch's LDS bytes");
 static_assert(SchurStage<LANES_W, true, true>::SIZE <= LANES_BUF, "a diagonal step fits the buffer");
 static_assert(3 * ((LANES_LDS + 511) / 512 * 512) <= 160 * 1024, "three waves per CU");
-
-template <bool DIAG>
+constexpr int LANES_BUF_C = SchurStage<LANES_W, false, true, true>::SIZE;
+constexpr int LANES_LDS_C = 3 * LANES_BUF_C + 2 * LANES_IDX * 4;
+static_assert(LANES_BUF_C == 13312 && LANES_LDS_C == 41472, "the compact launch's LDS bytes");
+static_assert(SchurStage<LANES_W, true, true, true>::SIZE == 12288, "a compact diagonal step fits the buffer");
+static_assert(3 * ((LANES_LDS_C + 511) / 512 * 512) <= 160 * 1024 && 4 * ((LANES_LDS_C + 511) / 512 * 512) > 160 * 1024, "three waves per CU");
+
+struct LanesCompact {
+  const double2 *res = nullptr;
+  const int4 *units = nullptr;
+  const double *cam15 = nullptr;
+};
+template <int SH>
+__device__ __forceinline__ void lds_gather16_rows(int row, unsigned slot16, const void *base, unsigned lds) {
+  unsigned o;
+  asm volatile("s_mov_b32 m0, %4\n\tv_lshl_add_u32 %0, %1, %5, %2\n\tglobal_load_lds_dwordx4 %0, %3" : "=&v"(o) : "v"(row), "v"(slot16), "s"(base), "s"(lds), "i"(SH) : "memory");
+}
+template <int G>
+__device__ __forceinline__ void lanes_wait() {
+  static_assert(G == 12 || G == 13 || G == 17, "the loops of k_schur_lanes and k_schur_lanes_compact");
+  if (G == 12) asm volatile("s_waitcnt vmcnt(12)" ::: "memory");
+  else if (G == 13) asm volatile("s_waitcnt vmcnt(13)" ::: "memory");
+  else asm volatile("s_waitcnt vmcnt(17)" ::: "memory");
+}
+
+template <bool DIAG, bool COMPACT = false>
 __device__ __forceinline__ void schur_lanes_run(char *wbuf, const int lane, const long long beg, const int nst,
                                                 const int *__restrict__ it_x, const double2 *__restrict__ rec,
                                                 const double *__restrict__ PB, const double c, const double cu,
-                                                double *__restrict__ out, const int *__restrict__ slot_unit) {
-  using S = SchurStage<LANES_W, DIAG, true>;
+                                                double *__restrict__ out, const int *__restrict__ slot_unit, const LanesCompact cx = {}) {
+  using S = SchurStage<LANES_W, DIAG, true, COMPACT>;
   constexpr int NPS = S::NPS, BUFSZ = S::SIZE, NBUF = 3;
-  constexpr int G = DIAG ? 7 + 1 + 5 : 7 + 7 + 3;
+  constexpr int RSL = COMPACT ? 4 : 7;
+  constexpr int G = DIAG ? RSL + 1 + NPS : RSL + RSL + NPS;
   double acc[9][9];
 #pragma unroll
   for (int i = 0; i < 9; ++i)
@@ -30,10 +54,10 @@
   const int *xring = reinterpret_cast<const int *>(wbuf + NBUF * BUFSZ);
   const int *xbase = it_x + beg * LANES_IDX;
   const int last_st = nst - 1;
-  auto rec_row = [&](int j) { return (64 * j + lane) / 7; };
-  auto rec_s16 = [&](int j) { return (unsigned)((64 * j + lane) % 7) << 4; };
+  auto rec_row = [&](int j) { return (64 * j + lane) / RSL; };
+  auto rec_s16 = [&](int j) { return COMPACT ? (unsigned)((lane & 3) ^ ((lane >> 4) & 3)) << 4 : (unsigned)((64 * j + lane) % 7) << 4; };
   auto pb_row = [&](int j) { return (64 * j + lane) / NPS; };
-  auto pb_s16 = [&](int j) { return (unsigned)((64 * j + lane) % NPS) << 4; };
+  auto pb_s16 = [&](int j) { return (unsigned)(COMPACT ? ((64 * j + lane) % NPS + 6) & 7 : (64 * j + lane) % NPS) << 4; };
   const unsigned lane16 = (unsigned)min(lane, 47) << 4;
   auto index_row = [&](int st, unsigned ring_off) {
     const int *src = xbase + (size_t)min(st, last_st) * LANES_IDX;
@@ -45,18 +69,25 @@
     index_row(st_idx, ring_next);
     const int *x = reinterpret_cast<const int *>(reinterpret_cast<const char *>(xring) + ring_off);
     const unsigned buf = lds0 + buf_off;
-    int kx[7], ax[NPS], lx[7];
-#pragma unroll
-    for (int j = 0; j < 7; ++j) kx[j] = x[rec_row(j)];
+    int kx[RSL], ax[NPS], lx[RSL];
+#pragma unroll
+    for (int j = 0; j < RSL; ++j) kx[j] = x[rec_row(j)];
 #pragma unroll
     for (int j = 0; j < NPS; ++j) ax[j] = x[2 * LANES_W + pb_row(j)];
 #pragma unroll
-    for (int j = 0; j < 7; ++j) lx[j] = DIAG ? (j == 0 ? x[lane] : 0) : x[LANES_W + rec_row(j)];
-#pragma unroll
-    for (int j = 0; j < 7; ++j) asm volatile("" : "+v"(kx[j]), "+v"(lx[j]));
+    for (int j = 0; j < RSL; ++j) lx[j] = DIAG ? (j == 0 ? x[lane] : 0) : x[LANES_W + rec_row(j)];
+#pragma unroll
+    for (int j = 0; j < RSL; ++j) asm volatile("" : "+v"(kx[j]), "+v"(lx[j]));
 #pragma unroll
     for (int j = 0; j < NPS; ++j) asm volatile("" : "+v"(ax[j]));
-    if (!DIAG) {
+    if constexpr (COMPACT) {
+#pragma unroll
+      for (int j = 0; j < RSL; ++j) {
+        lds_gather16_rows<6>(kx[j], rec_s16(j), rec, buf + 1024 * j);
+        if (!DIAG) lds_gather16_rows<6>(lx[j], rec_s16(j), rec, buf + S::L + 1024 * j);
+      }
+      if (DIAG) lds_gather16_rows<4>(lx[0], 0u, cx.res, buf + S::L);
+    } else if (!DIAG) {
 #pragma unroll
       for (int j = 0; j < 7; ++j) {
         lds_gather16(kx[j], rec_s16(j), rec, buf + 1024 * j);
@@ -71,15 +102,38 @@
     for (int j = 0; j < NPS; ++j) lds_gather16(ax[j], pb_s16(j), PB, buf + S::P + 1024 * j);
   };
 
+  int unit = -1;
+  double tk[3] = {0.0, 0.0, 0.0}, tl[3] = {0.0, 0.0, 0.0};
+  if constexpr (COMPACT) {
+    unit = slot_unit[lane];
+    if (unit >= 0) {
+      const int kl = cx.units[unit].w;
+      const double *ck = cx.cam15 + (size_t)((unsigned)kl >> 16) * CAM_IN + 3, *cl = cx.cam15 + (size_t)(kl & 0xffff) * CAM_IN + 3;
+#pragma unroll
+      for (int i = 0; i < 3; ++i) { tk[i] = ck[i]; tl[i] = DIAG ? tk[i] : cl[i]; }
+    }
+  }
+
   auto compute = [&](const char *buf) {
-    const double2 *kr = reinterpret_cast<const double2 *>(buf + lane * PROW);
-    const double2 *lr = DIAG ? kr : reinterpret_cast<const double2 *>(buf + S::L + lane * PROW);
-    const double *pb = reinterpret_cast<const double *>(buf + S::P + lane * (16 * NPS));
-    const double2 kx0 = kr[0], kx1 = kr[1], kx2 = kr[2];
-    const double2 lx0 = lr[0], lx1 = lr[1], lx2 = lr[2];
+    const double2 *kr = reinterpret_cast<const double2 *>(buf + lane * S::ROW);
+    const double2 *lr = DIAG ? kr : reinterpret_cast<const double2 *>(buf + S::L + lane * S::ROW);
+    const double *prow = reinterpret_cast<const double *>(buf + S::P + lane * (16 * NPS));
+    const double *pb = COMPACT ? prow + 4 : prow;
+    const int sw = COMPACT ? (lane >> 2) & 3 : 0;
+    const double2 kx0 = kr[0 ^ sw], kx1 = kr[1 ^ sw], kx2 = kr[2 ^ sw];
+    const double2 lx0 = lr[0 ^ sw], lx1 = lr[1 ^ sw], lx2 = lr[2 ^ sw];
     double t00, t01, t10, t11, w0, w1, wgt;
     schur_item<DIAG, true>(kx0, kx1, kx2, lx0, lx1, lx2, pb, buf, S::L, lane, t00, t01, t10, t11, w0, w1, wgt);
-    const double2 lf = lr[3], lw0 = lr[4], lw1 = lr[5], lw2 = lr[6];
+    auto omega = [&](const double2 j0, const double2 j1, const double2 j2, const double (&t)[3], double2 &o0, double2 &o1, double2 &o2) {
+      const double d0 = prow[0] - t[0], d1 = prow[1] - t[1], d2 = prow[2] - t[2];
+      o0 = make_double2(j1.x * d2 - j2.x * d1, j1.y * d2 - j2.y * d1);
+      o1 = make_double2(j2.x * d0 - j0.x * d2, j2.y * d0 - j0.y * d2);
+      o2 = make_double2(j0.x * d1 - j1.x * d0, j0.y * d1 - j1.y * d0);
+    };
+    const double2 lf = lr[3 ^ sw];
+    double2 lw0, lw1, lw2;
+    if constexpr (COMPACT) omega(lx0, lx1, lx2, tl, lw0, lw1, lw2);
+    else { lw0 = lr[4]; lw1 = lr[5]; lw2 = lr[6]; }
     const double sx[9] = {lf.x, 1.0, 0.0, lx0.x, lx1.x, lx2.x, lw0.x, lw1.x, lw2.x};
     const double sy[9] = {lf.y, 0.0, 1.0, lx0.y, lx1.y, lx2.y, lw0.y, lw1.y, lw2.y};
     double v0[9], v1[9];
@@ -93,7 +147,7 @@
         rb[j] += sx[j] * w0 + sy[j] * w1;
       }
     }
-    const double2 kf = kr[3];
+    const double2 kf = kr[3 ^ sw];
 #pragma unroll
     for (int j = 0; j < 9; ++j) {
       acc[0][j] = fma(kf.y, v1[j], fma(kf.x, v0[j], acc[0][j]));
@@ -103,7 +157,11 @@
       acc[4][j] = fma(kx1.y, v1[j], fma(kx1.x, v0[j], acc[4][j]));
       acc[5][j] = fma(kx2.y, v1[j], fma(kx2.x, v0[j], acc[5][j]));
     }
-    const double2 kw0 = kr[4], kw1 = kr[5], kw2 = kr[6];
+    double2 kw0, kw1, kw2;
+    if constexpr (COMPACT) {
+      if (DIAG) { kw0 = lw0; kw1 = lw1; kw2 = lw2; }
+      else omega(kx0, kx1, kx2, tk, kw0, kw1, kw2);
+    } else { kw0 = kr[4]; kw1 = kr[5]; kw2 = kr[6]; }
 #pragma unroll
     for (int j = 0; j < 9; ++j) {
       acc[6][j] = fma(kw0.y, v1[j], fma(kw0.x, v0[j], acc[6][j]));
@@ -116,21 +174,23 @@
   constexpr int SLOT_OPS = G;
   index_row(0, 0);
   asm volatile("s_waitcnt vmcnt(0)" ::: "memory");
+  if constexpr (COMPACT) {
+#pragma unroll
+    for (int i = 0; i < 3; ++i) asm volatile("" : "+v"(tk[i]), "+v"(tl[i]));
+  }
   issue_step(0, RING_B, 0, 1);
-  if (DIAG) asm volatile("s_waitcnt vmcnt(13)" ::: "memory");
-  else asm volatile("s_waitcnt vmcnt(17)" ::: "memory");
+  lanes_wait<G>();
   issue_step(RING_B, 0, BUFSZ, 2);
   unsigned b0 = 0, b1 = BUFSZ, b2 = 2 * BUFSZ, r0 = 0, r1 = RING_B;
   for (int st = 0; st < nst; ++st) {
-    if (DIAG) asm volatile("s_waitcnt vmcnt(13)" ::: "memory");
-    else asm volatile("s_waitcnt vmcnt(17)" ::: "memory");
+    lanes_wait<G>();
     issue_step(r0, r1, b2, st + 3);
     compute(wbuf + b0);
     { const unsigned tb = b0, tr = r0; b0 = b1; b1 = b2; b2 = tb; r0 = r1; r1 = tr; }
   }
-  static_assert(SLOT_OPS == (DIAG ? 13 : 17), "counted wait");
+  static_assert(SLOT_OPS == (COMPACT ? (DIAG ? 12 : 13) : (DIAG ? 13 : 17)), "counted wait");
   asm volatile("s_waitcnt vmcnt(0)" ::: "memory");
-  const int u = slot_unit[lane];
+  const int u = COMPACT ? unit : slot_unit[lane];
   if (u >= 0) {
     double *o = out + (size_t)u * UNIT_STRIDE;
 #pragma unroll
diff --git a/3d-reconstruction-from-multi-view-exp_amd/csrc/mvba_linearize.h b/3d-reconstruction-from-multi-view-exp_amd/csrc/mvba_linearize.h
--- a/3d-reconstruction-from-multi-view-exp_amd/csrc/mvba_linearize.h
+++ b/3d-reconstruction-from-multi-view-exp_amd/csrc/mvba_linearize.h
@@ -7,6 +7,10 @@
 template <bool GCAM, int LOSS = LOSS_SQUARED, typename... Robust>
 __global__ __launch_bounds__(1024, 4) void k_resid_jac(MVBA_RESID_JAC_ARGS, Robust... robust) {
   extern __shared__ __attribute__((aligned(16))) double smem[];
+  constexpr bool COMPACT = is_compact_rec<Robust...>::value;
+  static_assert(!COMPACT || LOSS == LOSS_SQUARED, "the compact record is the squared loss's");
+  constexpr int RS = COMPACT ? REC_C : REC;
+  auto swz = [](int row) { return COMPACT ? (row >> 1) & 3 : row & 7; };
   double *s_cam = smem;
   const int lane = threadIdx.x & 63, wave = threadIdx.x >> 6, nwave = blockDim.x >> 6;
   double2 *stage = reinterpret_cast<double2 *>(smem + (GCAM ? 0 : ((m * CAM_LDS + 1) & ~1))) + wave * (64 * REC);
@@ -46,16 +50,21 @@
         }
         la.sqw[o] = sw;
       }
-      double2 *row = stage + lane * REC;
-      const int sw = lane & 7;
+      double2 *row = stage + lane * RS;
+      const int sw = swz(lane);
       row[0 ^ sw] = make_double2(J.jx[0][0], J.jx[1][0]);
       row[1 ^ sw] = make_double2(J.jx[0][1], J.jx[1][1]);
       row[2 ^ sw] = make_double2(J.jx[0][2], J.jx[1][2]);
       row[3 ^ sw] = make_double2(J.jc[0][0], J.jc[1][0]);
-      row[4 ^ sw] = make_double2(J.jc[0][6], J.jc[1][6]);
-      row[5 ^ sw] = make_double2(J.jc[0][7], J.jc[1][7]);
-      row[6 ^ sw] = make_double2(J.jc[0][8], J.jc[1][8]);
-      row[7 ^ sw] = make_double2(J.e0, J.e1);
+      if constexpr (COMPACT) {
+        const CompactRec cr = (robust, ...);
+        cr.res[o] = make_double2(J.e0, J.e1);
+      } else {
+        row[4 ^ sw] = make_double2(J.jc[0][6], J.jc[1][6]);
+        row[5 ^ sw] = make_double2(J.jc[0][7], J.jc[1][7]);
+        row[6 ^ sw] = make_double2(J.jc[0][8], J.jc[1][8]);
+        row[7 ^ sw] = make_double2(J.e0, J.e1);
+      }
       c9[0] = 2.0 * (J.jx[0][0] * J.jx[0][0] + J.jx[1][0] * J.jx[1][0]);
       c9[1] = 2.0 * (J.jx[0][0] * J.jx[0][1] + J.jx[1][0] * J.jx[1][1]);
       c9[2] = 2.0 * (J.jx[0][0] * J.jx[0][2] + J.jx[1][0] * J.jx[1][2]);
@@ -68,10 +77,10 @@
     }
     wave_sync();
 #pragma unroll
-    for (int q = 0; q < REC; ++q) {
-      const int ol = q * 8 + (lane >> 3), pos = lane & 7;
-      const double2 v = stage[ol * REC + pos];
-      if (ol < n) rec[(wbase + ol) * REC + (pos ^ (ol & 7))] = v;
+    for (int q = 0; q < RS; ++q) {
+      const int ol = q * (64 / RS) + lane / RS, pos = lane % RS;
+      const double2 v = stage[ol * RS + pos];
+      if (ol < n) rec[(wbase + ol) * RS + (pos ^ swz(ol))] = v;
     }
     wave_sync();
     const int a_prev = __shfl_up(a, 1, 64);
@@ -116,7 +125,7 @@
 __global__ __launch_bounds__(256) void k_point_inv(long long npts, double c, const double *__restrict__ PL,
                                                    double *__restrict__ PB, int *__restrict__ flag,
                                                    double *__restrict__ Ab, long long nAb, int *__restrict__ prog, long long nprog, int want_r,
-                                                   Held... held) {
+                                                   const double *__restrict__ Xc, Held... held) {
   static_assert(sizeof...(Held) <= 1, "at most the held mask");
   __shared__ double2 s_out[256 * 8];
   double *s_in = reinterpret_cast<double *>(s_out);
@@ -146,6 +155,10 @@
       const int sw = threadIdx.x & 7;
 #pragma unroll
       for (int q = 0; q < 8; ++q) out[q ^ sw] = make_double2(0.0, q == 4 ? 1.0 : 0.0);
+      if (Xc) {
+        out[6 ^ sw] = make_double2(Xc[3 * a], Xc[3 * a + 1]);
+        out[7 ^ sw] = make_double2(Xc[3 * a + 2], 0.0);
+      }
     }
   }
   if (free_pt) {
@@ -176,6 +189,10 @@
       out[7 ^ sw] = make_double2(l21 * a1, a2);
     } else {
       out[5 ^ sw] = out[6 ^ sw] = out[7 ^ sw] = make_double2(0.0, 0.0);
+      if (Xc) {
+        out[6 ^ sw] = make_double2(Xc[3 * a], Xc[3 * a + 1]);
+        out[7 ^ sw] = make_double2(Xc[3 * a + 2], 0.0);
+      }
     }
   }
   __syncthreads();
diff --git a/3d-reconstruction-from-multi-view-exp_amd/csrc/mvba_schur.h b/3d-reconstruction-from-multi-view-exp_amd/csrc/mvba_schur.h
--- a/3d-reconstruction-from-multi-view-exp_amd/csrc/mvba_schur.h
+++ b/3d-reconstruction-from-multi-view-exp_amd/csrc/mvba_schur.h
@@ -6,11 +6,13 @@
 constexpr int SLOT_IDX = 64;
 constexpr int SLOT_IDX_RING = 3;
 
-template <int W, bool DIAG, bool PACKED>
+template <int W, bool DIAG, bool PACKED, bool COMPACT = false>
 struct SchurStage {
-  static constexpr int NPS = DIAG ? 5 : 3;
-  static constexpr int L = W * PROW;
-  static constexpr int P = L + ((PACKED && DIAG) ? W * 16 : W * PROW);
+  static_assert(!COMPACT || PACKED, "the compact rows are the slot forms'");
+  static constexpr int ROW = COMPACT ? 4 * 16 : PROW;
+  static constexpr int NPS = (DIAG ? 5 : 3) + (COMPACT ? 2 : 0);
+  static constexpr int L = W * ROW;
+  static constexpr int P = L + ((PACKED && DIAG) ? W * 16 : W * ROW);
   static constexpr int SIZE = P + W * 16 * (PACKED ? NPS : 5);
   static constexpr int SQW = DIAG ? L + W * 16 : P + W * 16 * NPS;
   static constexpr int SQW_END = SQW + (DIAG ? 1 : 2) * W * 8;
@@ -474,6 +476,24 @@
   if (flags & 1) schur_lanes_run<true>(smem_pairs, (int)threadIdx.x, beg, nsteps, it_x, rec_r, PB, c, 1.0 / f0, partial, su);
   else schur_lanes_run<false>(smem_pairs, (int)threadIdx.x, beg, nsteps, it_x, rec_r, PB, c, 1.0 / f0, partial, su);
 }
+__global__ __launch_bounds__(64, 1) void k_schur_lanes_compact(const int4 *__restrict__ wdesc, const int *__restrict__ wunits,
+                                                               const int *__restrict__ it_x, const double2 *__restrict__ rec,
+                                                               const double *__restrict__ PB, double c, double f0,
+                                                               double *__restrict__ partial, int nR,
+                                                               const long long *__restrict__ range_o0, const double2 *__restrict__ res,
+                                                               const int4 *__restrict__ units, const double *__restrict__ cam15) {
+  extern __shared__ char smem_pairs[];
+  const int bid = blockIdx.x;
+  const int MVBA_CONST_AS *dp = as_const(reinterpret_cast<const int *>(wdesc)) + 4 * (size_t)bid;
+  const int d_x = dp[0], d_y = dp[1], nsteps = dp[2], flags = dp[3];
+  if (nsteps <= 0) return;
+  const long long beg = ((long long)d_y << 32) | (unsigned)d_x;
+  const int *su = wunits + (size_t)bid * LANES_W;
+  const long long o0 = as_const(range_o0)[bid % nR];
+  const LanesCompact cx{res + o0, units, cam15};
+  if (flags & 1) schur_lanes_run<true, true>(smem_pairs, (int)threadIdx.x, beg, nsteps, it_x, rec + (size_t)o0 * REC_C, PB, c, 1.0 / f0, partial, su, cx);
+  else schur_lanes_run<false, true>(smem_pairs, (int)threadIdx.x, beg, nsteps, it_x, rec + (size_t)o0 * REC_C, PB, c, 1.0 / f0, partial, su, cx);
+}
 
 __global__ __launch_bounds__(128) void k_schur_reduce(int m, const int *__restrict__ unit_ptr,
                                                       const double *__restrict__ partial, double *__restrict__ Afull,
diff --git a/3d-reconstruction-from-multi-view-exp_amd/lib/_mvba.py b/3d-reconstruction-from-multi-view-exp_amd/lib/_mvba.py
--- a/3d-reconstruction-from-multi-view-exp_amd/lib/_mvba.py
+++ b/3d-reconstruction-from-multi-view-exp_amd/lib/_mvba.py
@@ -404,7 +404,8 @@
     def schur_info(self):
         i = self._info()
         return {"items": i[0], "offdiag_items": i[1], "units": i[2], "kernel": ("strip", "pairs", "slots", "dense")[i[3] & 0xff],
-                "slot_rows": i[7], "step_width": (i[3] >> 8) & 0xff}
+                "slot_rows": i[7], "step_width": (i[3] >> 8) & 0xff,
+                "record": "compact" if (i[3] >> 16) & 1 else "full"}
 
     def rccl_version(self):
         i = self._info()
```

Result: faster. 443.6 (median of 6 runs) (+2.7%).
